# Danderson123/Amira

Measured on AMD Instinct MI355X. Metric: gene-mers/s to corrected GeneMerGraph, higher is better.
Workload: dtype int32; 1 GPU; synthetic 1M reads x 60 genes, k=5, 20k-gene vocab: build + error-correction sweep (build, filter(3,1), correct, build, clip(5), correct, build); reads_per_gpu=1000000, genes_per_read=60, k=5, vocab=20000, gene_mers_per_gpu=56000000, final_nodes=472478, final_edges=1054844, multi_gpu=n/a

## Files before the change

amira_amd/csrc/amg_adjacency.hip:

```cpp
#include "amg_device.h"

__global__ void k_adj_keys(const int* __restrict__ e_src, const signed char* __restrict__ e_sdir,
                           long long n_edges, unsigned int* __restrict__ keys,
                           unsigned int* __restrict__ vals) {
  long long e = (long long)blockIdx.x * blockDim.x + threadIdx.x;
  if (e >= n_edges) return;
  keys[e] = 2u * (unsigned int)e_src[e] + (e_sdir[e] > 0 ? 0u : 1u);
  vals[e] = (unsigned int)e;
}

__global__ void k_row_offsets(const unsigned int* __restrict__ keys, long long n_edges, long long n_rows,
                              long long* __restrict__ off) {
  long long i = (long long)blockIdx.x * blockDim.x + threadIdx.x;
  if (i > n_edges) return;
  const long long prev = i > 0 ? (long long)keys[i - 1] : -1;
  const long long cur = i < n_edges ? (long long)keys[i] : n_rows;
  for (long long r = prev + 1; r <= cur; ++r) off[r] = i;
}

__device__ __forceinline__ unsigned int adj_row_of(const int* __restrict__ e_src, const signed char* __restrict__ e_sdir,
                                                   long long e) {
  return 2u * (unsigned int)e_src[e] + (e_sdir[e] > 0 ? 0u : 1u);
}

__global__ void k_adjc_ticket(const int* __restrict__ e_src, const signed char* __restrict__ e_sdir, long long n_edges,
                              unsigned int* __restrict__ cnt, unsigned int* __restrict__ tick) {
  long long e = (long long)blockIdx.x * blockDim.x + threadIdx.x;
  if (e < n_edges) tick[e] = atomicAdd(&cnt[adj_row_of(e_src, e_sdir, e)], 1u);
}

__global__ void k_adjc_fill(const int* __restrict__ e_src, const signed char* __restrict__ e_sdir, long long n_edges,
                            const long long* __restrict__ off, const unsigned int* __restrict__ tick,
                            unsigned int* __restrict__ tmp) {
  long long e = (long long)blockIdx.x * blockDim.x + threadIdx.x;
  if (e < n_edges) tmp[off[adj_row_of(e_src, e_sdir, e)] + tick[e]] = (unsigned int)e;
}

__global__ __launch_bounds__(256) void k_adjc_rows(const long long* __restrict__ off, long long n_rows,
                                                   const unsigned int* __restrict__ tmp, int* __restrict__ adj_edge,
                                                   unsigned int* __restrict__ long_rows, unsigned long long* n_long) {
  long long r = (long long)blockIdx.x * blockDim.x + threadIdx.x;
  long long o = 0;
  int cnt = 0;
  if (r < n_rows) {
    o = off[r];
    cnt = (int)(off[r + 1] - o);
  }
  bool mine = cnt > 2;
  if (cnt == 1) {
    adj_edge[o] = (int)tmp[o];
  } else if (cnt == 2) {
    const unsigned int a = tmp[o], b = tmp[o + 1];
    adj_edge[o] = (int)(a < b ? a : b);
    adj_edge[o + 1] = (int)(a < b ? b : a);
  } else if (cnt > WAVE_ROW_MAX) {
    long_rows[atomicAdd(n_long, 1ull)] = (unsigned int)r;
    mine = false;
  }
  wave_rows_in_order(mine, 0u, o, cnt, tmp,
                     [&](unsigned int, long long ro, int, int rank, unsigned int x) { adj_edge[ro + rank] = (int)x; });
}

#define HUB_BLOCKS 8
__global__ __launch_bounds__(256) void k_adjc_long(const unsigned int* __restrict__ long_rows,
                                                   const unsigned long long* __restrict__ n_long,
                                                   const long long* __restrict__ off, const unsigned int* __restrict__ tmp,
                                                   int* __restrict__ adj_edge, unsigned int* hub_bits, long long hub_words) {
  __shared__ unsigned int s_wave[4];
  const unsigned long long n = *n_long;
  for (unsigned long long q = blockIdx.x; q < n; q += gridDim.x) {
    const unsigned int r = long_rows[q];
    const long long o = off[r];
    const int cnt = (int)(off[r + 1] - o);
    if (cnt > HUGE_ROW) continue;
    for (int j = threadIdx.x; j < cnt; j += 256) {
      const unsigned int x = tmp[o + j];
      int rank = 0;
      for (int i = 0; i < cnt; ++i) rank += tmp[o + i] < x ? 1 : 0;
      adj_edge[o + rank] = (int)x;
    }
  }
  if (blockIdx.x >= HUB_BLOCKS) return;
  for (unsigned long long q = blockIdx.x; q < n; q += HUB_BLOCKS) {
    const unsigned int r = long_rows[q];
    const long long o = off[r];
    const long long cnt = off[r + 1] - o;
    if (cnt <= HUGE_ROW) continue;
    huge_row_in_order(tmp + o, cnt, hub_bits + (long long)blockIdx.x * hub_words, hub_words, s_wave,
                      [&](long long rank, unsigned int id) { adj_edge[o + rank] = (int)id; });
  }
}

__global__ void k_uf_init(int* parent, long long n) {
  long long i = (long long)blockIdx.x * blockDim.x + threadIdx.x;
  if (i < n) parent[i] = (int)i;
}

__global__ void k_uf_links(const unsigned long long* __restrict__ pkey, long long n_pairs, unsigned int* __restrict__ starts) {
  long long i = (long long)blockIdx.x * blockDim.x + threadIdx.x;
  if (i >= n_pairs) return;
  const unsigned long long key = pkey[i];
  const unsigned int a = (unsigned int)((key >> 32) & 0x7fffffffull), b = (unsigned int)(key & 0xffffffffull) - 1u;
  if (b == a + 1u) starts[b] = 0u;
}

__global__ void k_uf_run_starts(const unsigned int* __restrict__ starts, const long long* __restrict__ run_of, long long n,
                                int* __restrict__ run_start) {
  long long i = (long long)blockIdx.x * blockDim.x + threadIdx.x;
  if (i < n && starts[i]) run_start[run_of[i]] = (int)i;
}

__global__ void k_uf_init_runs(const unsigned int* __restrict__ starts, const long long* __restrict__ run_of,
                               const int* __restrict__ run_start, long long n, int* __restrict__ parent) {
  long long i = (long long)blockIdx.x * blockDim.x + threadIdx.x;
  if (i < n) parent[i] = run_start[run_of[i] + (long long)starts[i] - 1];
}

__global__ void k_uf_union(const unsigned long long* __restrict__ pkey, long long n_pairs, int* parent) {
  long long i = (long long)blockIdx.x * blockDim.x + threadIdx.x;
  if (i >= n_pairs) return;
  unsigned long long key = pkey[i];
  int a = (int)((key >> 32) & 0x7fffffffull);
  int b = (int)((key & 0xffffffffull) - 1ull);
  if (b == a + 1) return;
  while (true) {
    a = uf_find(parent, a);
    b = uf_find(parent, b);
    if (a == b) break;
    if (a > b) { int t = a; a = b; b = t; }
    int old = atomicCAS(parent + b, b, a);
    if (old == b) break;
    b = old;
  }
}

__global__ void k_uf_roots(int* parent, long long n, unsigned int* __restrict__ is_root, int* __restrict__ root_copy) {
  long long i = (long long)blockIdx.x * blockDim.x + threadIdx.x;
  if (i == 0) is_root[n] = 0u;
  if (i >= n) return;
  int r = uf_find(parent, (int)i);
  parent[i] = r;
  root_copy[i] = r;
  is_root[i] = (r == (int)i) ? 1u : 0u;
}

__global__ void k_uf_label(const int* __restrict__ root, const long long* __restrict__ root_rank,
                           long long n, int* __restrict__ comp) {
  long long i = (long long)blockIdx.x * blockDim.x + threadIdx.x;
  if (i >= n) return;
  int r = root[i];
  while (root[r] != r) r = root[r];
  comp[i] = (int)(root_rank[r] + 1);
}

int ensure_components(amg_ctx* c) {
  if (c->comp_valid) return AMG_OK;
  if (c->comp_from_claims) return bx_components_from_claims(c);
  hipStream_t st = c->stream;
  const long long P = c->n_pairs, D = c->n_nodes;
  stage_begin(c, "components");
  AMGCHK(c->node_comp.ensure((size_t)(D + 1) * sizeof(int)));
  int* parent = c->node_comp.as<int>();
  AMGCHK(c->s1.ensure((size_t)(D + 2) * sizeof(long long)));
  AMGCHK(c->s2.ensure((size_t)(D + 2) * sizeof(unsigned int) + (size_t)(D + 2) * sizeof(int)));
  unsigned int* is_root = c->s2.as<unsigned int>();
  int* root_copy = reinterpret_cast<int*>(is_root + (D + 2));
  long long ncomp = 0;
  if (D > 0) {
    if (P > 0) {
      AMGCHK(c->s3.ensure((size_t)(D + 2) * sizeof(unsigned int)));
      AMGCHK(c->s4.ensure((size_t)(D + 2) * sizeof(int)));
      AMGCHK(c->s5.ensure((size_t)(D + 2) * sizeof(long long)));
      unsigned int* starts = c->s3.as<unsigned int>();
      int* run_start = c->s4.as<int>();
      long long* run_of = c->s5.as<long long>();
      ClearList cl;
      cl.add(starts, (size_t)D * sizeof(unsigned int), 1u);
      AMGCHK(clear_many(c, cl));
      hipLaunchKernelGGL(k_uf_links, dim3(nblk(P, 256)), dim3(256), 0, st, c->pair_key.as<unsigned long long>(), P, starts);
      AMGCHK(prim_exscan_u32_to_i64(c, starts, run_of, (size_t)D));
      hipLaunchKernelGGL(k_uf_run_starts, dim3(nblk(D, 256)), dim3(256), 0, st, starts, run_of, D, run_start);
      hipLaunchKernelGGL(k_uf_init_runs, dim3(nblk(D, 256)), dim3(256), 0, st, starts, run_of, run_start, D, parent);
      hipLaunchKernelGGL(k_uf_union, dim3(nblk(P, 256)), dim3(256), 0, st,
                         c->pair_key.as<unsigned long long>(), P, parent);
    } else {
      hipLaunchKernelGGL(k_uf_init, dim3(nblk(D, 256)), dim3(256), 0, st, parent, D);
    }
    hipLaunchKernelGGL(k_uf_roots, dim3(nblk(D, 256)), dim3(256), 0, st, parent, D, is_root, root_copy);
    AMGCHK(prim_exscan_u32_to_i64(c, is_root, c->s1.as<long long>(), (size_t)D + 1));
    hipLaunchKernelGGL(k_uf_label, dim3(nblk(D, 256)), dim3(256), 0, st, root_copy,
                       c->s1.as<long long>(), D, parent);
    FetchList l;
    l.add(c->s1.as<long long>() + D);
    AMGCHK(fetch(c, l, reinterpret_cast<unsigned long long*>(&ncomp)));
  }
  stage_end(c);
  c->n_components = ncomp;
  c->comp_valid = true;
  return AMG_OK;
}

int ensure_adjacency(amg_ctx* c) {
  if (c->adj_valid) return AMG_OK;
  hipStream_t st = c->stream;
  const long long D = c->n_nodes, E = c->n_edges;
  stage_begin(c, "adjacency");
  AMGCHK(c->adj_off.ensure((size_t)(2 * D + 2) * sizeof(long long)));
  AMGCHK(c->adj_edge.ensure((size_t)(E + 2) * sizeof(int)));
  AMGCHK(c->s1.ensure((size_t)(E + 2) * sizeof(unsigned int)));
  AMGCHK(c->s2.ensure((size_t)(E + 2) * sizeof(unsigned int)));
  AMGCHK(c->s3.ensure((size_t)(E + 2) * sizeof(unsigned int)));
  const char* force_sort = getenv("AMG_ADJ_SORT");
  if (E > 0 && E <= (4ll << 20) && !(force_sort && force_sort[0] == '1')) {
    AMGCHK(c->s1.ensure((size_t)(2 * D + 2 > E + 2 ? 2 * D + 2 : E + 2) * sizeof(unsigned int)));
    unsigned int* cnt = c->s1.as<unsigned int>();
    unsigned int* tick = c->s2.as<unsigned int>();
    unsigned int* tmp = c->s3.as<unsigned int>();
    AMGCHK(c->s4.ensure((size_t)(E / WAVE_ROW_MAX + 2) * sizeof(unsigned int)));
    unsigned int* long_rows = c->s4.as<unsigned int>();
    unsigned long long* n_long = c->status.as<unsigned long long>() + ST_COMPACT_B;
    {
      ClearList cl;
      cl.add(cnt, (size_t)(2 * D + 2) * sizeof(unsigned int));
      cl.add(n_long, sizeof(unsigned long long));
      AMGCHK(clear_many(c, cl));
    }
    hipLaunchKernelGGL(k_adjc_ticket, dim3(nblk(E, 256)), dim3(256), 0, st, c->edge_src.as<int>(),
                       c->edge_sdir.as<signed char>(), E, cnt, tick);
    AMGCHK(prim_exscan_u32_to_i64(c, cnt, c->adj_off.as<long long>(), (size_t)(2 * D + 1)));
    hipLaunchKernelGGL(k_adjc_fill, dim3(nblk(E, 256)), dim3(256), 0, st, c->edge_src.as<int>(),
                       c->edge_sdir.as<signed char>(), E, c->adj_off.as<long long>(), tick, tmp);
    hipLaunchKernelGGL(k_adjc_rows, dim3(nblk(2 * D, 256)), dim3(256), 0, st, c->adj_off.as<long long>(), 2 * D, tmp,
                       c->adj_edge.as<int>(), long_rows, n_long);
    const long long hub_words = (E + 31) / 32 + 1;
    AMGCHK(c->hub_bits.ensure((size_t)HUB_BLOCKS * (size_t)hub_words * sizeof(unsigned int)));
    hipLaunchKernelGGL(k_adjc_long, dim3(256), dim3(256), 0, st, long_rows, n_long, c->adj_off.as<long long>(), tmp,
                       c->adj_edge.as<int>(), c->hub_bits.as<unsigned int>(), hub_words);
    stage_end(c);
    c->adj_valid = true;
    return AMG_OK;
  }
  if (E > 0) {
    hipLaunchKernelGGL(k_adj_keys, dim3(nblk(E, 256)), dim3(256), 0, st,
                       c->edge_src.as<int>(), c->edge_sdir.as<signed char>(), E,
                       c->s1.as<unsigned int>(), c->s2.as<unsigned int>());
    AMGCHK(prim_sort_u32_u32(c, c->s1.as<unsigned int>(), c->s3.as<unsigned int>(),
                             c->s2.as<unsigned int>(),
                             reinterpret_cast<unsigned int*>(c->adj_edge.p), (size_t)E,
                             ilog2_ceil((uint64_t)2 * D + 2) + 1));
  }
  hipLaunchKernelGGL(k_row_offsets, dim3(nblk(E + 1, 256)), dim3(256), 0, st,
                     c->s3.as<unsigned int>(), E, 2 * D, c->adj_off.as<long long>());
  stage_end(c);
  c->adj_valid = true;
  return AMG_OK;
}
```

amira_amd/csrc/amg_api.hip:

```cpp
#include <cstdarg>

#include "amg_device.h"

thread_local std::string g_amg_err;

int amg_fail(int code, const char* fmt, ...) {
  char buf[1024];
  va_list ap;
  va_start(ap, fmt);
  vsnprintf(buf, sizeof(buf), fmt, ap);
  va_end(ap);
  g_amg_err = buf;
  return code;
}

extern "C" const char* amg_last_error(void) { return g_amg_err.c_str(); }

void stages_reset(amg_ctx* c) {
  for (auto& s : c->stages) {
    (void)hipEventDestroy(s.a);
    (void)hipEventDestroy(s.b);
  }
  c->stages.clear();
}

void stage_begin(amg_ctx* c, const char* name) {
  if (!c->timing) return;
  StageTime s{name, nullptr, nullptr, 0.f};
  (void)hipEventCreate(&s.a);
  (void)hipEventCreate(&s.b);
  (void)hipEventRecord(s.a, c->stream);
  c->stages.push_back(s);
}

void stage_end(amg_ctx* c) {
  if (!c->timing || c->stages.empty()) return;
  (void)hipEventRecord(c->stages.back().b, c->stream);
}

extern "C" int amg_last_timings(amg_ctx* c, const char** names, float* ms, int cap) {
  if (!c) return amg_fail(AMG_E_ARG, "null ctx");
  (void)hipStreamSynchronize(c->stream);
  int n = 0;
  for (auto& s : c->stages) {
    if (n >= cap) break;
    float t = 0.f;
    if (hipEventElapsedTime(&t, s.a, s.b) != hipSuccess) t = -1.f;
    s.ms = t;
    names[n] = s.name;
    ms[n] = t;
    ++n;
  }
  return n;
}

extern "C" int amg_set_timing(amg_ctx* c, int on) {
  if (!c) return amg_fail(AMG_E_ARG, "null ctx");
  c->timing = on != 0;
  if (!c->timing) stages_reset(c);
  return AMG_OK;
}

__global__ __launch_bounds__(256) void k_clear_many(ClearArgs a) { clear_args_part(a, blockIdx.x, gridDim.x); }

__global__ void k_fetch(FetchList l, unsigned long long* mail, unsigned long long ticket) {
  const int i = threadIdx.x;
  const int n = l.n > 0 ? l.n : 1;
  if (i < n) {
    const unsigned long long v = i < l.n ? *l.p[i] : 0ull;
    mail[2 * i] = v;
    __threadfence_system();
    __hip_atomic_store(mail + 2 * i + 1, ticket, __ATOMIC_RELEASE, __HIP_MEMORY_SCOPE_SYSTEM);
  }
}

int fetch(amg_ctx* c, const FetchList& l, unsigned long long* out, const ClearList* filler) {
  if (l.overflow) return amg_fail(AMG_E_ARG, "fetch: more than %d words in one list", FETCH_MAX);
  const bool plain = getenv("AMG_PLAIN_SYNC") != nullptr;
  if (plain) {
    for (int i = 0; i < l.n; ++i)
      HIPCHK(hipMemcpyAsync(out + i, l.p[i], sizeof(unsigned long long), hipMemcpyDeviceToHost, c->stream));
    if (filler) AMGCHK(clear_many(c, *filler));
    HIPCHK(hipStreamSynchronize(c->stream));
    return AMG_OK;
  }
  if (!c->mail_host) {
    HIPCHK(hipHostMalloc(reinterpret_cast<void**>(&c->mail_host), 2 * (FETCH_MAX + 1) * sizeof(unsigned long long),
                         hipHostMallocMapped));
    HIPCHK(hipHostGetDevicePointer(reinterpret_cast<void**>(&c->mail_dev), c->mail_host, 0));
    for (int i = 0; i < 2 * (FETCH_MAX + 1); ++i) c->mail_host[i] = 0;
  }
  const unsigned long long ticket = ++c->mail_ticket;
  hipLaunchKernelGGL(k_fetch, dim3(1), dim3(FETCH_MAX <= 64 ? 64 : 128), 0, c->stream, l, c->mail_dev, ticket);
  if (filler) AMGCHK(clear_many(c, *filler));
  const int n = l.n > 0 ? l.n : 1;
  volatile unsigned long long* m = c->mail_host;
  int have = 0;
  for (unsigned long long spins = 0; have < n; ++spins) {
    while (have < n && __atomic_load_n(&m[2 * have + 1], __ATOMIC_ACQUIRE) == ticket) ++have;
    if (have == n) break;
    __builtin_ia32_pause();
    if ((spins & 0xfffffull) == 0xfffffull) {
      const hipError_t e = hipStreamQuery(c->stream);
      if (e != hipSuccess && e != hipErrorNotReady) return amg_fail(AMG_E_HIP, "%s", hipGetErrorString(e));
      if (e == hipSuccess) {
        while (have < n && __atomic_load_n(&m[2 * have + 1], __ATOMIC_ACQUIRE) == ticket) ++have;
        if (have < n) return amg_fail(AMG_E_HIP, "read-back kernel did not run");
      }
    }
  }
  for (int i = 0; i < l.n; ++i) out[i] = m[2 * i];
  return AMG_OK;
}

int stream_wait(amg_ctx* c) {
  FetchList l;
  return fetch(c, l, nullptr);
}

int fetch_status(amg_ctx* c, unsigned long long* out, const ClearList* filler) {
  FetchList l;
  l.add_words(c->status.p, ST_WORDS);
  return fetch(c, l, out, filler);
}

int clear_many(amg_ctx* c, const ClearList& l) {
  if (l.overflow) return amg_fail(AMG_E_ARG, "clear_many: more than %d ranges in one list", CLEAR_MAX);
  if (l.n == 0) return AMG_OK;
  const ClearArgs a = clear_args(l);
  unsigned long long most = 0;
  for (int i = 0; i < a.n; ++i) most = a.words[i] > most ? a.words[i] : most;
  unsigned long long blocks = (most / 4 + 256 * 8 - 1) / (256 * 8);
  if (blocks < 1) blocks = 1;
  if (blocks > 4096) blocks = 4096;
  hipLaunchKernelGGL(k_clear_many, dim3((unsigned int)blocks), dim3(256), 0, c->stream, a);
  return AMG_OK;
}

extern "C" int amg_create(int device, amg_ctx** out) {
  if (!out) return amg_fail(AMG_E_ARG, "null out pointer");
  *out = nullptr;
  int n = 0;
  hipError_t e = hipGetDeviceCount(&n);
  if (e != hipSuccess || n <= 0)
    return amg_fail(AMG_E_HIP, "no HIP device available (%s): libamg has no CPU path",
                    e == hipSuccess ? "count = 0" : hipGetErrorString(e));
  if (device < 0 || device >= n) return amg_fail(AMG_E_ARG, "device %d out of range [0,%d)", device, n);
  HIPCHK(hipSetDevice(device));
  amg_ctx* c = new amg_ctx();
  c->device = device;
  e = hipStreamCreateWithFlags(&c->stream, hipStreamNonBlocking);
  if (e != hipSuccess) {
    delete c;
    return amg_fail(AMG_E_HIP, "hipStreamCreate: %s", hipGetErrorString(e));
  }
  int r = c->status.ensure(ST_WORDS * sizeof(unsigned long long));
  if (r != AMG_OK) {
    delete c;
    return r;
  }
  const char* t = getenv("AMG_TIMING");
  c->timing = !(t && t[0] == '0');
  *out = c;
  return AMG_OK;
}

extern "C" int amg_destroy(amg_ctx* c) {
  if (!c) return AMG_OK;
  (void)hipSetDevice(c->device);
  (void)hipStreamSynchronize(c->stream);
  stages_reset(c);
  dist_release(c);
  bubbles_release(c);
  DevBuf* all[] = {&c->tokens,    &c->read_off,  &c->gene_start, &c->gene_end,  &c->read_len,
                   &c->node_tab,  &c->edge_tab,  &c->tok_slot,   &c->tok_node,  &c->tok_dir, &c->tok_pair,
                   &c->node_tokens, &c->node_cov, &c->node_first, &c->node_comp, &c->node_alive,
                   &c->edge_src,  &c->edge_tgt,  &c->edge_sdir,  &c->edge_tdir, &c->edge_cov,
                   &c->edge_alive, &c->adj_off,  &c->adj_edge,   &c->read_fix, &c->ladj_off, &c->ladj, &c->ladj_rows, &c->ladj_pos, &c->ladj_keys, &c->hub_bits, &c->pair_key, &c->pair_first, &c->pair_cnt, &c->match_read, &c->match_pos, &c->match_off, &c->match_wave,  &c->c_tokens_buf,
                   &c->c_read_off, &c->c_orig,   &c->c_changed,  &c->c_gstart,  &c->c_gend,
                   &c->c_read_len, &c->status,   &c->sort_tmp, &c->scan_state,   &c->s0, &c->s1, &c->s2, &c->s3,
                   &c->s4, &c->s5, &c->cnt_state, &c->cnt_list, &c->bnd_bits, &c->nw_rec, &c->gap_rec, &c->gm_mask, &c->gm_tab, &c->gm_res, &c->gm_list, &c->gm_q, &c->gm_pool, &c->gm_gene, &c->gm_fail, &c->gm_ctr, &c->routes_dev, &c->nw_big, &c->x_first, &c->x_slot, &c->x_final, &c->x_efirst, &c->x_eslot, &c->x_ecnt, &c->x_ncnt, &c->x_ftag, &c->f_ctrs, &c->x_efinal, &c->x_first_all, &c->pos_off, &c->c_pos_off, &c->pos1_s, &c->pos1_e,
                   &c->c_src, &c->rd_src, &c->alt_tok_node, &c->alt_tok_dir, &c->alt_ntok, &c->alt_ncov, &c->alt_nfirst,
                   &c->alt_nalive, &c->alt_pkey, &c->alt_pfirst, &c->alt_pcnt};
  for (DevBuf* b : all) b->release();
  if (c->mail_host) (void)hipHostFree(c->mail_host);
  (void)hipStreamDestroy(c->stream);
  delete c;
  return AMG_OK;
}

extern "C" int amg_sync(amg_ctx* c) {
  if (!c) return amg_fail(AMG_E_ARG, "null ctx");
  HIPCHK(hipStreamSynchronize(c->stream));
  return AMG_OK;
}

extern "C" void* amg_stream(amg_ctx* c) { return c ? (void*)c->stream : nullptr; }

static int copy_in(amg_ctx* c, DevBuf& dst, const void* src, size_t bytes, int on_device) {
  if (on_device == 2) {
    dst.borrow(src, bytes);
    return AMG_OK;
  }
  AMGCHK(dst.ensure(bytes + 64));
  if (bytes)
    HIPCHK(hipMemcpyAsync(dst.p, src, bytes, on_device ? hipMemcpyDeviceToDevice : hipMemcpyHostToDevice,
                          c->stream));
  return AMG_OK;
}

extern "C" int amg_set_reads(amg_ctx* c, const int32_t* tokens, const int64_t* read_offsets,
                             int64_t n_reads, int32_t two_v, int on_device) {
  if (!c) return amg_fail(AMG_E_ARG, "null ctx");
  if (n_reads < 0 || !read_offsets) return amg_fail(AMG_E_ARG, "bad read_offsets / n_reads");
  if (two_v <= 0 || (two_v & 1)) return amg_fail(AMG_E_ARG, "two_v must be a positive even number");
  HIPCHK(hipSetDevice(c->device));
  int64_t n_tokens = 0;
  if (on_device) {
    HIPCHK(hipMemcpy(&n_tokens, read_offsets + n_reads, sizeof(int64_t), hipMemcpyDeviceToHost));
  } else {
    if (read_offsets[0] != 0) return amg_fail(AMG_E_ARG, "read_offsets[0] must be 0");
    for (int64_t r = 0; r < n_reads; ++r)
      if (read_offsets[r + 1] < read_offsets[r])
        return amg_fail(AMG_E_ARG, "read_offsets not monotone at read %lld", (long long)r);
    n_tokens = read_offsets[n_reads];
  }
  if (n_tokens < 0) return amg_fail(AMG_E_ARG, "read_offsets[n_reads] is negative");
  if (n_tokens > 0 && !tokens) return amg_fail(AMG_E_ARG, "null tokens");
  AMGCHK(copy_in(c, c->tokens, tokens, (size_t)n_tokens * sizeof(int32_t), on_device));
  AMGCHK(copy_in(c, c->read_off, read_offsets, (size_t)(n_reads + 1) * sizeof(int64_t), on_device));
  HIPCHK(hipStreamSynchronize(c->stream));
  c->n_reads = n_reads;
  c->n_tokens = n_tokens;
  c->two_v = two_v;
  c->have_pos = c->have_read_len = false;
  c->built = false;
  c->derive_ready = c->dist_candidate = false;
  c->hint_bound = 0;
  c->have_corrected = false;
  c->match_valid = false;
  c->node_hint = 0;
  c->cnt_hint_reset = true;
  return AMG_OK;
}

extern "C" int amg_set_positions(amg_ctx* c, const int64_t* gene_start, const int64_t* gene_end,
                                 const int64_t* read_len, int on_device) {
  if (!c) return amg_fail(AMG_E_ARG, "null ctx");
  if (c->two_v <= 0) return amg_fail(AMG_E_STATE, "amg_set_reads first");
  if (!gene_start || !gene_end) return amg_fail(AMG_E_ARG, "null positions");
  HIPCHK(hipSetDevice(c->device));
  AMGCHK(copy_in(c, c->gene_start, gene_start, (size_t)c->n_tokens * sizeof(int64_t), on_device));
  AMGCHK(copy_in(c, c->gene_end, gene_end, (size_t)c->n_tokens * sizeof(int64_t), on_device));
  c->have_pos = true;
  c->pos_identity = true;
  c->pos0_own = false;
  c->pos_n0 = c->n_tokens;
  c->pos1_used = c->c_pos1_used = 0;
  c->have_corrected = false;
  c->have_read_len = false;
  if (read_len) {
    AMGCHK(copy_in(c, c->read_len, read_len, (size_t)c->n_reads * sizeof(int64_t), on_device));
    c->have_read_len = true;
  }
  HIPCHK(hipStreamSynchronize(c->stream));
  return AMG_OK;
}

extern "C" int amg_set_read_lengths(amg_ctx* c, const int64_t* read_len, int on_device) {
  if (!c || !read_len) return amg_fail(AMG_E_ARG, "null argument");
  if (c->two_v <= 0) return amg_fail(AMG_E_STATE, "amg_set_reads first");
  HIPCHK(hipSetDevice(c->device));
  AMGCHK(copy_in(c, c->read_len, read_len, (size_t)c->n_reads * sizeof(int64_t), on_device));
  c->have_read_len = true;
  HIPCHK(hipStreamSynchronize(c->stream));
  return AMG_OK;
}

__global__ void k_count_flags(const unsigned char* __restrict__ f, long long n,
                              unsigned long long* out) {
  long long i = (long long)blockIdx.x * blockDim.x + threadIdx.x;
  unsigned long long v = (i < n && f[i]) ? 1ull : 0ull;
  for (int d = 32; d > 0; d >>= 1) v += __shfl_down(v, d, 64);
  if ((threadIdx.x & 63) == 0 && v) atomicAdd(out, v);
}

static int count_flags(amg_ctx* c, const DevBuf& buf, long long n, int64_t* out) {
  *out = 0;
  if (n <= 0) return AMG_OK;
  unsigned long long* ctr = c->status.as<unsigned long long>() + ST_MISC;
  HIPCHK(hipMemsetAsync(ctr, 0, sizeof(unsigned long long), c->stream));
  hipLaunchKernelGGL(k_count_flags, dim3((unsigned)((n + 255) / 256)), dim3(256), 0, c->stream,
                     buf.as<unsigned char>(), n, ctr);
  unsigned long long h = 0;
  HIPCHK(hipMemcpyAsync(&h, ctr, sizeof(h), hipMemcpyDeviceToHost, c->stream));
  HIPCHK(hipStreamSynchronize(c->stream));
  *out = (int64_t)h;
  return AMG_OK;
}

extern "C" int amg_sizes(amg_ctx* c, int64_t* n_reads, int64_t* n_tokens) {
  if (!c) return amg_fail(AMG_E_ARG, "null ctx");
  if (n_reads) *n_reads = c->n_reads;
  if (n_tokens) *n_tokens = c->n_tokens;
  return AMG_OK;
}

extern "C" int amg_graph_sizes(amg_ctx* c, int64_t* n_nodes, int64_t* n_edges, int32_t* k) {
  if (!c) return amg_fail(AMG_E_ARG, "null ctx");
  if (!c->built) return amg_fail(AMG_E_STATE, "amg_build first");
  if (n_nodes) *n_nodes = c->n_nodes;
  if (n_edges) *n_edges = c->n_edges;
  if (k) *k = c->k;
  return AMG_OK;
}

extern "C" int amg_counts(amg_ctx* c, amg_counts_t* o) {
  if (!c || !o) return amg_fail(AMG_E_ARG, "null argument");
  memset(o, 0, sizeof(*o));
  o->n_reads = c->n_reads;
  o->n_tokens = c->n_tokens;
  o->two_v = c->two_v;
  if (!c->built) return AMG_OK;
  HIPCHK(hipSetDevice(c->device));
  o->k = c->k;
  o->n_windows = c->n_windows;
  o->n_short_reads = c->n_short;
  o->n_nodes = c->n_nodes;
  o->n_edges = c->n_edges;
  o->n_pairs = c->n_pairs;
  AMGCHK(ensure_components(c));
  o->n_components = c->n_components;
  o->node_table_slots = c->node_slots;
  o->edge_table_slots = c->edge_slots;
  o->exact_keys = c->exact_keys ? (c->x_fp ? 2 : 1) : 0;
  o->derived = c->derived ? 1 : 0;
  o->build_retries = c->retries;
  AMGCHK(count_flags(c, c->node_alive, c->n_nodes, &o->n_live_nodes));
  AMGCHK(count_flags(c, c->edge_alive, c->n_edges, &o->n_live_edges));
  AMGCHK(count_flags(c, c->read_fix, c->n_reads, &o->n_reads_to_correct));
  return AMG_OK;
}

static int d2h(amg_ctx* c, void* dst, const DevBuf& src, size_t bytes) {
  if (!dst || bytes == 0) return AMG_OK;
  HIPCHK(hipMemcpyAsync(dst, src.p, bytes, hipMemcpyDeviceToHost, c->stream));
  return AMG_OK;
}

__global__ void k_first_split(const long long* __restrict__ first, long long n,
                              long long* __restrict__ tok, signed char* __restrict__ dir) {
  long long i = (long long)blockIdx.x * blockDim.x + threadIdx.x;
  if (i >= n) return;
  long long f = first[i];
  tok[i] = f >> 1;
  dir[i] = (f & 1) ? -1 : 1;
}

extern "C" int amg_get_nodes(amg_ctx* c, int32_t* canon_tokens, uint32_t* coverage,
                             int64_t* first_token, int8_t* first_dir, int32_t* component,
                             uint8_t* alive) {
  NEED_BUILT(c);
  const size_t D = (size_t)c->n_nodes;
  if (component) AMGCHK(ensure_components(c));
  AMGCHK(d2h(c, canon_tokens, c->node_tokens, D * c->k * sizeof(int32_t)));
  AMGCHK(d2h(c, coverage, c->node_cov, D * sizeof(uint32_t)));
  AMGCHK(d2h(c, component, c->node_comp, D * sizeof(int32_t)));
  AMGCHK(d2h(c, alive, c->node_alive, D));
  if ((first_token || first_dir) && D) {
    AMGCHK(c->s1.ensure(D * sizeof(long long)));
    AMGCHK(c->s2.ensure(D));
    hipLaunchKernelGGL(k_first_split, dim3((unsigned)((D + 255) / 256)), dim3(256), 0, c->stream,
                       c->node_first.as<long long>(), (long long)D, c->s1.as<long long>(),
                       c->s2.as<signed char>());
    AMGCHK(d2h(c, first_token, c->s1, D * sizeof(int64_t)));
    AMGCHK(d2h(c, first_dir, c->s2, D));
  }
  HIPCHK(hipStreamSynchronize(c->stream));
  return AMG_OK;
}

extern "C" int amg_get_edges(amg_ctx* c, int32_t* src, int32_t* tgt, int8_t* sdir, int8_t* tdir,
                             uint32_t* coverage, uint8_t* alive) {
  NEED_BUILT(c);
  const size_t E = (size_t)c->n_edges;
  AMGCHK(d2h(c, src, c->edge_src, E * sizeof(int32_t)));
  AMGCHK(d2h(c, tgt, c->edge_tgt, E * sizeof(int32_t)));
  AMGCHK(d2h(c, sdir, c->edge_sdir, E));
  AMGCHK(d2h(c, tdir, c->edge_tdir, E));
  AMGCHK(d2h(c, coverage, c->edge_cov, E * sizeof(uint32_t)));
  AMGCHK(d2h(c, alive, c->edge_alive, E));
  HIPCHK(hipStreamSynchronize(c->stream));
  return AMG_OK;
}

extern "C" int amg_get_read_nodes(amg_ctx* c, int32_t* tok_node, int8_t* tok_dir) {
  NEED_BUILT(c);
  AMGCHK(d2h(c, tok_node, c->tok_node, (size_t)c->n_tokens * sizeof(int32_t)));
  AMGCHK(d2h(c, tok_dir, c->tok_dir, (size_t)c->n_tokens));
  HIPCHK(hipStreamSynchronize(c->stream));
  return AMG_OK;
}

__global__ __launch_bounds__(256) void k_gather_read_nodes(const int* __restrict__ tok_node,
                                                            const long long* __restrict__ first, const long long* __restrict__ start,
                                                            long long n_rows, int* __restrict__ out) {
  const long long r = (long long)blockIdx.x * 4 + (threadIdx.x >> 6);
  if (r >= n_rows) return;
  const long long a = first[r], o = start[r], n = start[r + 1] - o;
  for (long long i = threadIdx.x & 63; i < n; i += 64) out[o + i] = tok_node[a + i];
}

extern "C" int amg_get_read_nodes_rows(amg_ctx* c, const int64_t* first_token, const int64_t* out_start, int64_t n_rows,
                                       int32_t* node_ids) {
  NEED_BUILT(c);
  if (n_rows < 0 || (n_rows > 0 && (!first_token || !out_start || !node_ids))) return amg_fail(AMG_E_ARG, "bad arguments");
  if (n_rows == 0) return AMG_OK;
  const long long total = out_start[n_rows];
  for (int64_t r = 0; r < n_rows; ++r) {
    const long long n = out_start[r + 1] - out_start[r];
    if (out_start[0] != 0 || n < 0 || first_token[r] < 0 || first_token[r] + n > c->n_tokens)
      return amg_fail(AMG_E_ARG, "amg_get_read_nodes_rows: row %lld lies outside the read set", (long long)r);
  }
  if (total == 0) return AMG_OK;
  hipStream_t st = c->stream;
  AMGCHK(c->s0.ensure((size_t)n_rows * sizeof(long long)));
  AMGCHK(c->s1.ensure((size_t)(n_rows + 1) * sizeof(long long)));
  AMGCHK(c->s2.ensure((size_t)total * sizeof(int)));
  HIPCHK(hipMemcpyAsync(c->s0.p, first_token, (size_t)n_rows * sizeof(long long), hipMemcpyHostToDevice, st));
  HIPCHK(hipMemcpyAsync(c->s1.p, out_start, (size_t)(n_rows + 1) * sizeof(long long), hipMemcpyHostToDevice, st));
  hipLaunchKernelGGL(k_gather_read_nodes, dim3((unsigned)((n_rows + 3) / 4)), dim3(256), 0, st, c->tok_node.as<int>(),
                     c->s0.as<long long>(), c->s1.as<long long>(), (long long)n_rows, c->s2.as<int>());
  HIPCHK(hipMemcpyAsync(node_ids, c->s2.p, (size_t)total * sizeof(int), hipMemcpyDeviceToHost, st));
  HIPCHK(hipStreamSynchronize(st));
  return AMG_OK;
}

extern "C" int amg_get_node_adj(amg_ctx* c, int64_t* offsets, int32_t* edge_ids) {
  NEED_BUILT(c);
  AMGCHK(ensure_adjacency(c));
  AMGCHK(d2h(c, offsets, c->adj_off, (size_t)(2 * c->n_nodes + 1) * sizeof(int64_t)));
  AMGCHK(d2h(c, edge_ids, c->adj_edge, (size_t)c->n_edges * sizeof(int32_t)));
  HIPCHK(hipStreamSynchronize(c->stream));
  return AMG_OK;
}

extern "C" int amg_get_reads_to_correct(amg_ctx* c, uint8_t* flags) {
  NEED_BUILT(c);
  AMGCHK(d2h(c, flags, c->read_fix, (size_t)c->n_reads));
  HIPCHK(hipStreamSynchronize(c->stream));
  return AMG_OK;
}

__global__ void k_read_window_count(const int* __restrict__ tok_node,
                                    const long long* __restrict__ read_off, long long n_reads,
                                    unsigned int* __restrict__ cnt) {
  long long r = (long long)blockIdx.x * blockDim.x + threadIdx.x;
  if (r >= n_reads) return;
  unsigned int n = 0;
  for (long long t = read_off[r]; t < read_off[r + 1]; ++t) n += tok_node[t] >= 0 ? 1u : 0u;
  cnt[r] = n;
}

__global__ void k_read_window_emit(const int* __restrict__ tok_node,
                                   const long long* __restrict__ read_off, long long n_reads,
                                   const long long* __restrict__ base, unsigned int* __restrict__ keys,
                                   unsigned int* __restrict__ vals) {
  long long r = (long long)blockIdx.x * blockDim.x + threadIdx.x;
  if (r >= n_reads) return;
  long long o = base[r];
  for (long long t = read_off[r]; t < read_off[r + 1]; ++t) {
    int n = tok_node[t];
    if (n >= 0) {
      keys[o] = (unsigned int)n;
      vals[o] = (unsigned int)r;
      ++o;
    }
  }
}

__global__ void k_mark_first_of_run(const unsigned int* __restrict__ keys,
                                    const unsigned int* __restrict__ vals, long long n,
                                    unsigned int* __restrict__ keep,
                                    unsigned int* __restrict__ per_node) {
  long long i = (long long)blockIdx.x * blockDim.x + threadIdx.x;
  if (i >= n) return;
  unsigned int kf = (i == 0 || keys[i] != keys[i - 1] || vals[i] != vals[i - 1]) ? 1u : 0u;
  keep[i] = kf;
  if (kf) atomicAdd(&per_node[keys[i]], 1u);
}

__global__ void k_scatter_kept(const unsigned int* __restrict__ vals, const unsigned int* __restrict__ keep,
                               const long long* __restrict__ pos, long long n, int* __restrict__ out) {
  long long i = (long long)blockIdx.x * blockDim.x + threadIdx.x;
  if (i >= n) return;
  if (keep[i]) out[pos[i]] = (int)vals[i];
}

extern "C" int amg_get_node_reads(amg_ctx* c, int64_t* offsets, int32_t* read_idx) {
  NEED_BUILT(c);
  if (!offsets) return amg_fail(AMG_E_ARG, "offsets must not be NULL");
  hipStream_t st = c->stream;
  const long long R = c->n_reads, D = c->n_nodes;
  AMGCHK(c->s0.ensure((size_t)(R + 2) * sizeof(unsigned int)));
  AMGCHK(c->s5.ensure((size_t)(R + 2) * sizeof(long long)));
  HIPCHK(hipMemsetAsync(c->s0.p, 0, (size_t)(R + 2) * sizeof(unsigned int), st));
  if (R > 0)
    hipLaunchKernelGGL(k_read_window_count, dim3((unsigned)((R + 255) / 256)), dim3(256), 0, st,
                       c->tok_node.as<int>(), c->read_off.as<long long>(), R, c->s0.as<unsigned int>());
  AMGCHK(prim_exscan_u32_to_i64(c, c->s0.as<unsigned int>(), c->s5.as<long long>(), (size_t)R + 1));
  long long W = 0;
  HIPCHK(hipMemcpyAsync(&W, c->s5.as<long long>() + R, sizeof(long long), hipMemcpyDeviceToHost, st));
  HIPCHK(hipStreamSynchronize(st));
  AMGCHK(c->s1.ensure((size_t)(W + 2) * sizeof(unsigned int)));
  AMGCHK(c->s2.ensure((size_t)(W + 2) * sizeof(unsigned int)));
  AMGCHK(c->s3.ensure((size_t)(W + 2) * sizeof(unsigned int)));
  AMGCHK(c->s4.ensure((size_t)(W + 2) * sizeof(unsigned int)));
  if (R > 0)
    hipLaunchKernelGGL(k_read_window_emit, dim3((unsigned)((R + 255) / 256)), dim3(256), 0, st,
                       c->tok_node.as<int>(), c->read_off.as<long long>(), R, c->s5.as<long long>(),
                       c->s1.as<unsigned int>(), c->s2.as<unsigned int>());
  AMGCHK(prim_sort_u32_u32(c, c->s1.as<unsigned int>(), c->s3.as<unsigned int>(),
                           c->s2.as<unsigned int>(), c->s4.as<unsigned int>(), (size_t)W,
                           ilog2_ceil((uint64_t)D + 2) + 1));
  AMGCHK(c->s0.ensure((size_t)(D + 2) * sizeof(unsigned int)));
  HIPCHK(hipMemsetAsync(c->s0.p, 0, (size_t)(D + 2) * sizeof(unsigned int), st));
  if (W > 0)
    hipLaunchKernelGGL(k_mark_first_of_run, dim3((unsigned)((W + 255) / 256)), dim3(256), 0, st,
                       c->s3.as<unsigned int>(), c->s4.as<unsigned int>(), W,
                       c->s1.as<unsigned int>(), c->s0.as<unsigned int>());
  AMGCHK(c->s5.ensure((size_t)(D + 2) * sizeof(long long)));
  AMGCHK(prim_exscan_u32_to_i64(c, c->s0.as<unsigned int>(), c->s5.as<long long>(), (size_t)D + 1));
  AMGCHK(d2h(c, offsets, c->s5, (size_t)(D + 1) * sizeof(int64_t)));
  HIPCHK(hipStreamSynchronize(st));
  if (read_idx && W > 0) {
    long long total = offsets[D];
    AMGCHK(c->s2.ensure((size_t)(W + 2) * sizeof(long long)));
    HIPCHK(hipMemsetAsync(c->s1.as<unsigned int>() + W, 0, sizeof(unsigned int), st));
    AMGCHK(prim_exscan_u32_to_i64(c, c->s1.as<unsigned int>(), c->s2.as<long long>(), (size_t)W + 1));
    AMGCHK(c->s0.ensure((size_t)(total + 2) * sizeof(int)));
    hipLaunchKernelGGL(k_scatter_kept, dim3((unsigned)((W + 255) / 256)), dim3(256), 0, st,
                       c->s4.as<unsigned int>(), c->s1.as<unsigned int>(), c->s2.as<long long>(), W,
                       c->s0.as<int>());
    AMGCHK(d2h(c, read_idx, c->s0, (size_t)total * sizeof(int32_t)));
    HIPCHK(hipStreamSynchronize(st));
  }
  return AMG_OK;
}
```

amira_amd/csrc/amg_build.hip:

```cpp
#include "amg_device.h"

#include "amg_tile.h"

uint64_t pow2_at_least(uint64_t x) {
  uint64_t p = 1024;
  while (p < x) p <<= 1;
  return p;
}

int bs_read_stats(amg_ctx* c, int k, const ClearList* also) {
  hipStream_t st = c->stream;
  const long long T = c->n_tokens, R = c->n_reads;
  stage_begin(c, "read_stats");
  const size_t words = (size_t)(T >> 5) + BND_PAD_WORDS;
  AMGCHK(c->bnd_bits.ensure(words * sizeof(unsigned int)));
  {
    ClearList cl;
    if (also) cl = *also;
    cl.add(c->bnd_bits.p, words * sizeof(unsigned int));
    AMGCHK(clear_many(c, cl));
  }
  if (R > 0)
    hipLaunchKernelGGL(k_read_stats, dim3(nblk(R, 256) < 512u ? nblk(R, 256) : 512u), dim3(256), 0, st,
                       c->read_off.as<long long>(), R, T, k, c->status.as<unsigned long long>(),
                       c->bnd_bits.as<unsigned int>());
  stage_end(c);
  return AMG_OK;
}

int bs_alloc_nodes(amg_ctx* c, long long D) {
  AMGCHK(c->node_tokens.ensure((size_t)(D * c->k + 1) * sizeof(int)));
  AMGCHK(c->node_cov.ensure((size_t)(D + 1) * sizeof(unsigned int)));
  AMGCHK(c->node_first.ensure((size_t)(D + 1) * sizeof(long long)));
  AMGCHK(c->node_comp.ensure((size_t)(D + 1) * sizeof(int)));
  AMGCHK(c->node_alive.ensure((size_t)(D + 1)));
  return AMG_OK;
}

int bs_alloc_pairs(amg_ctx* c, long long P) {
  AMGCHK(c->pair_key.ensure((size_t)(P + 2) * sizeof(unsigned long long)));
  AMGCHK(c->pair_first.ensure((size_t)(P + 2) * sizeof(unsigned long long)));
  AMGCHK(c->pair_cnt.ensure((size_t)(P + 2) * sizeof(unsigned int)));
  return AMG_OK;
}

int bs_finish_from_pairs(amg_ctx* c) {
  const long long P = c->n_pairs, R = c->n_reads;
  stage_begin(c, "edge_emit");
  AMGCHK(c->s5.ensure((size_t)(P + 2) * sizeof(long long)));
  long long* base = c->s5.as<long long>();
  const long long cap = 2 * P;
  AMGCHK(c->edge_src.ensure((size_t)(cap + 2) * sizeof(int)));
  AMGCHK(c->edge_tgt.ensure((size_t)(cap + 2) * sizeof(int)));
  AMGCHK(c->edge_sdir.ensure((size_t)(cap + 2)));
  AMGCHK(c->edge_tdir.ensure((size_t)(cap + 2)));
  AMGCHK(c->edge_cov.ensure((size_t)(cap + 2) * sizeof(unsigned int)));
  AMGCHK(c->edge_alive.ensure((size_t)(cap + 2)));
  AMGCHK(c->read_fix.ensure((size_t)R + 1));
  long long total = 0;
  {
    ClearList cl;
    cl.add(c->read_fix.p, (size_t)R + 1);
    if (P > 0) {
      AMGCHK(prim_exscan_emit_edges(c, c->pair_key.as<unsigned long long>(), c->pair_cnt.as<unsigned int>(),
                                    c->pair_first.as<unsigned long long>(), (size_t)P, base + P, c->edge_src.as<int>(),
                                    c->edge_tgt.as<int>(), c->edge_sdir.as<signed char>(), c->edge_tdir.as<signed char>(),
                                    c->edge_cov.as<unsigned int>(), c->edge_alive.as<unsigned char>(), &cl));
    } else {
      AMGCHK(clear_many(c, cl));
    }
  }
  {
    FetchList l;
    l.add(P > 0 ? static_cast<const void*>(base + P) : c->status.p);
    const bool learn = count_learn_add(c, &l);
    unsigned long long v[1 + COUNT_LEARN_WORDS] = {0};
    AMGCHK(fetch(c, l, v));
    if (P > 0) total = (long long)v[0];
    if (learn) count_learn_take(c, v + 1);
  }
  c->n_edges = total;
  stage_end(c);
  c->ladj_valid = false;
  c->ladj_stale = false;
  c->pristine = !c->comp_from_claims;
  c->edge_own_deaths = false;
  c->comp_valid = false;
  c->adj_valid = false;
  c->n_components = 0;
  return AMG_OK;
}

extern "C" int amg_finalize(amg_ctx* c) {
  if (!c) return amg_fail(AMG_E_ARG, "null ctx");
  if (!c->built) return amg_fail(AMG_E_STATE, "amg_build first");
  HIPCHK(hipSetDevice(c->device));
  stages_reset(c);
  AMGCHK(ensure_components(c));
  AMGCHK(ensure_adjacency(c));
  HIPCHK(hipStreamSynchronize(c->stream));
  return AMG_OK;
}

uint64_t slots_for(uint64_t n) {
  const uint64_t lo = n * 3, hi = n * 32, cap = 4ull << 20;
  const uint64_t want = hi < cap ? hi : cap;
  return pow2_at_least(want > lo ? want : lo);
}

void bs_size_tables(amg_ctx* c) {
  uint64_t want = c->node_hint > 0 ? slots_for((uint64_t)c->node_hint) : (uint64_t)c->n_tokens / 4;
  c->node_slots = (int64_t)pow2_at_least(want);
  if (c->node_slots > (1ll << 30)) c->node_slots = 1ll << 30;
  c->edge_slots = 1024;
}

BuildSwitches read_build_switches() {
  BuildSwitches sw;
  auto is_zero = [](const char* v) { return v && atoi(v) == 0; };
  if (const char* e = getenv("AMG_X_HEAD_TILES")) sw.head_tiles_set = true, sw.head_tiles = atoll(e);
  if (const char* e = getenv("AMG_CLAIM_SHARDS")) sw.claim_shards = atoi(e) != 0;
  sw.tight_bits = getenv("AMG_X_TIGHT_BITS") != nullptr;
  if (const char* e = getenv("AMG_KEY_MODE")) sw.key_fp = e[0] == 'f';
  sw.node_buckets = !is_zero(getenv("AMG_NODE_BUCKETS"));
  sw.generic_k = getenv("AMG_X_GENERIC_K") != nullptr;
  sw.rank_sort = getenv("AMG_X_RANK_SORT") != nullptr;
  if (const char* e = getenv("AMG_EDGE_LONE")) sw.edge_lone = atoi(e) != 0;
  sw.edge_home = !is_zero(getenv("AMG_EDGE_HOME"));
  sw.no_derive = getenv("AMG_NO_DERIVE") != nullptr;
  if (const char* e = getenv("AMG_TEST_WEAK_FP")) sw.weak_fp = atoi(e);
  if (const char* e = getenv("AMG_COUNT_INLINE")) sw.count_inline = e[0] == '1';
  if (const char* e = getenv("AMG_COUNT_LIST_SEG")) sw.count_list_seg = atoi(e);
  sw.count_debug = getenv("AMG_COUNT_DEBUG") != nullptr;
  return sw;
}

int grow_after_overflow(amg_ctx* c, Overflow cause) {
  ++c->retries;
  if (cause == OV_NODE_TABLE) {
    if (c->node_slots >= (1ll << 30)) return amg_fail(AMG_E_OVERFLOW, "node table at maximum size");
    c->node_slots = c->node_slots * 4 > (1ll << 30) ? (1ll << 30) : c->node_slots * 4;
  } else if (cause == OV_EDGE_TABLE) {
    c->edge_slots *= 4;
  } else {
    c->seed = c->seed * 6364136223846793005ull + 1442695040888963407ull;
    if (c->weak_fp_builds > 0) --c->weak_fp_builds;
  }
  return AMG_OK;
}

static int build_impl(amg_ctx* c, int32_t k, uint32_t min_node_cov, uint32_t min_edge_cov, bool* fused) {
  *fused = false;
  if (!c) return amg_fail(AMG_E_ARG, "null ctx");
  if (k < 1 || k > AMG_MAX_K) return amg_fail(AMG_E_ARG, "k must be in [1, %d]", AMG_MAX_K);
  if (c->two_v <= 0) return amg_fail(AMG_E_STATE, "amg_set_reads first");
  HIPCHK(hipSetDevice(c->device));
  stages_reset(c);
  c->sw = read_build_switches();
  const bool derive = c->derive_ready && k == c->k && !c->dist_mode && !c->sw.no_derive;
  c->derive_ready = c->dist_candidate = false;
  c->derived = false;
  c->built = false;
  c->have_corrected = false;
  c->match_valid = false;
  c->retries = 0;
  c->tok_base = 0;
  c->tok_total = c->n_tokens;
  if (derive) {
    bool done = false;
    AMGCHK(derive_from_previous(c, k, &done));
    if (done) return AMG_OK;
  }
  c->k = k;
  c->dist_mode = false;
  c->comp_from_claims = false;
  if (c->hint_bound > 0) {
    if (c->hint_bound_k == k) c->node_hint = c->hint_bound > 256 ? c->hint_bound : 256;
    c->hint_bound = 0;
  }
  c->weak_fp_builds = c->sw.weak_fp;
  c->count_inline = c->sw.count_inline;
  bs_size_tables(c);
  c->exact_keys = false;
  const bool exact = bx_applicable(c, k);
  for (int attempt = 0; attempt < 12; ++attempt) {
    Overflow which = OV_NONE;
    int r;
    if (exact && min_node_cov > 0) {
      r = bx_nodes_filtered(c, k, min_node_cov, &which);
      if (r == AMG_OK) r = bx_edges(c, &which, min_edge_cov);
      *fused = true;
    } else if (exact) {
      r = bx_nodes(c, k, &which);
      if (r == AMG_OK) r = bx_edges(c, &which);
    } else {
      r = bs_nodes_pass(c, k, &which);
      if (r == AMG_OK) r = bs_nodes_rank_local(c);
      if (r == AMG_OK) r = bs_edges_pass(c, &which);
      if (r == AMG_OK) r = bs_pairs_from_local(c);
    }
    if (r == AMG_OK) r = bs_finish_from_pairs(c);
    if (r == AMG_OK && *fused) r = bx_flag_dead_reads(c);
    if (r == AMG_OK) {
      c->built = true;
      const int64_t seen = *fused ? c->n_local_nodes : c->n_nodes;
      c->node_hint = seen > 256 ? seen : 256;
      return AMG_OK;
    }
    if (r != AMG_E_OVERFLOW || which == OV_NONE) return r;
    AMGCHK(grow_after_overflow(c, which));
  }
  return amg_fail(AMG_E_OVERFLOW, "build did not converge after 12 attempts");
}

extern "C" int amg_build(amg_ctx* c, int32_t k) {
  bool fused = false;
  return build_impl(c, k, 0, 0, &fused);
}

extern "C" int amg_build_filtered(amg_ctx* c, int32_t k, uint32_t min_node_cov, uint32_t min_edge_cov) {
  bool fused = false;
  const int r = build_impl(c, k, min_node_cov < 1 ? 1 : min_node_cov, min_edge_cov < 1 ? 1 : min_edge_cov, &fused);
  if (r != AMG_OK || fused) return r;
  return amg_filter(c, min_node_cov, min_edge_cov);
}

#define MULTI_MAX 8
extern "C" int amg_build_multi(amg_ctx* const* ctxs, const int32_t* ks, int32_t n) {
  if (!ctxs || !ks || n < 1 || n > MULTI_MAX) return amg_fail(AMG_E_ARG, "amg_build_multi: 1 .. %d graphs", MULTI_MAX);
  amg_ctx* c0 = ctxs[0];
  if (!c0 || c0->two_v <= 0) return amg_fail(AMG_E_STATE, "amg_set_reads on the first ctx first");
  for (int i = 0; i < n; ++i) {
    if (!ctxs[i]) return amg_fail(AMG_E_ARG, "null ctx");
    if (ctxs[i]->device != c0->device) return amg_fail(AMG_E_ARG, "amg_build_multi: one device");
    if (ks[i] < 1 || ks[i] > AMG_MAX_K) return amg_fail(AMG_E_ARG, "k must be in [1, %d]", AMG_MAX_K);
    for (int j = 0; j < i; ++j)
      if (ctxs[j] == ctxs[i]) return amg_fail(AMG_E_ARG, "amg_build_multi: one ctx per graph");
  }
  HIPCHK(hipSetDevice(c0->device));
  HIPCHK(hipStreamSynchronize(c0->stream));
  const long long T = c0->n_tokens, R = c0->n_reads;
  std::vector<hipStream_t> own(n);
  for (int i = 0; i < n; ++i) {
    amg_ctx* c = ctxs[i];
    own[i] = c->stream;
    if (i == 0) continue;
    HIPCHK(hipStreamSynchronize(c->stream));
    c->tokens.borrow(c0->tokens.p, (size_t)T * sizeof(int32_t));
    c->read_off.borrow(c0->read_off.p, (size_t)(R + 1) * sizeof(int64_t));
    c->n_reads = R;
    c->n_tokens = T;
    c->two_v = c0->two_v;
    c->have_pos = c->have_read_len = false;
    c->node_hint = 0;
    c->cnt_hint_reset = true;
    c->derive_ready = c->dist_candidate = false;
    c->stream = c0->stream;
  }
  struct Restore {
    amg_ctx* const* ctxs;
    std::vector<hipStream_t>& own;
    int n;
    ~Restore() {
      for (int i = 0; i < n; ++i) ctxs[i]->stream = own[i];
    }
  } restore{ctxs, own, n};
  for (int i = 0; i < n; ++i) AMGCHK(amg_build(ctxs[i], ks[i]));
  HIPCHK(hipStreamSynchronize(c0->stream));
  return AMG_OK;
}
```

amira_amd/csrc/amg_correct.h:

```cpp
#pragma once
#include "amg_device.h"

enum { RC_SKIP = 0, RC_COPY = 1, RC_DROP = 2, RC_TRIM = 3, RC_GAPPED = 4, RC_KEEP_ORIG = 5 };

struct CorrArgs {
  const int* tokens;
  const long long* read_off;
  const int* tok_node;
  const signed char* tok_dir;
  const unsigned char* read_fix;
  const long long* p0s;
  const long long* p0e;
  const long long* p1s;
  const long long* p1e;
  long long n0;
  const long long* pos_off;
  const long long* read_len;
  long long n_reads;
  int k, flip, have_pos;
  unsigned int* gflag;
  unsigned long long* max_bound;
  unsigned long long* lmask;
  unsigned long long* n_runs;
  unsigned char* cls;
  unsigned char* cls_final;
  int* r_start;
  int* r_end;
  unsigned int* bound;
  const long long* tmp_off;
  unsigned int* new_len;
  int* tmp_tok;
};

__device__ __forceinline__ void pos_base(const CorrArgs& a, long long off, const long long*& gs, const long long*& ge) {
  if (off < a.n0) {
    gs = a.p0s + off;
    ge = a.p0e + off;
  } else {
    gs = a.p1s + (off - a.n0);
    ge = a.p1e + (off - a.n0);
  }
}

__device__ __forceinline__ long long bcast_i64(long long v, int lane) {
  const unsigned int lo = (unsigned int)__builtin_amdgcn_readlane((int)(unsigned int)v, lane);
  const unsigned int hi = (unsigned int)__builtin_amdgcn_readlane((int)(unsigned int)((unsigned long long)v >> 32), lane);
  return (long long)(((unsigned long long)hi << 32) | lo);
}

__device__ __forceinline__ void wave_sync() {
  __builtin_amdgcn_fence(__ATOMIC_ACQ_REL, "wavefront");
  __builtin_amdgcn_wave_barrier();
}

struct __attribute__((aligned(16))) GapRec {
  int r, L0, start, end;
  long long t0, dst;
  unsigned long long mask;
  long long pad;
};

__device__ __forceinline__ unsigned long long gap_run_ends(unsigned long long lv, int start, int end) {
  const unsigned long long inside =
      (end >= 63 ? ~0ull : ((1ull << (end + 1)) - 1ull)) & ~((1ull << (start & 63)) - 1ull);
  return ~lv & inside & (lv >> 1);
}
__device__ __forceinline__ void gap_run_terminals(unsigned long long lv, int i, int& ps, int& pe) {
  ps = 63 - __clzll((long long)(lv & ((1ull << i) - 1ull)));
  pe = i + 1;
}

struct GapArgs {
  CorrArgs a;
  GView g;
  const GapRec* rec;
  const int* gapped_reads;
  long long n_gapped;
  int* pool;
  unsigned long long pool_cap;
  unsigned long long* pool_used;
  unsigned long long* status;
  int* cand;
  unsigned int cand_stride;
  unsigned char* final_cls;
  unsigned char* need_slow;
  const int* gq;
  const int4* qres;
  const int* qpool;
};

#define GF_MAXW 128
#define GF_MAXGAP 16
#define GF_POOL 384
#define GF_CAND 136
#define GF_MAXCOMBO 256
#define GM_INLINE 64
#define LEAN_CHUNK 32
#define CLS_READS 64
#define PACK_READS 64
enum {
  GS_NOT_TRIED = 1,
  GS_WINDOWS = 2,
  GS_RUNS = 3,
  GS_MEMO_UNFIT = 4,
  GS_RECORDS = 5,
  GS_COMBOS = 6,
  GS_CAND = 7,
  GS_CODES = 8
};
enum {
  GL_NO_SLOTS = 1,
  GL_ANSWERS = 2,
  GL_LONG = 3,
  GL_OTHER = 4,
  GL_CODES = 5
};

#define NWF_MAX_M 64
#define NWF_MAX_N 128
__device__ __forceinline__ bool nw_fast_ok(long long N, long long M) {
  return N <= NWF_MAX_N && M <= NWF_MAX_M && N > 0 && M > 0;
}

struct __attribute__((aligned(16))) NwRec {
  int r, M, N, pad;
  long long t0, dst;
  long long pdst;
  long long poff;
};

struct NwArgs {
  CorrArgs a;
  const NwRec* rec;
  long long* o_gs;
  long long* o_ge;
  const int* gapped_reads;
  long long n_gapped;
  const unsigned char* final_cls;
  const long long* big_off;
  unsigned char* big_buf;
  int allow_fast;
  int shortcuts;
};

struct PackArgs {
  CorrArgs a;
  const long long* new_idx;
  const long long* new_off;
  const unsigned char* final_cls;
  int* o_tok;
  long long* o_off;
  int* o_orig;
  unsigned char* o_changed;
  long long* o_src;
  const long long* pos_new;
  long long* o_posoff;
  long long* o_rl;
  long long out_reads, out_tokens;
  unsigned long long* dead_kept;
};

struct CorrSwitches {
  bool gap_memo;
  bool fast_gapped;
  bool lean_gapped;
  int fast_nw;
  int nw_shortcuts;
  const char* node_bound;
  bool routes;
  const char* gap_pool;
  const char* memo_spill;
};

struct CorrScratch {
  size_t per_read = 0;
  unsigned char *cls = nullptr, *final_cls = nullptr;
  int *r_start = nullptr, *r_end = nullptr;
  long long *nw_size = nullptr, *nw_off = nullptr;
  unsigned int *bound = nullptr, *new_len = nullptr, *flag = nullptr;
  long long *tmp_off = nullptr, *new_idx = nullptr, *new_off = nullptr;
  int* tmp_tok = nullptr;
  long long *plen = nullptr, *poffs = nullptr, *pos_new = nullptr;
  unsigned long long *max_bound = nullptr, *n_general = nullptr;
  unsigned long long* n_runs = nullptr;
  unsigned long long* dead_kept = nullptr;
  bool count_alive = false;
  DevBuf* glist = nullptr;
  DevBuf* cand = nullptr;
  DevBuf* pool = nullptr;
  DevBuf* need_slow = nullptr;
};

struct CorrCounts {
  long long tmp_total = 0, n_gapped = 0, total_runs = 0;
  unsigned long long max_bound = 0;
  bool carry = false;
  long long out_reads = 0, out_tokens = 0, big_total = 0, pos_total = 0;
  unsigned long long n_general = 0;
  long long n_queries = 0;
  int pool_retries = 0;
  bool lean_ran = false, fast_ran = false, memo = false;
};

static void fill_pos_args(amg_ctx* c, CorrArgs& a) {
  a.p0s = c->have_pos ? c->gene_start.as<long long>() : nullptr;
  a.p0e = c->have_pos ? c->gene_end.as<long long>() : nullptr;
  a.p1s = c->pos1_s.as<long long>();
  a.p1e = c->pos1_e.as<long long>();
  a.n0 = c->pos_n0;
  a.pos_off = (c->have_pos && !c->pos_identity) ? c->pos_off.as<long long>() : nullptr;
}

void corr_classify_launch(amg_ctx* c, const CorrArgs& a);
int corr_gapped(amg_ctx* c, const CorrSwitches& sw, const CorrScratch& S, const CorrArgs& a, CorrCounts& n);
int corr_nw_sizes(amg_ctx* c, const CorrSwitches& sw, const CorrScratch& S, const CorrArgs& a, long long n_gapped,
                  FetchList& shape);
int corr_grow_pos_pools(amg_ctx* c, const CorrCounts& n);
int corr_positions(amg_ctx* c, const CorrSwitches& sw, const CorrScratch& S, const CorrArgs& a, const CorrCounts& n);

int routes_begin(amg_ctx* c);
int routes_gapped(amg_ctx* c, const CorrScratch& S, const CorrCounts& n, const unsigned char* need_slow, const int* gq);
int routes_nw(amg_ctx* c, const CorrScratch& S, const CorrCounts& n);
int routes_end(amg_ctx* c, const CorrCounts& n);
```

amira_amd/csrc/amg_correct.hip:

```cpp
#include "amg_correct.h"

__global__ __launch_bounds__(256) void k_count_alive(const unsigned char* __restrict__ alive, long long n,
                                                     unsigned long long* out) {
  __shared__ unsigned int s_part[4];
  unsigned int c = 0;
  for (long long i = ((long long)blockIdx.x * blockDim.x + threadIdx.x) * 4; i < n; i += (long long)gridDim.x * blockDim.x * 4) {
    if (i + 4 <= n) {
      const unsigned int w = *reinterpret_cast<const unsigned int*>(alive + i);
      c += __popc(w & 0x01010101u);
    } else {
      for (long long j = i; j < n; ++j) c += alive[j] ? 1u : 0u;
    }
  }
  for (int d = 32; d > 0; d >>= 1) c += (unsigned int)__shfl_xor((int)c, d, 64);
  if ((threadIdx.x & 63) == 0) s_part[threadIdx.x >> 6] = c;
  __syncthreads();
  if (threadIdx.x == 0 && (s_part[0] | s_part[1] | s_part[2] | s_part[3]))
    atomicAdd(out, (unsigned long long)s_part[0] + s_part[1] + s_part[2] + s_part[3]);
}

__global__ __launch_bounds__(256) void k_corr_pack(PackArgs A) {
  const CorrArgs& a = A.a;
  const int lane = threadIdx.x & 63;
  const long long r = ((long long)blockIdx.x * 4 + (threadIdx.x >> 6)) * PACK_READS + lane;
  if (blockIdx.x == 0 && threadIdx.x == 0) A.o_off[A.out_reads] = A.out_tokens;
  long long dst = 0, src = 0;
  int n = 0;
  unsigned int dead = 0;
  if (r < a.n_reads && a.new_len[r] > 0) {
    dst = A.new_off[r];
    n = (int)a.new_len[r];
    const unsigned char fc = A.final_cls[r];
    if (fc == RC_KEEP_ORIG) {
      const long long nw = a.read_off[r + 1] - a.read_off[r] - a.k + 1;
      dead = nw <= 64 ? (unsigned int)(nw - __popcll(a.lmask[r])) : (unsigned int)nw;
    }
    long long poff = 0;
    if (fc == RC_GAPPED) {
      src = a.tmp_off[r] | (1ll << 62);
      if (a.have_pos) poff = A.pos_new[r];
    } else {
      const long long cut = fc == RC_TRIM ? a.r_start[r] : 0;
      src = a.read_off[r] + cut;
      if (a.have_pos) poff = (a.pos_off ? a.pos_off[r] : a.read_off[r]) + cut;
    }
    const long long q = A.new_idx[r];
    A.o_off[q] = dst;
    A.o_orig[q] = (int)r;
    A.o_changed[q] = (fc == RC_TRIM || fc == RC_GAPPED) ? 1 : 0;
    A.o_src[q] = fc == RC_GAPPED ? -1ll : src;
    if (a.have_pos) A.o_posoff[q] = poff;
    if (a.read_len) A.o_rl[q] = a.read_len[r];
  }
  if (__ballot(dead != 0u) != 0ull) {
    for (int d = 32; d > 0; d >>= 1) dead += (unsigned int)__shfl_xor((int)dead, d, 64);
    if (lane == 0) atomicAdd(A.dead_kept + 16 * (blockIdx.x & 15), (unsigned long long)dead);
  }
  if (__ballot(n > 0) == 0ull) return;
  for (int j0 = 0; j0 < PACK_READS; j0 += 4) {
    const int* sp[4];
    long long d[4];
    int nn[4], vt[4];
#pragma unroll
    for (int j = 0; j < 4; ++j) {
      nn[j] = __builtin_amdgcn_readlane(n, j0 + j);
      const long long sj = bcast_i64(src, j0 + j);
      d[j] = bcast_i64(dst, j0 + j);
      sp[j] = ((sj >> 62) & 1 ? a.tmp_tok : a.tokens) + (sj & ~(1ll << 62));
    }
#pragma unroll
    for (int j = 0; j < 4; ++j)
      if (lane < nn[j]) vt[j] = sp[j][lane];
#pragma unroll
    for (int j = 0; j < 4; ++j)
      if (lane < nn[j]) A.o_tok[d[j] + lane] = vt[j];
#pragma unroll
    for (int j = 0; j < 4; ++j)
      for (int i = 64 + lane; i < nn[j]; i += 64)
        A.o_tok[d[j] + i] = sp[j][i];
  }
}

static CorrSwitches read_switches() {
  auto is_one = [](const char* name) {
    const char* v = getenv(name);
    return v && v[0] == '1';
  };
  CorrSwitches sw;
  sw.gap_memo = !is_one("AMG_NO_GAP_MEMO");
  sw.fast_gapped = !is_one("AMG_NO_FAST_GAPPED");
  sw.lean_gapped = !is_one("AMG_NO_LEAN_GAPPED");
  sw.fast_nw = !is_one("AMG_NO_FAST_NW");
  sw.nw_shortcuts = !is_one("AMG_NW_NO_SHORTCUT");
  sw.node_bound = getenv("AMG_TEST_NODE_BOUND");
  sw.routes = is_one("AMG_CORR_ROUTES");
  sw.gap_pool = getenv("AMG_TEST_GAP_POOL");
  sw.memo_spill = getenv("AMG_TEST_MEMO_SPILL");
  return sw;
}

static int plan_per_read(amg_ctx* c, CorrScratch& S) {
  const size_t per_read = (size_t)(c->n_reads + 2);
  AMGCHK(c->s0.ensure(per_read * (1 + 1) + 64));
  AMGCHK(c->s1.ensure(per_read * sizeof(int) * 2 + per_read * sizeof(long long) * 2 + 64));
  AMGCHK(c->s2.ensure(per_read * sizeof(unsigned int) * 3));
  AMGCHK(c->s3.ensure(per_read * sizeof(long long) * 3));
  AMGCHK(c->gm_mask.ensure(per_read * sizeof(unsigned long long)));
  AMGCHK(c->gm_ctr.ensure((16 + 256 + 256 + 16) * sizeof(unsigned long long)));
  S.per_read = per_read;
  S.cls = c->s0.as<unsigned char>();
  S.final_cls = S.cls + per_read;
  S.r_start = c->s1.as<int>();
  S.r_end = S.r_start + per_read;
  S.nw_size = reinterpret_cast<long long*>(((uintptr_t)(S.r_end + per_read) + 15) & ~(uintptr_t)15);
  S.nw_off = S.nw_size + per_read;
  S.bound = c->s2.as<unsigned int>();
  S.new_len = S.bound + per_read;
  S.flag = S.new_len + per_read;
  S.tmp_off = c->s3.as<long long>();
  S.new_idx = S.tmp_off + per_read;
  S.new_off = S.new_idx + per_read;
  S.max_bound = S.n_general = c->status.as<unsigned long long>() + ST_MISC;
  S.n_runs = c->gm_ctr.as<unsigned long long>() + 16;
  S.dead_kept = S.n_runs + 256;
  S.count_alive = c->n_nodes >= (1ll << 20);
  S.glist = &c->c_orig;
  S.cand = &c->c_gstart;
  S.pool = &c->c_gend;
  S.need_slow = &c->c_changed;
  return AMG_OK;
}

static int plan_staging(amg_ctx* c, CorrScratch& S, long long tmp_total) {
  AMGCHK(c->c_tokens_buf.ensure((size_t)(tmp_total + 4) * sizeof(int)));
  AMGCHK(c->s4.ensure((size_t)(tmp_total + 4) * sizeof(int)));
  S.tmp_tok = c->s4.as<int>();
  return AMG_OK;
}

static int plan_positions(amg_ctx* c, CorrScratch& S, long long n_gapped) {
  AMGCHK(c->s5.ensure((size_t)(2 * (n_gapped + 2) + c->n_reads + 2) * sizeof(long long)));
  S.plen = c->s5.as<long long>();
  S.poffs = S.plen + (n_gapped + 2);
  S.pos_new = S.poffs + (n_gapped + 2);
  return AMG_OK;
}

static void corr_args(amg_ctx* c, const CorrScratch& S, CorrArgs& a) {
  a.tokens = c->tokens.as<int>();
  a.read_off = c->read_off.as<long long>();
  a.tok_node = c->tok_node.as<int>();
  a.tok_dir = c->tok_dir.as<signed char>();
  a.read_fix = c->read_fix.as<unsigned char>();
  fill_pos_args(c, a);
  a.read_len = c->have_read_len ? c->read_len.as<long long>() : nullptr;
  a.n_reads = c->n_reads;
  a.k = c->k;
  a.flip = c->two_v - 1;
  a.have_pos = c->have_pos ? 1 : 0;
  a.gflag = S.flag;
  a.max_bound = S.max_bound;
  a.lmask = c->gm_mask.as<unsigned long long>();
  a.n_runs = S.n_runs;
  a.cls = S.cls;
  a.cls_final = S.final_cls;
  a.r_start = S.r_start;
  a.r_end = S.r_end;
  a.bound = S.bound;
  a.tmp_off = S.tmp_off;
  a.new_len = S.new_len;
  a.tmp_tok = S.tmp_tok;
}

static int corr_classify(amg_ctx* c, const CorrScratch& S, const CorrArgs& a, CorrCounts& n) {
  hipStream_t st = c->stream;
  const long long R = c->n_reads;
  {
    ClearList cl;
    cl.add(S.bound, S.per_read * sizeof(unsigned int) * 3);
    cl.add(S.max_bound, sizeof(unsigned long long));
    cl.add(S.n_runs, (256 + 256 + 16) * sizeof(unsigned long long));
    AMGCHK(clear_many(c, cl));
  }
  if (R > 0) corr_classify_launch(c, a);
  if (S.count_alive)
    hipLaunchKernelGGL(k_count_alive, dim3(128), dim3(256), 0, st, c->node_alive.as<unsigned char>(), c->n_nodes,
                       S.dead_kept + 256);
  AMGCHK(prim_exscan_u32_pair(c, S.bound, S.tmp_off, S.flag, S.new_idx, (size_t)R));
  FetchList l;
  l.add(S.tmp_off + R);
  l.add(S.max_bound);
  l.add(S.new_idx + R);
  for (int i = 0; i < 16; ++i) l.add(S.n_runs + 16 * i);
  unsigned long long v[3 + 16];
  AMGCHK(fetch(c, l, v));
  n.tmp_total = (long long)v[0];
  n.max_bound = v[1];
  n.n_gapped = (long long)v[2];
  for (int i = 0; i < 16; ++i) n.total_runs += (long long)v[3 + i];
  n.carry = n.n_gapped > 0 && c->have_pos;
  return AMG_OK;
}

static int corr_shape(amg_ctx* c, const CorrSwitches& sw, CorrScratch& S, const CorrArgs& a, CorrCounts& n) {
  const long long R = c->n_reads;
  AMGCHK(prim_exscan_keep_and_len(c, S.new_len, S.new_idx, S.new_off, (size_t)R));
  FetchList shape;
  shape.add(S.new_idx + R);
  shape.add(S.new_off + R);
  if (n.carry) {
    AMGCHK(plan_positions(c, S, n.n_gapped));
    AMGCHK(corr_nw_sizes(c, sw, S, a, n.n_gapped, shape));
  }
  unsigned long long v[5] = {0, 0, 0, 0, 0};
  AMGCHK(fetch(c, shape, v));
  n.out_reads = (long long)v[0];
  n.out_tokens = (long long)v[1];
  n.big_total = (long long)v[2];
  n.pos_total = (long long)v[3];
  n.n_general = v[4];
  return AMG_OK;
}

static int ensure_outputs(amg_ctx* c, const CorrCounts& n) {
  AMGCHK(c->c_tokens_buf.ensure((size_t)(n.out_tokens + 64) * sizeof(int)));
  AMGCHK(c->c_read_off.ensure((size_t)(n.out_reads + 2) * sizeof(long long)));
  AMGCHK(c->c_orig.ensure((size_t)(n.out_reads + 2) * sizeof(int)));
  AMGCHK(c->c_changed.ensure((size_t)(n.out_reads + 2)));
  AMGCHK(c->c_src.ensure((size_t)(n.out_reads + 2) * sizeof(long long)));
  if (c->have_pos) AMGCHK(c->c_pos_off.ensure((size_t)(n.out_reads + 2) * sizeof(long long)));
  if (c->have_read_len) AMGCHK(c->c_read_len.ensure((size_t)(n.out_reads + 2) * sizeof(long long)));
  return AMG_OK;
}

static int corr_pack(amg_ctx* c, const CorrScratch& S, const CorrArgs& a, const CorrCounts& n) {
  PackArgs Pk;
  Pk.a = a;
  Pk.new_idx = S.new_idx;
  Pk.new_off = S.new_off;
  Pk.final_cls = S.final_cls;
  Pk.o_tok = c->c_tokens_buf.as<int>();
  Pk.o_off = c->c_read_off.as<long long>();
  Pk.o_orig = c->c_orig.as<int>();
  Pk.o_changed = c->c_changed.as<unsigned char>();
  Pk.o_src = c->c_src.as<long long>();
  Pk.pos_new = S.pos_new;
  Pk.o_posoff = c->have_pos ? c->c_pos_off.as<long long>() : nullptr;
  Pk.o_rl = c->have_read_len ? c->c_read_len.as<long long>() : nullptr;
  Pk.out_reads = n.out_reads;
  Pk.out_tokens = n.out_tokens;
  Pk.dead_kept = S.dead_kept;
  if (c->n_reads > 0)
    hipLaunchKernelGGL(k_corr_pack, dim3(nblk(c->n_reads, 4 * PACK_READS)), dim3(256), 0, c->stream, Pk);
  else
    HIPCHK(hipMemcpyAsync(c->c_read_off.as<long long>() + n.out_reads, &n.out_tokens, sizeof(long long),
                          hipMemcpyHostToDevice, c->stream));
  return AMG_OK;
}

static int corr_node_bound(amg_ctx* c, const CorrSwitches& sw, const CorrScratch& S, const CorrCounts& n) {
  FetchList l;
  for (int i = 0; i < 16; ++i) l.add(S.dead_kept + 16 * i);
  l.add(S.dead_kept + 256);
  unsigned long long v[17];
  AMGCHK(fetch(c, l, v));
  unsigned long long bound = S.count_alive ? v[16] : (unsigned long long)c->n_nodes;
  unsigned long long dead_kept = 0;
  for (int i = 0; i < 16; ++i) dead_kept += v[i];
  bound += dead_kept;
  c->c_derivable = n.n_gapped == 0 && dead_kept == 0 && !c->edge_own_deaths;
  c->c_node_bound = (int64_t)bound;
  if (sw.node_bound) c->c_node_bound = atoll(sw.node_bound);
  c->c_node_bound_k = c->k;
  return AMG_OK;
}

extern "C" int amg_correct_reads(amg_ctx* c, int64_t* n_out_reads, int64_t* n_out_tokens) {
  NEED_BUILT(c);
  const CorrSwitches sw = read_switches();
  stages_reset(c);
  c->have_corrected = false;
  CorrScratch S;
  CorrCounts n;
  CorrArgs a;
  AMGCHK(plan_per_read(c, S));
  corr_args(c, S, a);
  c->have_routes = false;
  if (sw.routes) AMGCHK(routes_begin(c));

  stage_begin(c, "correct_classify");
  AMGCHK(corr_classify(c, S, a, n));
  stage_end(c);
  AMGCHK(plan_staging(c, S, n.tmp_total));
  corr_args(c, S, a);

  if (n.n_gapped > 0) {
    stage_begin(c, "live_adjacency");
    AMGCHK(ensure_live_adj(c));
    stage_end(c);
    stage_begin(c, "correct_gapped");
    AMGCHK(corr_gapped(c, sw, S, a, n));
    stage_end(c);
  }

  stage_begin(c, "correct_pack");
  AMGCHK(corr_shape(c, sw, S, a, n));
  stage_end(c);
  AMGCHK(ensure_outputs(c, n));

  if (n.carry) {
    stage_begin(c, "correct_positions");
    AMGCHK(corr_grow_pos_pools(c, n));
    corr_args(c, S, a);
    AMGCHK(corr_positions(c, sw, S, a, n));
    if (sw.routes) AMGCHK(routes_nw(c, S, n));
    stage_end(c);
  }

  stage_begin(c, "correct_pack");
  AMGCHK(corr_pack(c, S, a, n));
  AMGCHK(corr_node_bound(c, sw, S, n));
  stage_end(c);
  if (sw.routes) AMGCHK(routes_end(c, n));
  c->c_reads = n.out_reads;
  c->c_tokens = n.out_tokens;
  c->c_pos1_used = c->pos1_used + (n.carry ? n.pos_total : 0);
  c->have_corrected = true;
  if (n_out_reads) *n_out_reads = n.out_reads;
  if (n_out_tokens) *n_out_tokens = n.out_tokens;
  return AMG_OK;
}
```

amira_amd/csrc/amg_count.hip:

```cpp
#include "amg_device.h"

#define HOT_IDS 39936
#define COUNT_MAX_SWEEPS 4
#define COUNT_LIST_SEG 256
#define COUNT_MAX_BLOCKS 256
#define COUNT_LIST_HEAD (2 + COUNT_MAX_BLOCKS)
struct CountSweeps {
  unsigned long long beyond[COUNT_MAX_SWEEPS];
  unsigned long long done[COUNT_MAX_SWEEPS];
};
struct CountHint { unsigned long long beyond, n; };
struct CountState {
  CountSweeps sweeps[2];
  CountHint hint[2];
};

template <bool GATHER>
__global__ __launch_bounds__(1024) void k_count_ids(int* __restrict__ ids, long long n,
                                                    const Slot* __restrict__ tab, long long lo,
                                                    int sweep, int last, CountSweeps* state,
                                                    CountHint* hint, unsigned int* __restrict__ out,
                                                    bool marked, unsigned int* list, unsigned int seg_cap) {
  __shared__ unsigned int s_cnt[HOT_IDS];
  __shared__ unsigned int s_listed;
  bool tail_all = last != 0;
  if (sweep > 0) {
    for (int q = 0; q < sweep; ++q)
      if (state->done[q]) return;
    const unsigned long long left = state->beyond[sweep - 1];
    if (sweep == 1 && blockIdx.x == 0 && threadIdx.x == 0) {
      hint->beyond = left;
      hint->n = (unsigned long long)n;
    }
    if (left == 0ull) return;
    if (sweep == 1 && list && list[1] == 1u && list[0] == 0u) {
      const unsigned int mine = list[2 + blockIdx.x];
      for (unsigned int i = threadIdx.x; i < mine; i += 1024u)
        atomicAdd(&out[list[COUNT_LIST_HEAD + blockIdx.x * COUNT_LIST_SEG + i]], 1u);
      if (blockIdx.x == 0 && threadIdx.x == 0) state->done[sweep] = 1ull;
      return;
    }
    if (left * 8ull <= (unsigned long long)n) tail_all = true;
  } else if (hint->n != 0ull && hint->beyond * 8ull <= hint->n) {
    tail_all = true;
  }
  const bool listing = sweep == 0 && !tail_all && list != nullptr && gridDim.x <= COUNT_MAX_BLOCKS;
  if (threadIdx.x == 0) s_listed = 0u;
  auto list_id = [&](int id) {
    const unsigned int at = atomicAdd(&s_listed, 1u);
    if (at < seg_cap) list[COUNT_LIST_HEAD + blockIdx.x * COUNT_LIST_SEG + at] = (unsigned int)id;
  };
  for (int i = threadIdx.x; i < HOT_IDS; i += 1024) s_cnt[i] = 0;
  __syncthreads();
  const long long stride = (long long)gridDim.x * 1024;
  unsigned int beyond = 0;
  auto tally = [&](int id, long long t) {
    bool made = false;
    if (marked && id != -1) {
      made = ((unsigned int)id & AMG_MADE_FLAG) != 0u;
      id = (int)((unsigned int)id & ~AMG_FLAG_MASK);
    }
    if (GATHER) {
      id = id < 0 ? -1 : tab[id].id;
      ids[t] = id;
    }
    if (id < 0 || made) return;
    const long long rel = (long long)id - lo;
    if (rel < 0) return;
    if (rel < HOT_IDS) {
      atomicAdd(&s_cnt[rel], 1u);
    } else {
      ++beyond;
      if (tail_all) atomicAdd(&out[id], 1u);
      else if (listing) list_id(id);
    }
  };
  typedef int i4 __attribute__((ext_vector_type(4)));
  const long long n4 = ((reinterpret_cast<uintptr_t>(ids) & 15) == 0) ? (n >> 2) : 0;
  i4* ids4 = reinterpret_cast<i4*>(ids);
  long long q = (long long)blockIdx.x * 1024 + threadIdx.x;
  auto tally4 = [&](i4 x, long long qi) {
    unsigned int mades = 0;
    if (marked) {
#pragma unroll
      for (int j = 0; j < 4; ++j)
        if (x[j] != -1 && ((unsigned int)x[j] & AMG_MADE_FLAG)) mades |= 1u << j;
    }
    if (GATHER) {
      i4 y;
#pragma unroll
      for (int j = 0; j < 4; ++j) {
        int id = x[j];
        if (marked && id != -1) id = (int)((unsigned int)id & ~AMG_FLAG_MASK);
        y[j] = id < 0 ? -1 : tab[id].id;
      }
      ids4[qi] = y;
      x = y;
    }
#pragma unroll
    for (int j = 0; j < 4; ++j) {
      int id = x[j];
      if (!GATHER && marked && id != -1) id = (int)((unsigned int)id & ~AMG_FLAG_MASK);
      if (id < 0 || (mades & (1u << j))) continue;
      const long long rel = (long long)id - lo;
      if (rel < 0) continue;
      if (rel < HOT_IDS) {
        atomicAdd(&s_cnt[rel], 1u);
      } else {
        ++beyond;
        if (tail_all) atomicAdd(&out[id], 1u);
        else if (listing) list_id(id);
      }
    }
  };
  for (; q + 3 * stride < n4; q += 4 * stride) {
    i4 v[4];
#pragma unroll
    for (int j = 0; j < 4; ++j) v[j] = GATHER ? ids4[q + j * stride] : __builtin_nontemporal_load(ids4 + q + j * stride);
#pragma unroll
    for (int j = 0; j < 4; ++j) tally4(v[j], q + j * stride);
  }
  for (; q < n4; q += stride) tally4(GATHER ? ids4[q] : __builtin_nontemporal_load(ids4 + q), q);
  for (long long t = 4 * n4 + (long long)blockIdx.x * 1024 + threadIdx.x; t < n; t += stride) tally(ids[t], t);
  for (int d = 32; d > 0; d >>= 1) beyond += __shfl_down(beyond, d, 64);
  if ((threadIdx.x & 63) == 0 && beyond) atomicAdd(&state->beyond[sweep], (unsigned long long)beyond);
  if (tail_all && blockIdx.x == 0 && threadIdx.x == 0) state->done[sweep] = 1ull;
  __syncthreads();
  if (listing && threadIdx.x == 0) {
    const unsigned int got = s_listed;
    list[2 + blockIdx.x] = got < seg_cap ? got : seg_cap;
    if (got > seg_cap) list[0] = 1u;
    if (blockIdx.x == 0) list[1] = 1u;
  }
  for (int i = threadIdx.x; i < HOT_IDS; i += 1024) {
    const unsigned int cnt = s_cnt[i];
    if (cnt) atomicAdd(&out[lo + i], cnt);
  }
}

static_assert(sizeof(CountState) == (4 * COUNT_MAX_SWEEPS + 4) * sizeof(unsigned long long), "cnt_state: two blocks, two hints");

int count_ids(amg_ctx* c, CountKind what, CountIds form, int* ids, long long n, long long n_ids, unsigned int* out,
              const Slot* gather_tab) {
  hipStream_t st = c->stream;
  const bool marked = form == IdsClaimsMarked;
  ClearList cl;
  cl.add(out, (size_t)(n_ids + 1) * sizeof(unsigned int), marked ? 1u : 0u);
  const bool fresh = !c->cnt_state.p || c->cnt_hint_reset;
  AMGCHK(c->cnt_state.ensure(sizeof(CountState)));
  if (fresh) c->cnt_sweeps[CountNodes] = c->cnt_sweeps[CountEdgeClasses] = COUNT_MAX_SWEEPS;
  c->cnt_hint_reset = false;
  CountState* cs = c->cnt_state.as<CountState>();
  CountSweeps* state = &cs->sweeps[what];
  CountHint* hint = &cs->hint[what];
  if (fresh) cl.add(cs, sizeof(CountState));
  else cl.add(state, sizeof(CountSweeps));
  AMGCHK(c->cnt_list.ensure((size_t)(COUNT_LIST_HEAD + COUNT_MAX_BLOCKS * COUNT_LIST_SEG) * sizeof(unsigned int)));
  unsigned int* list = c->cnt_list.as<unsigned int>();
  cl.add(list, COUNT_LIST_HEAD * sizeof(unsigned int));
  const unsigned int seg_cap = (unsigned int)std::min(std::max(c->sw.count_list_seg, 0), COUNT_LIST_SEG);
  AMGCHK(clear_many(c, cl));
  c->cnt_launched[0] = c->cnt_launched[1] = 0;
  if (n <= 0 || n_ids <= 0) return AMG_OK;
  long long ranges = (n_ids + HOT_IDS - 1) / HOT_IDS;
  if (ranges > COUNT_MAX_SWEEPS) ranges = COUNT_MAX_SWEEPS;
  if (ranges > c->cnt_sweeps[what]) ranges = c->cnt_sweeps[what];
  long long want_blocks = (n + 2 * HOT_IDS - 1) / (2 * HOT_IDS);
  unsigned int blocks = (unsigned int)(want_blocks < 1 ? 1 : (want_blocks < COUNT_MAX_BLOCKS ? want_blocks : COUNT_MAX_BLOCKS));
  c->cnt_launched[0] = (int)ranges;
  c->cnt_launched[1] = (int)blocks;
  for (long long r = 0; r < ranges; ++r) {
    const long long lo = r * HOT_IDS;
    const int last = (r == ranges - 1) ? 1 : 0;
    if (gather_tab && r == 0)
      hipLaunchKernelGGL(k_count_ids<true>, dim3(blocks), dim3(1024), 0, st, ids, n, gather_tab, lo,
                         (int)r, last, state, hint, out, marked, list, seg_cap);
    else
      hipLaunchKernelGGL(k_count_ids<false>, dim3(blocks), dim3(1024), 0, st, ids, n, gather_tab, lo,
                         (int)r, last, state, hint, out, marked, list, seg_cap);
  }
  if (c->sw.count_debug) {
    CountSweeps h;
    HIPCHK(hipStreamSynchronize(st));
    HIPCHK(hipMemcpy(&h, state, sizeof(h), hipMemcpyDeviceToHost));
    fprintf(stderr, "[amg] count %s%s: n %lld ids %lld sweeps %lld beyond %llu %llu %llu %llu done %llu %llu %llu %llu\n",
            what == CountNodes ? "nodes" : "edge classes", marked ? " (marked claims)" : "", n, n_ids, ranges, h.beyond[0],
            h.beyond[1], h.beyond[2], h.beyond[3], h.done[0], h.done[1], h.done[2], h.done[3]);
  }
  return AMG_OK;
}

static_assert(COUNT_LEARN_WORDS == 2 * COUNT_MAX_SWEEPS, "the done flags of both kinds");
bool count_learn_add(amg_ctx* c, FetchList* l) {
  if (!c->cnt_state.p || c->cnt_hint_reset) return false;
  CountState* cs = c->cnt_state.as<CountState>();
  for (int s = 0; s < 2; ++s) l->add_words(cs->sweeps[s].done, COUNT_MAX_SWEEPS);
  return true;
}

void count_learn_take(amg_ctx* c, const unsigned long long* done) {
  for (int s = 0; s < 2; ++s) {
    int used = COUNT_MAX_SWEEPS;
    for (int q = COUNT_MAX_SWEEPS - 1; q >= 0; --q)
      if (done[s * COUNT_MAX_SWEEPS + q]) used = q + 1;
    c->cnt_sweeps[s] = used;
  }
}

extern "C" int amg_count_probe(amg_ctx* c, int kind, int form, int32_t* ids, int64_t n, int64_t n_ids, const int32_t* tab_ids,
                               int64_t n_slots, int misalign, int flags, uint32_t* counts, int64_t* state) {
  if (!c || (kind != CountNodes && kind != CountEdgeClasses) || form < 0 || form > 2 || n < 0 || n_ids < 0 ||
      n_ids >= (1ll << 29) || (n > 0 && !ids) || misalign < 0 || misalign > 3 || !counts || !state ||
      (form == 2 && (n_slots < 0 || (n_slots > 0 && !tab_ids))))
    return amg_fail(AMG_E_ARG, "count_probe: bad arguments");
  for (int64_t i = 0; i < n; ++i) {
    long long id = ids[i];
    if (form == 1 && id != -1) id = (long long)((unsigned int)ids[i] & ~AMG_FLAG_MASK);
    if (form == 2 && id >= 0) {
      if (id >= n_slots) return amg_fail(AMG_E_ARG, "count_probe: slot %lld at %lld beyond the table", id, (long long)i);
      id = tab_ids[id];
    }
    if (id >= n_ids) return amg_fail(AMG_E_ARG, "count_probe: id %lld at %lld, n_ids %lld", id, (long long)i, (long long)n_ids);
  }
  HIPCHK(hipSetDevice(c->device));
  const size_t guard = 64;
  const size_t ids_words = guard + (size_t)n + 4 + guard, cnt_words = (size_t)n_ids + 1 + guard;
  const size_t tab_bytes = form == 2 ? ((size_t)n_slots + 1) * sizeof(Slot) : 0;
  const size_t ids_cap = (ids_words * 4 + 255) & ~(size_t)255, cnt_cap = (cnt_words * 4 + 255) & ~(size_t)255;
  char* d = nullptr;
  HIPCHK(hipMalloc(reinterpret_cast<void**>(&d), ids_cap + cnt_cap + tab_bytes));
  int* dbuf = reinterpret_cast<int*>(d);
  int* dids = dbuf + guard + misalign;
  unsigned int* dcnt = reinterpret_cast<unsigned int*>(d + ids_cap);
  Slot* dtab = form == 2 ? reinterpret_cast<Slot*>(d + ids_cap + cnt_cap) : nullptr;
  std::vector<unsigned int> back;
  int rc = AMG_OK;
  do {
    if (hipMemset(d, 0xff, ids_cap + cnt_cap) != hipSuccess) { rc = amg_fail(AMG_E_HIP, "count_probe: memset"); break; }
    if (n && hipMemcpy(dids, ids, (size_t)n * 4, hipMemcpyHostToDevice) != hipSuccess) { rc = amg_fail(AMG_E_HIP, "h2d"); break; }
    if (form == 2) {
      std::vector<Slot> tab((size_t)n_slots + 1);
      memset(tab.data(), 0xff, tab.size() * sizeof(Slot));
      for (int64_t i = 0; i < n_slots; ++i) tab[i].id = tab_ids[i];
      if (hipMemcpy(dtab, tab.data(), tab_bytes, hipMemcpyHostToDevice) != hipSuccess) { rc = amg_fail(AMG_E_HIP, "h2d"); break; }
    }
    if (hipDeviceSynchronize() != hipSuccess) { rc = amg_fail(AMG_E_HIP, "count_probe: sync"); break; }
    c->sw = read_build_switches();
    if (flags & 1) c->cnt_hint_reset = true;
    rc = count_ids(c, (CountKind)kind, form == 1 ? IdsClaimsMarked : IdsPlain, dids, n, n_ids, dcnt, dtab);
    if (rc != AMG_OK) break;
    if (flags & 2) {
      FetchList l;
      unsigned long long v[COUNT_LEARN_WORDS] = {0};
      if (count_learn_add(c, &l)) {
        if ((rc = fetch(c, l, v)) != AMG_OK) break;
        count_learn_take(c, v);
      }
    }
    if (hipStreamSynchronize(c->stream) != hipSuccess) { rc = amg_fail(AMG_E_HIP, "count_probe: stream"); break; }
    CountSweeps h;
    unsigned int lst[2];
    if (hipMemcpy(&h, &c->cnt_state.as<CountState>()->sweeps[kind], sizeof(h), hipMemcpyDeviceToHost) != hipSuccess ||
        hipMemcpy(lst, c->cnt_list.p, sizeof(lst), hipMemcpyDeviceToHost) != hipSuccess) {
      rc = amg_fail(AMG_E_HIP, "d2h");
      break;
    }
    back.resize(ids_words > cnt_words ? ids_words : cnt_words);
    bool intact = true;
    if (hipMemcpy(back.data(), dbuf, ids_words * 4, hipMemcpyDeviceToHost) != hipSuccess) { rc = amg_fail(AMG_E_HIP, "d2h"); break; }
    const size_t first = guard + (size_t)misalign;
    for (size_t i = 0; i < ids_words; ++i)
      if ((i < first || i >= first + (size_t)n) && back[i] != 0xffffffffu) intact = false;
    if (n) memcpy(ids, back.data() + first, (size_t)n * 4);
    if (hipMemcpy(back.data(), dcnt, cnt_words * 4, hipMemcpyDeviceToHost) != hipSuccess) { rc = amg_fail(AMG_E_HIP, "d2h"); break; }
    for (size_t i = (size_t)n_ids + 1; i < cnt_words; ++i)
      if (back[i] != 0xffffffffu) intact = false;
    memcpy(counts, back.data(), ((size_t)n_ids + 1) * 4);
    for (int q = 0; q < COUNT_MAX_SWEEPS; ++q) state[q] = (int64_t)h.beyond[q], state[4 + q] = (int64_t)h.done[q];
    state[8] = lst[0];
    state[9] = lst[1];
    state[10] = c->cnt_launched[0];
    state[11] = c->cnt_launched[1];
    state[12] = c->cnt_sweeps[kind];
    state[13] = intact ? 1 : 0;
  } while (false);
  (void)hipFree(d);
  return rc;
}
```

amira_amd/csrc/amg_derive.hip:

```cpp
#include "amg_device.h"

__device__ __forceinline__ long long dv_new_token(long long t, const long long* __restrict__ src,
                                                  const long long* __restrict__ read_off, long long n_reads, int k,
                                                  bool* ok) {
  long long lo = 0, hi = n_reads;
  while (lo < hi) {
    const long long mid = (lo + hi) >> 1;
    if (src[mid] <= t) lo = mid + 1; else hi = mid;
  }
  const long long i = lo - 1;
  if (i < 0) {
    *ok = false;
    return 0;
  }
  const long long q = t - src[i], len = read_off[i + 1] - read_off[i];
  if (q + k > len) *ok = false;
  return read_off[i] + q;
}

#define DV_READS 64
__device__ __forceinline__ long long dv_bcast(long long v, int lane) {
  const unsigned int lo = (unsigned int)__builtin_amdgcn_readlane((int)(unsigned int)(unsigned long long)v, lane);
  const unsigned int hi = (unsigned int)__builtin_amdgcn_readlane((int)(unsigned int)((unsigned long long)v >> 32), lane);
  return (long long)(((unsigned long long)hi << 32) | lo);
}
__global__ __launch_bounds__(256) void k_dv_windows(const long long* __restrict__ read_off, const long long* __restrict__ src,
                                                    long long n_reads, int k, const int* __restrict__ old_node,
                                                    const signed char* __restrict__ old_dir,
                                                    const long long* __restrict__ new_id, int* __restrict__ tok_node,
                                                    signed char* __restrict__ tok_dir, unsigned long long* bad) {
  const int lane = threadIdx.x & 63;
  const long long r0 = ((long long)blockIdx.x * 4 + (threadIdx.x >> 6)) * DV_READS;
  if (r0 >= n_reads) return;
  long long o = 0, s = 0;
  int n = 0;
  if (r0 + lane < n_reads) {
    o = read_off[r0 + lane];
    n = (int)(read_off[r0 + lane + 1] - o);
    s = src[r0 + lane];
  }
  for (int j0 = 0; j0 < DV_READS; j0 += 4) {
    long long oo[4], ss[4];
    int nn[4], most = 0;
#pragma unroll
    for (int j = 0; j < 4; ++j) {
      nn[j] = __builtin_amdgcn_readlane(n, j0 + j);
      oo[j] = dv_bcast(o, j0 + j);
      ss[j] = dv_bcast(s, j0 + j);
      most = nn[j] > most ? nn[j] : most;
    }
    for (int q = lane; q < most; q += 64) {
      int old[4];
      signed char d[4];
#pragma unroll
      for (int j = 0; j < 4; ++j) {
        old[j] = -1;
        d[j] = 0;
        if (q + k <= nn[j]) {
          old[j] = old_node[ss[j] + q];
          d[j] = old_dir[ss[j] + q];
        }
      }
#pragma unroll
      for (int j = 0; j < 4; ++j) {
        if (q >= nn[j]) continue;
        int v = -1;
        if (q + k <= nn[j]) {
          if (old[j] >= 0) v = (int)new_id[old[j]];
          else *bad = 1ull;
        }
        tok_node[oo[j] + q] = v;
        tok_dir[oo[j] + q] = v >= 0 ? d[j] : (signed char)0;
      }
    }
  }
}

__global__ void k_dv_nodes(const unsigned char* __restrict__ alive, const long long* __restrict__ new_id, long long n_old, int k,
                           const int* __restrict__ tok_in, const unsigned int* __restrict__ cov_in,
                           const long long* __restrict__ first_in, const long long* __restrict__ src,
                           const long long* __restrict__ read_off, long long n_reads, long long own_lo, long long own_hi,
                           int* __restrict__ tok_out, unsigned int* __restrict__ cov_out, long long* __restrict__ first_out,
                           unsigned char* __restrict__ alive_out, unsigned long long* bad) {
  long long n = (long long)blockIdx.x * blockDim.x + threadIdx.x;
  if (n >= n_old || !alive[n]) return;
  const long long i = new_id[n];
  for (int x = 0; x < k; ++x) tok_out[i * k + x] = tok_in[n * k + x];
  cov_out[i] = cov_in[n];
  alive_out[i] = 1;
  const long long f = first_in[n], tg = f >> 1;
  if (tg < own_lo || tg >= own_hi) {
    first_out[i] = 0;
    return;
  }
  bool ok = true;
  const long long t = dv_new_token(tg - own_lo, src, read_off, n_reads, k, &ok);
  if (!ok) *bad = 2ull;
  first_out[i] = (t << 1) | (f & 1ll);
}

__global__ void k_dv_pair_keep(const unsigned long long* __restrict__ pkey, long long n_pairs,
                               const unsigned char* __restrict__ alive, unsigned int* __restrict__ keep) {
  long long p = (long long)blockIdx.x * blockDim.x + threadIdx.x;
  if (p >= n_pairs) return;
  const unsigned long long key = pkey[p];
  const unsigned int lo = (unsigned int)((key >> 32) & 0x7fffffffull), hi = (unsigned int)(key & 0xffffffffull) - 1u;
  keep[p] = (alive[lo] && alive[hi]) ? 1u : 0u;
}

__global__ void k_dv_pairs(const unsigned long long* __restrict__ pkey, const unsigned long long* __restrict__ pfirst,
                           const unsigned int* __restrict__ pcnt, long long n_pairs, const unsigned int* __restrict__ keep,
                           const long long* __restrict__ pos, const long long* __restrict__ new_id,
                           const long long* __restrict__ src, const long long* __restrict__ read_off, long long n_reads, int k,
                           long long own_lo, long long own_hi,
                           unsigned long long* __restrict__ okey, unsigned long long* __restrict__ ofirst,
                           unsigned int* __restrict__ ocnt, unsigned long long* bad) {
  long long p = (long long)blockIdx.x * blockDim.x + threadIdx.x;
  if (p >= n_pairs || !keep[p]) return;
  const unsigned long long key = pkey[p], f = pfirst[p];
  const unsigned int lo = (unsigned int)((key >> 32) & 0x7fffffffull), hi = (unsigned int)(key & 0xffffffffull) - 1u;
  const unsigned long long nlo = (unsigned long long)new_id[lo], nhi = (unsigned long long)new_id[hi];
  const long long q = pos[p];
  okey[q] = (key & (1ull << 63)) | (nlo << 32) | (nhi + 1ull);
  ocnt[q] = pcnt[p];
  const long long tg = (long long)(f >> 3);
  if (tg < own_lo || tg >= own_hi) {
    ofirst[q] = 0ull;
    return;
  }
  bool ok = true;
  const long long t = dv_new_token(tg - own_lo, src, read_off, n_reads, k, &ok);
  if (!ok) *bad = 3ull;
  ofirst[q] = ((unsigned long long)t << 3) | (f & 7ull);
}

__global__ void k_dv_bounds(const long long* __restrict__ base, int world, const long long* __restrict__ node_first,
                            long long n_nodes, const long long* __restrict__ new_id, const unsigned long long* __restrict__ pfirst,
                            long long n_pairs, const long long* __restrict__ ppos, long long* __restrict__ bounds) {
  const int r = blockIdx.x * blockDim.x + threadIdx.x;
  if (r > world) return;
  {
    long long lo = 0, hi = n_nodes;
    const long long want = r == world ? 0x7fffffffffffffffll : (base[r] << 1);
    while (lo < hi) {
      const long long mid = (lo + hi) >> 1;
      if (node_first[mid] < want) lo = mid + 1; else hi = mid;
    }
    bounds[r] = new_id[lo];
  }
  {
    long long lo = 0, hi = n_pairs;
    const unsigned long long want = r == world ? ~0ull : ((unsigned long long)base[r] << 3);
    while (lo < hi) {
      const long long mid = (lo + hi) >> 1;
      if (pfirst[mid] < want) lo = mid + 1; else hi = mid;
    }
    bounds[world + 1 + r] = ppos[lo];
  }
}

int derive_local(amg_ctx* c, int k, long long own_lo, long long own_tokens, const long long* d_bases, int world,
                 long long* bounds_host, long long* D2_out, long long* P2_out, bool* ok) {
  *ok = false;
  hipStream_t st = c->stream;
  const long long D = c->n_nodes, P = c->n_pairs, R = c->n_reads, T = c->n_tokens;
  stage_begin(c, "derive");
  unsigned long long* bad = c->status.as<unsigned long long>() + ST_MISC;
  AMGCHK(c->s2.ensure((size_t)(D + 2) * sizeof(long long)));
  AMGCHK(c->s3.ensure((size_t)(P + 2) * sizeof(unsigned int)));
  AMGCHK(c->s4.ensure((size_t)(P + 2) * sizeof(long long)));
  long long* new_id = c->s2.as<long long>();
  unsigned int* keep = c->s3.as<unsigned int>();
  long long* ppos = c->s4.as<long long>();
  {
    ClearList cl;
    cl.add(c->status.p, ST_WORDS * sizeof(unsigned long long));
    cl.add(keep + P, sizeof(unsigned int));
    AMGCHK(clear_many(c, cl));
  }
  AMGCHK(prim_exscan_bytes_set(c, c->node_alive.as<unsigned char>(), new_id, (size_t)D));
  if (P > 0)
    hipLaunchKernelGGL(k_dv_pair_keep, dim3(nblk(P, 256)), dim3(256), 0, st, c->pair_key.as<unsigned long long>(), P,
                       c->node_alive.as<unsigned char>(), keep);
  AMGCHK(prim_exscan_u32_to_i64(c, keep, ppos, (size_t)P + 1));
  AMGCHK(c->alt_tok_node.ensure((size_t)(T + 8) * sizeof(int)));
  AMGCHK(c->alt_tok_dir.ensure((size_t)(T + 8)));
  if (R > 0)
    hipLaunchKernelGGL(k_dv_windows, dim3(nblk(R, 4 * DV_READS)), dim3(256), 0, st, c->read_off.as<long long>(),
                       c->rd_src.as<long long>(), R, k, c->tok_node.as<int>(), c->tok_dir.as<signed char>(), new_id,
                       c->alt_tok_node.as<int>(), c->alt_tok_dir.as<signed char>(), bad);
  long long* d_bounds = nullptr;
  if (d_bases) {
    AMGCHK(c->s1.ensure((size_t)(2 * (world + 1)) * sizeof(long long)));
    d_bounds = c->s1.as<long long>();
    hipLaunchKernelGGL(k_dv_bounds, dim3(nblk(world + 1, 64)), dim3(64), 0, st, d_bases, world, c->node_first.as<long long>(), D,
                       new_id, c->pair_first.as<unsigned long long>(), P, ppos, d_bounds);
  }
  unsigned long long v[2 + FETCH_MAX - 2];
  {
    FetchList l;
    l.add(new_id + D);
    l.add(ppos + P);
    if (d_bounds) l.add_words(d_bounds, 2 * (world + 1));
    if (l.overflow) return amg_fail(AMG_E_ARG, "derive: world too large");
    AMGCHK(fetch(c, l, v));
  }
  const long long D2 = (long long)v[0], P2 = (long long)v[1];
  if (bounds_host)
    for (int i = 0; i < 2 * (world + 1); ++i) bounds_host[i] = (long long)v[2 + i];
  AMGCHK(c->alt_ntok.ensure((size_t)(D2 * k + 1) * sizeof(int)));
  AMGCHK(c->alt_ncov.ensure((size_t)(D2 + 1) * sizeof(unsigned int)));
  AMGCHK(c->alt_nfirst.ensure((size_t)(D2 + 1) * sizeof(long long)));
  AMGCHK(c->alt_nalive.ensure((size_t)(D2 + 1)));
  AMGCHK(c->alt_pkey.ensure((size_t)(P2 + 2) * sizeof(unsigned long long)));
  AMGCHK(c->alt_pfirst.ensure((size_t)(P2 + 2) * sizeof(unsigned long long)));
  AMGCHK(c->alt_pcnt.ensure((size_t)(P2 + 2) * sizeof(unsigned int)));
  if (D > 0)
    hipLaunchKernelGGL(k_dv_nodes, dim3(nblk(D, 256)), dim3(256), 0, st, c->node_alive.as<unsigned char>(), new_id, D, k,
                       c->node_tokens.as<int>(), c->node_cov.as<unsigned int>(), c->node_first.as<long long>(),
                       c->rd_src.as<long long>(), c->read_off.as<long long>(), R, own_lo, own_lo + own_tokens,
                       c->alt_ntok.as<int>(), c->alt_ncov.as<unsigned int>(), c->alt_nfirst.as<long long>(),
                       c->alt_nalive.as<unsigned char>(), bad);
  if (P > 0)
    hipLaunchKernelGGL(k_dv_pairs, dim3(nblk(P, 256)), dim3(256), 0, st, c->pair_key.as<unsigned long long>(),
                       c->pair_first.as<unsigned long long>(), c->pair_cnt.as<unsigned int>(), P, keep, ppos, new_id,
                       c->rd_src.as<long long>(), c->read_off.as<long long>(), R, k, own_lo, own_lo + own_tokens,
                       c->alt_pkey.as<unsigned long long>(), c->alt_pfirst.as<unsigned long long>(),
                       c->alt_pcnt.as<unsigned int>(), bad);
  stage_end(c);
  AMGCHK(bs_read_stats(c, k));
  unsigned long long hs[ST_WORDS];
  AMGCHK(fetch_status(c, hs));
  if (hs[ST_MISC] || hs[ST_BADINPUT]) return AMG_OK;
  c->n_windows = (int64_t)hs[ST_N_WINDOWS];
  c->n_short = (int64_t)hs[ST_N_SHORT];
  *D2_out = D2;
  *P2_out = P2;
  *ok = true;
  return AMG_OK;
}

int derive_commit(amg_ctx* c, long long D2, long long P2) {
  std::swap(c->tok_node, c->alt_tok_node);
  std::swap(c->tok_dir, c->alt_tok_dir);
  std::swap(c->node_tokens, c->alt_ntok);
  std::swap(c->node_cov, c->alt_ncov);
  std::swap(c->node_first, c->alt_nfirst);
  std::swap(c->node_alive, c->alt_nalive);
  std::swap(c->pair_key, c->alt_pkey);
  std::swap(c->pair_first, c->alt_pfirst);
  std::swap(c->pair_cnt, c->alt_pcnt);
  AMGCHK(c->node_comp.ensure((size_t)(D2 + 1) * sizeof(int)));
  c->n_nodes = c->n_local_nodes = D2;
  c->n_pairs = c->n_local_pairs = P2;
  c->comp_from_claims = false;
  c->filtered_build = false;
  AMGCHK(bs_finish_from_pairs(c));
  c->built = true;
  c->derived = true;
  c->node_hint = D2 > 256 ? D2 : 256;
  return AMG_OK;
}

int derive_from_previous(amg_ctx* c, int k, bool* done) {
  *done = false;
  if (c->n_nodes <= 0 || c->n_reads <= 0 || c->n_tokens <= 0) return AMG_OK;
  long long D2 = 0, P2 = 0;
  bool ok = false;
  AMGCHK(derive_local(c, k, 0, 0x3fffffffffffffffll, nullptr, 1, nullptr, &D2, &P2, &ok));
  if (!ok) return AMG_OK;
  AMGCHK(derive_commit(c, D2, P2));
  *done = true;
  return AMG_OK;
}
```

amira_amd/csrc/amg_filter.hip:

```cpp
#include "amg_device.h"

__global__ void k_filter_nodes(const unsigned int* __restrict__ cov, unsigned char* __restrict__ alive,
                               long long n, unsigned int min_cov) {
  long long i = (long long)blockIdx.x * blockDim.x + threadIdx.x;
  if (i < n && alive[i] && cov[i] < min_cov) alive[i] = 0;
}

__global__ void k_filter_edges(const int* __restrict__ src, const int* __restrict__ tgt,
                               const unsigned int* __restrict__ cov,
                               const unsigned char* __restrict__ node_alive,
                               unsigned char* __restrict__ alive, long long n, unsigned int min_cov) {
  long long e = (long long)blockIdx.x * blockDim.x + threadIdx.x;
  if (e >= n || !alive[e]) return;
  if ((min_cov > 1 && cov[e] < min_cov) || !node_alive[src[e]] || !node_alive[tgt[e]]) alive[e] = 0;
}

#define READS_PER_WAVE 8
__global__ __launch_bounds__(256) void k_mask_reads(int* __restrict__ tok_node,
                                                    const long long* __restrict__ read_off,
                                                    long long n_reads,
                                                    const unsigned char* __restrict__ node_alive,
                                                    unsigned char* __restrict__ read_fix) {
  const long long rbase = ((long long)blockIdx.x * 4 + (threadIdx.x >> 6)) * READS_PER_WAVE;
  if (rbase >= n_reads) return;
  const int lane = threadIdx.x & 63;
  const long long off_l = (lane <= READS_PER_WAVE && rbase + lane <= n_reads) ? read_off[rbase + lane] : 0;
  long long a[READS_PER_WAVE], b[READS_PER_WAVE];
  int v[READS_PER_WAVE];
#pragma unroll
  for (int j = 0; j < READS_PER_WAVE; ++j) {
    a[j] = __shfl(off_l, j, 64);
    b[j] = rbase + j < n_reads ? __shfl(off_l, j + 1, 64) : a[j];
  }
#pragma unroll
  for (int j = 0; j < READS_PER_WAVE; ++j) v[j] = a[j] + lane < b[j] ? tok_node[a[j] + lane] : -1;
  bool dead[READS_PER_WAVE];
#pragma unroll
  for (int j = 0; j < READS_PER_WAVE; ++j) dead[j] = v[j] >= 0 && !node_alive[v[j]];
#pragma unroll
  for (int j = 0; j < READS_PER_WAVE; ++j) {
    if (dead[j]) tok_node[a[j] + lane] = -2;
    bool hit = dead[j];
    for (long long t = a[j] + 64 + lane; t < b[j]; t += 64) {
      const int n = tok_node[t];
      if (n >= 0 && !node_alive[n]) {
        tok_node[t] = -2;
        hit = true;
      }
    }
    if (__any(hit) && lane == 0) read_fix[rbase + j] = 1;
  }
}

static int apply_removals(amg_ctx* c, unsigned int min_edge_cov) {
  hipStream_t st = c->stream;
  if (c->ladj_valid && min_edge_cov <= 1 && !getenv("AMG_NO_LADJ_PATCH")) c->ladj_stale = true;
  else if (!c->ladj_stale || min_edge_cov > 1) c->ladj_stale = false;
  c->ladj_valid = false;
  c->pristine = false;
  if (min_edge_cov > 1) c->edge_own_deaths = true;
  c->match_valid = false;
  if (c->n_edges > 0)
    hipLaunchKernelGGL(k_filter_edges, dim3(nblk(c->n_edges, 256)), dim3(256), 0, st,
                       c->edge_src.as<int>(), c->edge_tgt.as<int>(), c->edge_cov.as<unsigned int>(),
                       c->node_alive.as<unsigned char>(), c->edge_alive.as<unsigned char>(),
                       c->n_edges, min_edge_cov);
  if (c->n_reads > 0)
    hipLaunchKernelGGL(k_mask_reads, dim3(nblk(c->n_reads, 4 * READS_PER_WAVE)), dim3(256), 0, st,
                       c->tok_node.as<int>(), c->read_off.as<long long>(), c->n_reads,
                       c->node_alive.as<unsigned char>(), c->read_fix.as<unsigned char>());
  return AMG_OK;
}

extern "C" int amg_filter(amg_ctx* c, uint32_t min_node_cov, uint32_t min_edge_cov) {
  NEED_BUILT(c);
  stages_reset(c);
  stage_begin(c, "filter");
  if (c->n_nodes > 0)
    hipLaunchKernelGGL(k_filter_nodes, dim3(nblk(c->n_nodes, 256)), dim3(256), 0, c->stream,
                       c->node_cov.as<unsigned int>(), c->node_alive.as<unsigned char>(),
                       c->n_nodes, min_node_cov);
  AMGCHK(apply_removals(c, min_edge_cov));
  stage_end(c);
  c->have_corrected = false;
  return AMG_OK;
}

__global__ void k_kill_listed(const int* __restrict__ ids, long long n, long long n_nodes,
                              unsigned char* __restrict__ alive) {
  long long i = (long long)blockIdx.x * blockDim.x + threadIdx.x;
  if (i >= n) return;
  int v = ids[i];
  if (v >= 0 && v < n_nodes) alive[v] = 0;
}

extern "C" int amg_remove_nodes(amg_ctx* c, const int32_t* node_ids, int64_t n) {
  NEED_BUILT(c);
  if (n < 0 || (n > 0 && !node_ids)) return amg_fail(AMG_E_ARG, "bad node list");
  if (n == 0) return AMG_OK;
  AMGCHK(c->s0.ensure((size_t)n * sizeof(int)));
  HIPCHK(hipMemcpyAsync(c->s0.p, node_ids, (size_t)n * sizeof(int), hipMemcpyHostToDevice, c->stream));
  hipLaunchKernelGGL(k_kill_listed, dim3(nblk(n, 256)), dim3(256), 0, c->stream, c->s0.as<int>(),
                     (long long)n, c->n_nodes, c->node_alive.as<unsigned char>());
  AMGCHK(apply_removals(c, 0));
  HIPCHK(hipStreamSynchronize(c->stream));
  c->have_corrected = false;
  return AMG_OK;
}



__global__ void k_live_keys(const unsigned char* __restrict__ e_alive, const int* __restrict__ e_src,
                            const signed char* __restrict__ e_sdir, const long long* __restrict__ pos,
                            long long n_edges, unsigned int* __restrict__ keys, unsigned int* __restrict__ vals) {
  long long e = (long long)blockIdx.x * blockDim.x + threadIdx.x;
  if (e >= n_edges || !e_alive[e]) return;
  const long long o = pos[e];
  keys[o] = 2u * (unsigned int)e_src[e] + (e_sdir[e] > 0 ? 0u : 1u);
  vals[o] = (unsigned int)e;
}

__global__ void k_lr_count(const unsigned int* __restrict__ keys, long long n_live, int4* __restrict__ lrows) {
  long long i = (long long)blockIdx.x * blockDim.x + threadIdx.x;
  if (i < n_live) atomicAdd(&lrows[keys[i]].y, 1);
}

#define LR_PER 8
__global__ __launch_bounds__(256) void k_lr_alloc(const unsigned int* __restrict__ keys, long long n_live,
                                                  int4* __restrict__ lrows, unsigned int* __restrict__ tick,
                                                  unsigned long long* pool) {
  __shared__ unsigned int s_wave[4];
  __shared__ unsigned long long s_base;
  const long long i0 = (long long)blockIdx.x * (256 * LR_PER) + threadIdx.x;
  unsigned int cnt[LR_PER], key[LR_PER], mine = 0;
#pragma unroll
  for (int j = 0; j < LR_PER; ++j) {
    const long long i = i0 + (long long)j * 256;
    cnt[j] = 0;
    key[j] = 0;
    if (i < n_live) {
      key[j] = keys[i];
      const unsigned int t = (unsigned int)atomicAdd(&lrows[key[j]].z, 1);
      tick[i] = t;
      if (t == 0) cnt[j] = (unsigned int)lrows[key[j]].y | 0x80000000u;
      mine += cnt[j] & 0x7fffffffu;
    }
  }
  unsigned int total;
  unsigned int off = block_exscan_256(mine, &total, s_wave);
  if (threadIdx.x == 0) s_base = total ? atomicAdd(pool, (unsigned long long)total) : 0ull;
  __syncthreads();
#pragma unroll
  for (int j = 0; j < LR_PER; ++j)
    if (cnt[j] & 0x80000000u) {
      lrows[key[j]].x = (int)(s_base + off);
      off += cnt[j] & 0x7fffffffu;
    }
}

#define LR_DONE 0xffffffffu
__global__ void k_lr_fill(const unsigned int* __restrict__ keys, const unsigned int* __restrict__ edge_of,
                          unsigned int* __restrict__ tick, long long n_live, int4* __restrict__ lrows,
                          const int* __restrict__ e_tgt, const signed char* __restrict__ e_tdir,
                          unsigned int* __restrict__ tmp, int2* __restrict__ lent) {
  long long i = (long long)blockIdx.x * blockDim.x + threadIdx.x;
  if (i >= n_live) return;
  const unsigned int key = keys[i], e = edge_of[i];
  const int4 rw = lrows[key];
  if (rw.y == 1) {
    const int t = e_tgt[e], d = (int)e_tdir[e];
    lent[rw.x] = make_int2(t, d);
    lrows[key] = make_int4(rw.x, 1, t, d);
    tick[i] = LR_DONE;
    return;
  }
  tmp[rw.x + tick[i]] = e;
}

__global__ __launch_bounds__(256) void k_lr_finish(const unsigned int* __restrict__ keys, const unsigned int* __restrict__ tick,
                                                   long long n_live, const unsigned int* __restrict__ tmp,
                                                   const int* __restrict__ e_tgt, const signed char* __restrict__ e_tdir,
                                                   int4* __restrict__ lrows, int2* __restrict__ lent,
                                                   unsigned int* __restrict__ long_rows, unsigned long long* n_long) {
  long long i = (long long)blockIdx.x * blockDim.x + threadIdx.x;
  bool mine = i < n_live && tick[i] == 0u;
  unsigned int key = 0;
  int off = 0, cnt = 0;
  if (mine) {
    key = keys[i];
    off = lrows[key].x;
    cnt = lrows[key].y;
    if (cnt > WAVE_ROW_MAX) {
      long_rows[atomicAdd(n_long, 1ull)] = key;
      mine = false;
    } else if (cnt == 2) {
      unsigned int a = tmp[off], b = tmp[off + 1];
      if (a > b) {
        const unsigned int t = a;
        a = b;
        b = t;
      }
      const int ta = e_tgt[a], da = (int)e_tdir[a];
      lent[off] = make_int2(ta, da);
      lent[off + 1] = make_int2(e_tgt[b], (int)e_tdir[b]);
      lrows[key] = make_int4(off, 2, ta, da);
      mine = false;
    }
  }
  wave_rows_in_order(mine, key, (long long)off, cnt, tmp, [&](unsigned int row, long long o, int n, int rank, unsigned int x) {
    const int t = e_tgt[x], d = (int)e_tdir[x];
    lent[o + rank] = make_int2(t, d);
    if (rank == 0) lrows[row] = make_int4((int)o, n, t, d);
  });
}

#define LR_HUB_BLOCKS 8
__global__ __launch_bounds__(256) void k_lr_long(const unsigned int* __restrict__ long_rows,
                                                 const unsigned long long* __restrict__ n_long,
                                                 const unsigned int* __restrict__ tmp, const int* __restrict__ e_tgt,
                                                 const signed char* __restrict__ e_tdir, int4* __restrict__ lrows,
                                                 int2* __restrict__ lent, unsigned int* hub_bits, long long hub_words) {
  __shared__ unsigned int s_wave[4];
  const unsigned long long n = *n_long;
  for (unsigned long long r = blockIdx.x; r < n; r += gridDim.x) {
    const unsigned int key = long_rows[r];
    const int off = lrows[key].x, cnt = lrows[key].y;
    __syncthreads();
    if (cnt > HUGE_ROW) continue;
    for (int j = threadIdx.x; j < cnt; j += 256) {
      const unsigned int x = tmp[off + j];
      int rank = 0;
      for (int q = 0; q < cnt; ++q) rank += tmp[off + q] < x ? 1 : 0;
      lent[off + rank] = make_int2(e_tgt[x], (int)e_tdir[x]);
      if (rank == 0) lrows[key] = make_int4(off, cnt, e_tgt[x], (int)e_tdir[x]);
    }
  }
  if (blockIdx.x >= LR_HUB_BLOCKS) return;
  for (unsigned long long r = blockIdx.x; r < n; r += LR_HUB_BLOCKS) {
    const unsigned int key = long_rows[r];
    const int off = lrows[key].x, cnt = lrows[key].y;
    if (cnt <= HUGE_ROW) continue;
    huge_row_in_order(tmp + off, (long long)cnt, hub_bits + (long long)blockIdx.x * hub_words, hub_words, s_wave,
                      [&](long long rank, unsigned int x) {
                        lent[off + rank] = make_int2(e_tgt[x], (int)e_tdir[x]);
                        if (rank == 0) lrows[key] = make_int4(off, cnt, e_tgt[x], (int)e_tdir[x]);
                      });
  }
}

__global__ void k_lr_patch(int4* __restrict__ lrows, int2* __restrict__ lent, long long n_rows,
                           const unsigned char* __restrict__ n_alive) {
  long long r = (long long)blockIdx.x * blockDim.x + threadIdx.x;
  if (r >= n_rows) return;
  const int4 rw = lrows[r];
  if (rw.y == 0) return;
  if (!n_alive[r >> 1]) {
    lrows[r] = make_int4(rw.x, 0, 0, 0);
    return;
  }
  if (rw.y == 1) {
    if (!n_alive[rw.z]) lrows[r] = make_int4(rw.x, 0, 0, 0);
    return;
  }
  int w = 0;
  int2 first = make_int2(0, 0);
  for (int j = 0; j < rw.y; ++j) {
    const int2 e = lent[rw.x + j];
    if (!n_alive[e.x]) continue;
    if (w != j) lent[rw.x + w] = e;
    if (w == 0) first = e;
    ++w;
  }
  if (w != rw.y) lrows[r] = make_int4(rw.x, w, first.x, first.y);
}

int ensure_live_adj(amg_ctx* c) {
  if (c->ladj_valid) return AMG_OK;
  hipStream_t st = c->stream;
  if (c->ladj_stale) {
    hipLaunchKernelGGL(k_lr_patch, dim3(nblk(2 * c->n_nodes, 256)), dim3(256), 0, st, c->ladj_rows.as<int4>(),
                       c->ladj.as<int2>(), 2 * c->n_nodes, c->node_alive.as<unsigned char>());
    c->ladj_stale = false;
    c->ladj_valid = true;
    return AMG_OK;
  }
  const long long rows = 2 * c->n_nodes, E = c->n_edges;
  AMGCHK(c->ladj_rows.ensure((size_t)(rows + 2) * sizeof(int4)));
  AMGCHK(c->ladj_pos.ensure((size_t)(E + 2) * sizeof(long long)));
  unsigned long long* ctr = c->status.as<unsigned long long>() + ST_COMPACT_A;
  {
    ClearList cl;
    cl.add(c->ladj_rows.p, (size_t)(rows + 2) * sizeof(int4));
    cl.add(ctr, 2 * sizeof(unsigned long long));
    AMGCHK(prim_exscan_bytes_set(c, c->edge_alive.as<unsigned char>(), c->ladj_pos.as<long long>(), (size_t)E, &cl));
  }
  long long total = 0;
  {
    FetchList l;
    l.add(c->ladj_pos.as<long long>() + E);
    AMGCHK(fetch(c, l, reinterpret_cast<unsigned long long*>(&total)));
  }
  AMGCHK(c->ladj.ensure((size_t)(total + 1) * sizeof(int2)));
  AMGCHK(c->ladj_keys.ensure(5 * (size_t)(total + 2) * sizeof(unsigned int)));
  unsigned int* keys = c->ladj_keys.as<unsigned int>();
  unsigned int* edge_of = keys + (total + 2);
  unsigned int* tick = edge_of + (total + 2);
  unsigned int* tmp = tick + (total + 2);
  unsigned int* long_rows = tmp + (total + 2);
  if (total > 0) {
    hipLaunchKernelGGL(k_live_keys, dim3(nblk(E, 256)), dim3(256), 0, st, c->edge_alive.as<unsigned char>(),
                       c->edge_src.as<int>(), c->edge_sdir.as<signed char>(), c->ladj_pos.as<long long>(), E, keys,
                       edge_of);
    hipLaunchKernelGGL(k_lr_count, dim3(nblk(total, 256)), dim3(256), 0, st, keys, total, c->ladj_rows.as<int4>());
    hipLaunchKernelGGL(k_lr_alloc, dim3(nblk(total, 256 * LR_PER)), dim3(256), 0, st, keys, total, c->ladj_rows.as<int4>(),
                       tick, ctr);
    hipLaunchKernelGGL(k_lr_fill, dim3(nblk(total, 256)), dim3(256), 0, st, keys, edge_of, tick, total,
                       c->ladj_rows.as<int4>(), c->edge_tgt.as<int>(), c->edge_tdir.as<signed char>(), tmp, c->ladj.as<int2>());
    hipLaunchKernelGGL(k_lr_finish, dim3(nblk(total, 256)), dim3(256), 0, st, keys, tick, total, tmp, c->edge_tgt.as<int>(),
                       c->edge_tdir.as<signed char>(), c->ladj_rows.as<int4>(), c->ladj.as<int2>(), long_rows, ctr + 1);
    const long long hub_words = (E + 31) / 32 + 1;
    AMGCHK(c->hub_bits.ensure((size_t)LR_HUB_BLOCKS * (size_t)hub_words * sizeof(unsigned int)));
    hipLaunchKernelGGL(k_lr_long, dim3(64), dim3(256), 0, st, long_rows, ctr + 1, tmp, c->edge_tgt.as<int>(),
                       c->edge_tdir.as<signed char>(), c->ladj_rows.as<int4>(), c->ladj.as<int2>(),
                       c->hub_bits.as<unsigned int>(), hub_words);
  }
  c->ladj_valid = true;
  return AMG_OK;
}

GView make_view(amg_ctx* c) {
  GView g;
  g.lent = c->ladj.as<int2>();
  g.lrows = c->ladj_rows.as<int4>();
  g.n_alive = c->node_alive.as<unsigned char>();
  g.n_cov = c->node_cov.as<unsigned int>();
  g.n_tok = c->node_tokens.as<int>();
  g.n_first = c->node_first.as<long long>();
  g.n_comp = c->node_comp.as<int>();
  g.k = c->k;
  g.flip = c->two_v - 1;
  return g;
}

__device__ __forceinline__ int node_degree(const GView& g, int n) {
  return g.lrows[2ll * n].y + g.lrows[2ll * n + 1].y;
}

__device__ __forceinline__ int lin_step(const GView& g, int n, bool use_forward, int* tgt, int* tdir) {
  const long long row = 2ll * n + (use_forward ? 0 : 1);
  const int4 rw = g.lrows[row];
  if (rw.y == 0 || (use_forward && rw.y != 1)) return 0;
  *tgt = rw.z;
  *tdir = rw.w;
  const int deg = node_degree(g, *tgt);
  return ((deg == 1 || deg == 2) && *tgt != n) ? 2 : 1;
}

extern "C" int amg_remove_edges(amg_ctx* c, const int32_t* edge_ids, int64_t n) {
  NEED_BUILT(c);
  if (n < 0 || (n > 0 && !edge_ids)) return amg_fail(AMG_E_ARG, "bad edge list");
  if (n == 0) return AMG_OK;
  AMGCHK(c->s0.ensure((size_t)n * sizeof(int)));
  HIPCHK(hipMemcpyAsync(c->s0.p, edge_ids, (size_t)n * sizeof(int), hipMemcpyHostToDevice, c->stream));
  hipLaunchKernelGGL(k_kill_listed, dim3(nblk(n, 256)), dim3(256), 0, c->stream, c->s0.as<int>(), (long long)n,
                     c->n_edges, c->edge_alive.as<unsigned char>());
  c->ladj_valid = false;
  c->pristine = false;
  c->edge_own_deaths = true;
  c->ladj_stale = false;
  c->match_valid = false;
  HIPCHK(hipStreamSynchronize(c->stream));
  c->have_corrected = false;
  return AMG_OK;
}

#define CLIP_MAX 64
__global__ void k_clip_mark(GView g, long long n_nodes, int min_length, const unsigned long long* __restrict__ acc,
                            const unsigned int* __restrict__ comp_live,
                            const unsigned char* __restrict__ protect,
                            unsigned char* __restrict__ kill) {
  long long i = (long long)blockIdx.x * blockDim.x + threadIdx.x;
  if (i >= n_nodes || !g.n_alive[i]) return;
  int n = (int)i;
  if (node_degree(g, n) != 1) return;
  int d0 = (g.n_first[n] & 1ll) ? -1 : 1;
  int path[CLIP_MAX];
  int len = 0;
  path[len++] = n;
  int tgt = -1, td = 0;
  int r = lin_step(g, n, d0 == -1, &tgt, &td);
  while (r == 2 && tgt != n) {
    if (len >= min_length) return;
    path[len++] = tgt;
    r = lin_step(g, tgt, td == 1, &tgt, &td);
  }
  r = lin_step(g, n, d0 == 1, &tgt, &td);
  while (r == 2 && tgt != n) {
    if (len >= min_length) return;
    path[len++] = tgt;
    r = lin_step(g, tgt, td == 1, &tgt, &td);
  }
  if (!(len > 0 && len < min_length)) return;
  const double thr = ((double)acc[0] / (double)acc[1]) * 1.5;
  bool all_high = true;
  for (int j = 0; j < len; ++j) all_high = all_high && ((double)g.n_cov[path[j]] > thr);
  if (all_high) return;
  if (comp_live) {
    int distinct = 0;
    for (int j = 0; j < len; ++j) {
      bool dup = false;
      for (int q = 0; q < j; ++q) dup = dup || (path[q] == path[j]);
      distinct += dup ? 0 : 1;
    }
    if ((unsigned int)distinct == comp_live[g.n_comp[n]]) return;
  } else {
    bool closed = true;
    for (int j = 0; j < len && closed; ++j)
      for (int side = 0; side < 2 && closed; ++side) {
        const int4 rw = g.lrows[2ll * path[j] + side];
        for (int q = 0; q < rw.y && closed; ++q) {
          const int t = q == 0 ? rw.z : g.lent[rw.x + q].x;
          bool in = false;
          for (int m = 0; m < len; ++m) in = in || (path[m] == t);
          closed = in;
        }
      }
    if (closed) return;
  }
  for (int j = 0; j < len; ++j)
    if (!protect || !protect[path[j]]) kill[path[j]] = 1;
}

__global__ void k_comp_hist(const int* __restrict__ comp, const unsigned char* __restrict__ alive,
                            const unsigned int* __restrict__ cov, long long n, unsigned int min_cov,
                            unsigned int* __restrict__ live_cnt, unsigned int* __restrict__ high_cnt,
                            unsigned long long* __restrict__ acc ) {
  int cid = -1;
  unsigned int n_live = 0, n_high = 0;
  unsigned long long s_cov = 0, s_n = 0;
  for (long long i = (long long)blockIdx.x * blockDim.x + threadIdx.x; i < n; i += (long long)gridDim.x * blockDim.x) {
    if (!alive[i]) continue;
    if (acc) {
      s_cov += cov[i];
      s_n += 1;
    }
    const int id = comp[i];
    if (id != cid) {
      if (cid >= 0) {
        atomicAdd(&live_cnt[cid], n_live);
        if (high_cnt && n_high) atomicAdd(&high_cnt[cid], n_high);
      }
      cid = id;
      n_live = n_high = 0;
    }
    ++n_live;
    n_high += (high_cnt && cov[i] >= min_cov) ? 1u : 0u;
  }
  const int lane = threadIdx.x & 63;
  if (acc) {
    __shared__ unsigned long long s_part[2][4];
    for (int d = 32; d > 0; d >>= 1) {
      s_cov += __shfl_xor(s_cov, d, 64);
      s_n += __shfl_xor(s_n, d, 64);
    }
    if (lane == 0) {
      s_part[0][threadIdx.x >> 6] = s_cov;
      s_part[1][threadIdx.x >> 6] = s_n;
    }
    __syncthreads();
    if (threadIdx.x == 0) {
      const unsigned long long n_all = s_part[1][0] + s_part[1][1] + s_part[1][2] + s_part[1][3];
      if (n_all) {
        atomicAdd(&acc[0], s_part[0][0] + s_part[0][1] + s_part[0][2] + s_part[0][3]);
        atomicAdd(&acc[1], n_all);
      }
    }
  }
  bool active = cid >= 0;
  unsigned long long todo = __ballot(active);
  while (todo) {
    const int leader = __ffsll((long long)todo) - 1;
    const int lc = __shfl(cid, leader, 64);
    const bool same = active && cid == lc;
    const unsigned long long m = __ballot(same);
    unsigned int sl = same ? n_live : 0u, sh = same ? n_high : 0u;
    for (int d = 32; d > 0; d >>= 1) {
      sl += __shfl_xor(sl, d, 64);
      sh += __shfl_xor(sh, d, 64);
    }
    if (lane == leader) {
      atomicAdd(&live_cnt[lc], sl);
      if (high_cnt && sh) atomicAdd(&high_cnt[lc], sh);
    }
    active = active && !same;
    todo &= ~m;
  }
}

__global__ __launch_bounds__(256) void k_cov_acc(const unsigned char* __restrict__ alive, const unsigned int* __restrict__ cov,
                                                 long long n, unsigned long long* __restrict__ acc) {
  __shared__ unsigned long long s_part[2][4];
  unsigned long long s_cov = 0, s_n = 0;
  for (long long i = (long long)blockIdx.x * blockDim.x + threadIdx.x; i < n; i += (long long)gridDim.x * blockDim.x)
    if (alive[i]) {
      s_cov += cov[i];
      s_n += 1;
    }
  for (int d = 32; d > 0; d >>= 1) {
    s_cov += __shfl_xor(s_cov, d, 64);
    s_n += __shfl_xor(s_n, d, 64);
  }
  if ((threadIdx.x & 63) == 0) {
    s_part[0][threadIdx.x >> 6] = s_cov;
    s_part[1][threadIdx.x >> 6] = s_n;
  }
  __syncthreads();
  if (threadIdx.x == 0) {
    const unsigned long long n_all = s_part[1][0] + s_part[1][1] + s_part[1][2] + s_part[1][3];
    if (n_all) {
      atomicAdd(&acc[0], s_part[0][0] + s_part[0][1] + s_part[0][2] + s_part[0][3]);
      atomicAdd(&acc[1], n_all);
    }
  }
}

__global__ void k_scatter_ids(const unsigned char* __restrict__ killed, const long long* __restrict__ pos,
                              long long n, int* __restrict__ out) {
  long long i = (long long)blockIdx.x * blockDim.x + threadIdx.x;
  if (i < n && killed[i]) out[pos[i]] = (int)i;
}

static int finish_kill(amg_ctx* c, int64_t* n_removed, int32_t* removed_ids) {
  hipStream_t st = c->stream;
  const long long D = c->n_nodes;
  AMGCHK(c->s2.ensure((size_t)(D + 2) * sizeof(long long)));
  AMGCHK(prim_exscan_apply_kill(c, c->s0.as<unsigned char>(), c->node_alive.as<unsigned char>(), c->s2.as<long long>(),
                                (size_t)D));
  long long total = 0;
  {
    FetchList l;
    l.add(c->s2.as<long long>() + D);
    AMGCHK(fetch(c, l, reinterpret_cast<unsigned long long*>(&total)));
  }
  if (n_removed) *n_removed = total;
  if (removed_ids && total > 0) {
    AMGCHK(c->s3.ensure((size_t)total * sizeof(int)));
    hipLaunchKernelGGL(k_scatter_ids, dim3(nblk(D, 256)), dim3(256), 0, st, c->s0.as<unsigned char>(),
                       c->s2.as<long long>(), D, c->s3.as<int>());
    HIPCHK(hipMemcpyAsync(removed_ids, c->s3.p, (size_t)total * sizeof(int), hipMemcpyDeviceToHost, st));
  }
  if (total > 0) AMGCHK(apply_removals(c, 0));
  if (removed_ids && total > 0) HIPCHK(hipStreamSynchronize(st));
  return AMG_OK;
}

extern "C" int amg_remove_short_linear_paths(amg_ctx* c, int32_t min_length, const uint8_t* protect,
                                             int64_t* n_removed, int32_t* removed_ids) {
  NEED_BUILT(c);
  if (min_length < 1 || min_length > CLIP_MAX)
    return amg_fail(AMG_E_ARG, "min_length must be in [1, %d]", CLIP_MAX);
  hipStream_t st = c->stream;
  const long long D = c->n_nodes;
  if (n_removed) *n_removed = 0;
  if (D == 0) return AMG_OK;
  stages_reset(c);
  const bool by_labels = !c->pristine || getenv("AMG_CLIP_COMPONENTS");
  if (by_labels) AMGCHK(ensure_components(c));
  stage_begin(c, "clip");
  unsigned long long* acc = c->status.as<unsigned long long>() + ST_COV_SUM;
  AMGCHK(c->s0.ensure((size_t)D + 8));
  if (by_labels) AMGCHK(c->s4.ensure((size_t)(c->n_components + 2) * sizeof(unsigned int)));
  {
    ClearList cl;
    cl.add(acc, 2 * sizeof(unsigned long long));
    cl.add(c->s0.p, (size_t)D + 8);
    if (by_labels) cl.add(c->s4.p, (size_t)(c->n_components + 2) * sizeof(unsigned int));
    AMGCHK(clear_many(c, cl));
  }
  if (by_labels)
    hipLaunchKernelGGL(k_comp_hist, dim3(nblk(D, 256) < 256u ? nblk(D, 256) : 256u), dim3(256), 0, st, c->node_comp.as<int>(),
                       c->node_alive.as<unsigned char>(), c->node_cov.as<unsigned int>(), D, 0u,
                       c->s4.as<unsigned int>(), (unsigned int*)nullptr, acc);
  else
    hipLaunchKernelGGL(k_cov_acc, dim3(nblk(D, 2048) < 256u ? nblk(D, 2048) : 256u), dim3(256), 0, st,
                       c->node_alive.as<unsigned char>(), c->node_cov.as<unsigned int>(), D, acc);
  unsigned char* d_protect = nullptr;
  if (protect) {
    AMGCHK(c->s5.ensure((size_t)D + 8));
    HIPCHK(hipMemcpyAsync(c->s5.p, protect, (size_t)D, hipMemcpyHostToDevice, st));
    d_protect = c->s5.as<unsigned char>();
  }
  AMGCHK(ensure_live_adj(c));
  hipLaunchKernelGGL(k_clip_mark, dim3(nblk(D, 128)), dim3(128), 0, st, make_view(c), D, (int)min_length,
                     acc, by_labels ? c->s4.as<unsigned int>() : (const unsigned int*)nullptr, d_protect,
                     c->s0.as<unsigned char>());
  int r = finish_kill(c, n_removed, removed_ids);
  stage_end(c);
  c->have_corrected = false;
  return r;
}

__global__ void k_kill_low_components(const int* __restrict__ comp, const unsigned char* __restrict__ alive,
                                      const unsigned int* __restrict__ high_cnt, long long n,
                                      unsigned char* __restrict__ kill) {
  long long i = (long long)blockIdx.x * blockDim.x + threadIdx.x;
  if (i < n && alive[i] && high_cnt[comp[i]] == 0) kill[i] = 1;
}

extern "C" int amg_remove_low_coverage_components(amg_ctx* c, uint32_t min_cov) {
  NEED_BUILT(c);
  hipStream_t st = c->stream;
  const long long D = c->n_nodes;
  if (D == 0) return AMG_OK;
  AMGCHK(ensure_components(c));
  size_t nc = (size_t)(c->n_components + 2);
  AMGCHK(c->s0.ensure((size_t)D + 8));
  AMGCHK(c->s4.ensure(2 * nc * sizeof(unsigned int)));
  {
    ClearList cl;
    cl.add(c->s0.p, (size_t)D + 8);
    cl.add(c->s4.p, 2 * nc * sizeof(unsigned int));
    AMGCHK(clear_many(c, cl));
  }
  unsigned int* live = c->s4.as<unsigned int>();
  unsigned int* high = live + nc;
  hipLaunchKernelGGL(k_comp_hist, dim3(nblk(D, 256) < 256u ? nblk(D, 256) : 256u), dim3(256), 0, st, c->node_comp.as<int>(),
                     c->node_alive.as<unsigned char>(), c->node_cov.as<unsigned int>(), D, min_cov, live, high,
                     (unsigned long long*)nullptr);
  hipLaunchKernelGGL(k_kill_low_components, dim3(nblk(D, 256)), dim3(256), 0, st, c->node_comp.as<int>(),
                     c->node_alive.as<unsigned char>(), high, D, c->s0.as<unsigned char>());
  c->have_corrected = false;
  return finish_kill(c, nullptr, nullptr);
}
```

amira_amd/csrc/amg_internal.h:

```cpp
#pragma once
#include <cstdint>
#include <cstdio>
#include <cstring>
#include <string>
#include <vector>

#include <hip/hip_runtime.h>

#include "../../include/amg.h"

extern thread_local std::string g_amg_err;
int amg_fail(int code, const char* fmt, ...);

#define HIPCHK(call)                                                                   \
  do {                                                                                 \
    hipError_t e_ = (call);                                                            \
    if (e_ != hipSuccess)                                                              \
      return amg_fail(AMG_E_HIP, "%s:%d %s -> %s", __FILE__, __LINE__, #call,          \
                      hipGetErrorString(e_));                                          \
  } while (0)
#define AMGCHK(call)                 \
  do {                               \
    int r_ = (call);                 \
    if (r_ != AMG_OK) return r_;     \
  } while (0)

struct DevBuf {
  void* p = nullptr;
  size_t cap = 0;
  void* own_p = nullptr;
  size_t own_cap = 0;
  bool borrowed = false;
  void borrow(const void* ptr, size_t bytes) {
    if (!borrowed) {
      own_p = p;
      own_cap = cap;
    }
    p = const_cast<void*>(ptr);
    cap = bytes;
    borrowed = true;
  }
  void unborrow() {
    if (!borrowed) return;
    p = own_p;
    cap = own_cap;
    own_p = nullptr;
    own_cap = 0;
    borrowed = false;
  }
  int ensure(size_t bytes) {
    unborrow();
    if (bytes <= cap) return AMG_OK;
    if (p) (void)hipFree(p);
    p = nullptr;
    cap = 0;
    size_t want = bytes + bytes / 8 + 256;
    hipError_t e = hipMalloc(&p, want);
    if (e != hipSuccess) {
      p = nullptr;
      return amg_fail(AMG_E_NOMEM, "hipMalloc(%zu) failed: %s", want, hipGetErrorString(e));
    }
    cap = want;
    return AMG_OK;
  }
  void release() {
    unborrow();
    if (p) (void)hipFree(p);
    p = nullptr;
    cap = 0;
  }
  template <class T>
  T* as() const {
    return reinterpret_cast<T*>(p);
  }
};

struct __attribute__((aligned(32))) Slot {
  unsigned long long key;
  unsigned long long first_inv;
  unsigned int count;
  int id;
  unsigned long long pad;
};
static_assert(sizeof(Slot) == 32, "slot must be one 32-byte sector");

enum {
  ST_NODE_INSERTS = 0,
  ST_PAIR_INSERTS = 1,
  ST_OVERFLOW = 2,
  ST_PALINDROME = 3,
  ST_COLLISION = 4,
  ST_N_WINDOWS = 5,
  ST_N_SHORT = 6,
  ST_COMPACT_A = 7,
  ST_COMPACT_B = 8,
  ST_MISC = 9,
  ST_BADINPUT = 10,
  ST_COV_SUM = 11,
  ST_WORDS = 16
};

struct StageTime {
  const char* name;
  hipEvent_t a, b;
  float ms;
};

static const uint64_t kAmgSeed0 = 0x9E3779B97F4A7C15ull;
static const unsigned int kProbeLimit = 1024;

struct BuildSwitches {
  bool head_tiles_set = false;
  long long head_tiles = 0;
  int claim_shards = -1;
  bool tight_bits = false;
  bool key_fp = false;
  bool node_buckets = true;
  bool generic_k = false;
  bool rank_sort = false;
  int edge_lone = -1;
  bool edge_home = true;
  bool no_derive = false;
  int weak_fp = 0;
  bool count_inline = false;
  int count_list_seg = 1 << 30;
  bool count_debug = false;
};
BuildSwitches read_build_switches();

enum Overflow { OV_NONE = 0, OV_NODE_TABLE = 1, OV_EDGE_TABLE = 2, OV_COLLISION = 3 };
static inline int overflowed(Overflow* which, Overflow cause) { return *which = cause, AMG_E_OVERFLOW; }

struct DistState;
struct BubbleState;

struct amg_ctx {
  int device = 0;
  hipStream_t stream = nullptr;

  DevBuf tokens;
  DevBuf read_off;
  DevBuf gene_start;
  DevBuf gene_end;
  DevBuf read_len;
  bool have_pos = false, have_read_len = false;
  DevBuf pos_off, c_pos_off;
  DevBuf pos1_s, pos1_e;
  bool pos_identity = true;
  int64_t pos_n0 = 0, pos1_used = 0, c_pos1_used = 0;
  int64_t n_reads = 0, n_tokens = 0;
  int32_t two_v = 0;

  bool built = false;
  int32_t k = 0;
  uint64_t seed = kAmgSeed0;
  int64_t n_windows = 0, n_short = 0;
  int64_t n_nodes = 0, n_pairs = 0, n_edges = 0, n_components = 0;
  int64_t node_slots = 0, edge_slots = 0, retries = 0;
  int64_t node_hint = 0;
  int64_t c_node_bound = 0;
  int c_node_bound_k = 0;
  int64_t hint_bound = 0;
  int hint_bound_k = 0;
  bool filtered_build = false;
  int64_t n_local_nodes = 0, n_local_pairs = 0;
  int64_t tok_base = 0;
  int64_t tok_total = 0;

  DevBuf node_tab;
  DevBuf edge_tab;
  DevBuf tok_slot;
  DevBuf tok_node;
  DevBuf tok_dir;
  DevBuf tok_pair;
  bool packed_nodes = false;
  int weak_fp_builds = 0;
  bool dist_mode = false;
  bool count_inline = false;
  DevBuf node_tokens;
  DevBuf node_cov;
  DevBuf node_first;
  DevBuf node_comp;
  DevBuf node_alive;
  DevBuf edge_src, edge_tgt;
  DevBuf edge_sdir, edge_tdir;
  DevBuf edge_cov;
  DevBuf edge_alive;
  DevBuf pair_key, pair_first;
  DevBuf pair_cnt;
  DevBuf adj_off;
  DevBuf adj_edge;
  DevBuf ladj_off;
  DevBuf ladj;
  DevBuf ladj_rows;
  DevBuf ladj_pos, ladj_keys;
  DevBuf hub_bits;
  bool ladj_valid = false;
  bool ladj_stale = false;
  bool comp_valid = false, adj_valid = false;
  bool pristine = false;
  DevBuf read_fix;

  bool have_corrected = false;
  bool pos0_own = false;
  int64_t c_reads = 0, c_tokens = 0;
  DevBuf c_tokens_buf, c_read_off, c_orig, c_changed, c_gstart, c_gend, c_read_len;

  DevBuf c_src, rd_src;
  bool c_derivable = false;
  bool derive_ready = false;
  bool derived = false;
  bool dist_candidate = false;
  bool edge_own_deaths = false;
  DevBuf alt_tok_node, alt_tok_dir, alt_ntok, alt_ncov, alt_nfirst, alt_nalive, alt_pkey, alt_pfirst, alt_pcnt;

  bool exact_keys = false;
  int x_bits = 0;
  bool x_fp = false;
  bool x_two = false;
  int x_kbits = 0;
  int64_t x_nspace = 0, x_espace = 0;
  int64_t x_max_claims = 0, x_max_eclaims = 0;
  bool dist_x = false;
  DevBuf x_first, x_slot;
  DevBuf x_final;
  DevBuf x_efirst, x_eslot;
  DevBuf x_ecnt;
  DevBuf x_ncnt;
  int64_t rank_flags_clean = 0;
  DevBuf x_ftag;
  DevBuf f_ctrs;
  DevBuf x_efinal;
  DevBuf x_first_all;
  bool comp_from_claims = false;

  int world = 1;
  uint32_t dist_min_node = 1, dist_min_edge = 1;
  DistState* dist = nullptr;
  BubbleState* bub = nullptr;

  bool match_valid = false;
  int64_t match_total = 0, match_npat = 0;
  DevBuf match_read, match_pos, match_off, match_wave;

  DevBuf status;
  unsigned long long* mail_host = nullptr;
  unsigned long long* mail_dev = nullptr;
  unsigned long long mail_ticket = 0;
  DevBuf sort_tmp;
  DevBuf scan_state;
  unsigned long long scan_tickets = 0;
  unsigned int scan_epoch = 0;
  DevBuf s0, s1, s2, s3, s4, s5;
  DevBuf nw_big;
  DevBuf gap_rec;
  DevBuf gm_mask;
  DevBuf gm_tab;
  DevBuf gm_res;
  DevBuf gm_list;
  DevBuf gm_q;
  DevBuf gm_pool;
  DevBuf gm_gene;
  DevBuf gm_fail;
  DevBuf gm_ctr;
  DevBuf nw_rec;
  DevBuf routes_dev;
  bool have_routes = false;
  int64_t routes[AMG_ROUTE_WORDS] = {0};
  DevBuf bnd_bits;
  DevBuf cnt_state;
  bool cnt_hint_reset = false;
  DevBuf cnt_list;
  int cnt_sweeps[2] = {4, 4};
  int cnt_launched[2] = {0, 0};

  BuildSwitches sw;
  std::vector<StageTime> stages;
  bool timing = true;
};

int prim_sort_u64_u32(amg_ctx* c, const unsigned long long* kin, unsigned long long* kout,
                      const unsigned int* vin, unsigned int* vout, size_t n, int end_bit);
int prim_sort_u32_u32(amg_ctx* c, const unsigned int* kin, unsigned int* kout,
                      const unsigned int* vin, unsigned int* vout, size_t n, int end_bit);
struct ClearList;
int prim_exscan_i64(amg_ctx* c, const long long* in, long long* out, size_t n);
int prim_exscan_u32_to_i64(amg_ctx* c, const unsigned int* in, long long* out, size_t n);
int prim_exscan_u32_pair(amg_ctx* c, const unsigned int* in_a, long long* out_a, const unsigned int* in_b, long long* out_b,
                         size_t n);
int prim_exscan_i64_pair(amg_ctx* c, const long long* in_a, long long* out_a, const long long* in_b, long long* out_b,
                         size_t n);
int prim_exscan_bytes_set(amg_ctx* c, const unsigned char* in, long long* out, size_t n, const ClearList* side = nullptr);
int prim_exscan_apply_kill(amg_ctx* c, unsigned char* kill, unsigned char* alive, long long* out, size_t n);
int prim_exscan_keep_and_len(amg_ctx* c, const unsigned int* len, long long* out_keep, long long* out_off, size_t n);
int prim_exscan_flag_words(amg_ctx* c, const unsigned char* flags, unsigned int* bits, long long* out, size_t n_words);
int prim_exscan_bits_popc(amg_ctx* c, const unsigned int* bits, long long* out, size_t n_words);
int prim_exscan_pair_width(amg_ctx* c, const unsigned long long* pkey, long long* out, size_t n_pairs);
int prim_exscan_emit_edges(amg_ctx* c, const unsigned long long* pkey, const unsigned int* pcnt,
                           const unsigned long long* pfirst, size_t n_pairs, long long* total, int* e_src, int* e_tgt,
                           signed char* e_sdir, signed char* e_tdir, unsigned int* e_cov, unsigned char* e_alive,
                           const ClearList* side);

#define CLEAR_MAX 8
struct ClearList {
  void* p[CLEAR_MAX];
  unsigned long long bytes[CLEAR_MAX];
  int n = 0;
  bool overflow = false;
  unsigned int fill[CLEAR_MAX];
  void add(void* ptr, size_t b, unsigned int value = 0u) {
    if (b == 0) return;
    if (n >= CLEAR_MAX) {
      overflow = true;
      return;
    }
    p[n] = ptr;
    bytes[n] = (unsigned long long)((b + 3) & ~(size_t)3);
    fill[n] = value;
    ++n;
  }
};
int clear_many(amg_ctx* c, const ClearList& l);

#define FETCH_MAX 96
struct FetchList {
  const unsigned long long* p[FETCH_MAX];
  int n = 0;
  bool overflow = false;
  void add(const void* q) {
    if (n < FETCH_MAX)
      p[n++] = static_cast<const unsigned long long*>(q);
    else
      overflow = true;
  }
  void add_words(const void* q, int words) { for (int i = 0; i < words; ++i) add(static_cast<const unsigned long long*>(q) + i); }
};
int fetch(amg_ctx* c, const FetchList& l, unsigned long long* out, const ClearList* filler = nullptr);
static_assert(ST_WORDS <= FETCH_MAX, "fetch_status reads the status words in one list");
int fetch_status(amg_ctx* c, unsigned long long* out , const ClearList* filler = nullptr);
int stream_wait(amg_ctx* c);

void stage_begin(amg_ctx* c, const char* name);
void stage_end(amg_ctx* c);
void stages_reset(amg_ctx* c);

struct GView {
  const int2* lent;
  const int4* lrows;
  const unsigned char* n_alive;
  const unsigned int* n_cov;
  const int* n_tok;
  const long long* n_first;
  const int* n_comp;
  int k, flip;
};
int ensure_live_adj(amg_ctx* c);
GView make_view(amg_ctx* c);
void bubbles_release(amg_ctx* c);

void dist_release(amg_ctx* c);
int derive_from_previous(amg_ctx* c, int k, bool* done);
int derive_local(amg_ctx* c, int k, long long own_lo, long long own_tokens, const long long* d_bases, int world,
                 long long* bounds_host, long long* D2_out, long long* P2_out, bool* ok);
int derive_commit(amg_ctx* c, long long D2, long long P2);

uint64_t pow2_at_least(uint64_t x);
uint64_t slots_for(uint64_t n_keys);
void bs_size_tables(amg_ctx* c);
int grow_after_overflow(amg_ctx* c, Overflow cause);
int bs_read_stats(amg_ctx* c, int k, const ClearList* also = nullptr);
int bs_alloc_nodes(amg_ctx* c, long long D);
int bs_alloc_pairs(amg_ctx* c, long long P);
int bs_finish_from_pairs(amg_ctx* c);
int bs_nodes_pass(amg_ctx* c, int k, Overflow* which);
int bs_nodes_rank_local(amg_ctx* c);
int bs_edges_pass(amg_ctx* c, Overflow* which);
int bs_pairs_from_local(amg_ctx* c);
int ensure_components(amg_ctx* c);
int ensure_adjacency(amg_ctx* c);
enum CountKind { CountNodes = 0, CountEdgeClasses = 1 };
enum CountIds {
  IdsPlain,
  IdsClaimsMarked,
};
int count_ids(amg_ctx* c, CountKind what, CountIds form, int* ids, long long n, long long n_ids, unsigned int* out,
              const Slot* gather_tab = nullptr);
#define COUNT_LEARN_WORDS 8
bool count_learn_add(amg_ctx* c, FetchList* l);
void count_learn_take(amg_ctx* c, const unsigned long long* done );
bool bx_applicable(const amg_ctx* c, int k);
bool bx_fits(const amg_ctx* c, int k);
bool bx_tuple_fits(const amg_ctx* c, int k);
int bx_nodes(amg_ctx* c, int k, Overflow* which);
int bx_nodes_upsert(amg_ctx* c, int k, Overflow* which, bool sharded = false, bool rank_follows = true);
int bx_nodes_rank(amg_ctx* c);
int bx_edges(amg_ctx* c, Overflow* which, unsigned int min_edge_cov = 0);
int bx_nodes_filtered(amg_ctx* c, int k, unsigned int min_cov, Overflow* which);
int bx_flag_dead_reads(amg_ctx* c);
int bx_edges_upsert(amg_ctx* c, Overflow* which, bool lone = false, bool sharded = false, bool rank_follows = true);
int bx_edges_rank(amg_ctx* c, unsigned int min_edge_cov = 0, bool nodes_counted = false);
int bx_node_count(amg_ctx* c, bool tag);
int bx_bits(const amg_ctx* c, int k);
int bx_pairs_rank(amg_ctx* c, const int* final_of_claim, int* efinal);
int bx_components_from_claims(amg_ctx* c);
int bs_count_by_slot(amg_ctx* c, CountKind what, const int* slots, int* ids_scratch, long long n, Slot* tab,
                     const unsigned int* slot_sorted, long long n_ids, unsigned int* out);

#define NEED_BUILT(c)                                                     \
  do {                                                                    \
    if (!(c)) return amg_fail(AMG_E_ARG, "null ctx");                     \
    if (!(c)->built) return amg_fail(AMG_E_STATE, "amg_build first");     \
    HIPCHK(hipSetDevice((c)->device));                                    \
  } while (0)

static inline unsigned int nblk(long long n, int per) {
  long long b = (n + per - 1) / per;
  return (unsigned int)(b < 1 ? 1 : b);
}

static inline int ilog2_ceil(uint64_t x) {
  int b = 0;
  while ((1ull << b) < x && b < 63) ++b;
  return b;
}
```

Baseline: 10.04 billion gene-mers/s.

## Defer edge and component counts to device-resident late words to drop host syncs

Edge count after build and component count after union-find are no longer fetched to the host right away. They stay in a device 'late' buffer that kernels read through a pointer and launch over an upper bound. The values ride along on the next fetch, or are settled by a stream wait when a host consumer needs them. The dead-kept tally moves out of the pack kernel into its own kernel. This removes several blocking device-to-host round trips per pipeline stage, at the cost of oversized grids and more complex state tracking.

```diff
diff --git a/amira_amd/csrc/amg_adjacency.hip b/amira_amd/csrc/amg_adjacency.hip
--- a/amira_amd/csrc/amg_adjacency.hip
+++ b/amira_amd/csrc/amg_adjacency.hip
@@ -23,17 +23,18 @@
   return 2u * (unsigned int)e_src[e] + (e_sdir[e] > 0 ? 0u : 1u);
 }
 
-__global__ void k_adjc_ticket(const int* __restrict__ e_src, const signed char* __restrict__ e_sdir, long long n_edges,
-                              unsigned int* __restrict__ cnt, unsigned int* __restrict__ tick) {
+__global__ void k_adjc_ticket(const int* __restrict__ e_src, const signed char* __restrict__ e_sdir,
+                              const long long* __restrict__ n_edges, unsigned int* __restrict__ cnt,
+                              unsigned int* __restrict__ tick) {
   long long e = (long long)blockIdx.x * blockDim.x + threadIdx.x;
-  if (e < n_edges) tick[e] = atomicAdd(&cnt[adj_row_of(e_src, e_sdir, e)], 1u);
-}
-
-__global__ void k_adjc_fill(const int* __restrict__ e_src, const signed char* __restrict__ e_sdir, long long n_edges,
-                            const long long* __restrict__ off, const unsigned int* __restrict__ tick,
-                            unsigned int* __restrict__ tmp) {
+  if (e < *n_edges) tick[e] = atomicAdd(&cnt[adj_row_of(e_src, e_sdir, e)], 1u);
+}
+
+__global__ void k_adjc_fill(const int* __restrict__ e_src, const signed char* __restrict__ e_sdir,
+                            const long long* __restrict__ n_edges, const long long* __restrict__ off,
+                            const unsigned int* __restrict__ tick, unsigned int* __restrict__ tmp) {
   long long e = (long long)blockIdx.x * blockDim.x + threadIdx.x;
-  if (e < n_edges) tmp[off[adj_row_of(e_src, e_sdir, e)] + tick[e]] = (unsigned int)e;
+  if (e < *n_edges) tmp[off[adj_row_of(e_src, e_sdir, e)] + tick[e]] = (unsigned int)e;
 }
 
 __global__ __launch_bounds__(256) void k_adjc_rows(const long long* __restrict__ off, long long n_rows,
@@ -145,8 +146,9 @@
 }
 
 __global__ void k_uf_label(const int* __restrict__ root, const long long* __restrict__ root_rank,
-                           long long n, int* __restrict__ comp) {
-  long long i = (long long)blockIdx.x * blockDim.x + threadIdx.x;
+                           long long n, int* __restrict__ comp, long long* __restrict__ n_comp) {
+  long long i = (long long)blockIdx.x * blockDim.x + threadIdx.x;
+  if (i == 0) *n_comp = root_rank[n];
   if (i >= n) return;
   int r = root[i];
   while (root[r] != r) r = root[r];
@@ -165,7 +167,6 @@
   AMGCHK(c->s2.ensure((size_t)(D + 2) * sizeof(unsigned int) + (size_t)(D + 2) * sizeof(int)));
   unsigned int* is_root = c->s2.as<unsigned int>();
   int* root_copy = reinterpret_cast<int*>(is_root + (D + 2));
-  long long ncomp = 0;
   if (D > 0) {
     if (P > 0) {
       AMGCHK(c->s3.ensure((size_t)(D + 2) * sizeof(unsigned int)));
@@ -189,13 +190,11 @@
     hipLaunchKernelGGL(k_uf_roots, dim3(nblk(D, 256)), dim3(256), 0, st, parent, D, is_root, root_copy);
     AMGCHK(prim_exscan_u32_to_i64(c, is_root, c->s1.as<long long>(), (size_t)D + 1));
     hipLaunchKernelGGL(k_uf_label, dim3(nblk(D, 256)), dim3(256), 0, st, root_copy,
-                       c->s1.as<long long>(), D, parent);
-    FetchList l;
-    l.add(c->s1.as<long long>() + D);
-    AMGCHK(fetch(c, l, reinterpret_cast<unsigned long long*>(&ncomp)));
+                       c->s1.as<long long>(), D, parent, const_cast<long long*>(late_word(c, LATE_N_COMPONENTS)));
   }
   stage_end(c);
-  c->n_components = ncomp;
+  c->n_components = 0;
+  c->late_pending[LATE_N_COMPONENTS] = D > 0;
   c->comp_valid = true;
   return AMG_OK;
 }
@@ -203,15 +202,19 @@
 int ensure_adjacency(amg_ctx* c) {
   if (c->adj_valid) return AMG_OK;
   hipStream_t st = c->stream;
-  const long long D = c->n_nodes, E = c->n_edges;
+  const char* force_sort = getenv("AMG_ADJ_SORT");
+  const bool force = force_sort && force_sort[0] == '1';
+  if (c->edge_bound > (4ll << 20) || force) AMGCHK(late_settle(c));
+  const long long D = c->n_nodes, E = c->edge_bound;
+  const bool sorted = E > (4ll << 20) || force;
+  const long long* n_edges = late_word(c, LATE_N_EDGES);
   stage_begin(c, "adjacency");
   AMGCHK(c->adj_off.ensure((size_t)(2 * D + 2) * sizeof(long long)));
   AMGCHK(c->adj_edge.ensure((size_t)(E + 2) * sizeof(int)));
   AMGCHK(c->s1.ensure((size_t)(E + 2) * sizeof(unsigned int)));
   AMGCHK(c->s2.ensure((size_t)(E + 2) * sizeof(unsigned int)));
   AMGCHK(c->s3.ensure((size_t)(E + 2) * sizeof(unsigned int)));
-  const char* force_sort = getenv("AMG_ADJ_SORT");
-  if (E > 0 && E <= (4ll << 20) && !(force_sort && force_sort[0] == '1')) {
+  if (E > 0 && !sorted) {
     AMGCHK(c->s1.ensure((size_t)(2 * D + 2 > E + 2 ? 2 * D + 2 : E + 2) * sizeof(unsigned int)));
     unsigned int* cnt = c->s1.as<unsigned int>();
     unsigned int* tick = c->s2.as<unsigned int>();
@@ -226,10 +229,10 @@
       AMGCHK(clear_many(c, cl));
     }
     hipLaunchKernelGGL(k_adjc_ticket, dim3(nblk(E, 256)), dim3(256), 0, st, c->edge_src.as<int>(),
-                       c->edge_sdir.as<signed char>(), E, cnt, tick);
+                       c->edge_sdir.as<signed char>(), n_edges, cnt, tick);
     AMGCHK(prim_exscan_u32_to_i64(c, cnt, c->adj_off.as<long long>(), (size_t)(2 * D + 1)));
     hipLaunchKernelGGL(k_adjc_fill, dim3(nblk(E, 256)), dim3(256), 0, st, c->edge_src.as<int>(),
-                       c->edge_sdir.as<signed char>(), E, c->adj_off.as<long long>(), tick, tmp);
+                       c->edge_sdir.as<signed char>(), n_edges, c->adj_off.as<long long>(), tick, tmp);
     hipLaunchKernelGGL(k_adjc_rows, dim3(nblk(2 * D, 256)), dim3(256), 0, st, c->adj_off.as<long long>(), 2 * D, tmp,
                        c->adj_edge.as<int>(), long_rows, n_long);
     const long long hub_words = (E + 31) / 32 + 1;
diff --git a/amira_amd/csrc/amg_api.hip b/amira_amd/csrc/amg_api.hip
--- a/amira_amd/csrc/amg_api.hip
+++ b/amira_amd/csrc/amg_api.hip
@@ -74,14 +74,60 @@
   }
 }
 
-int fetch(amg_ctx* c, const FetchList& l, unsigned long long* out, const ClearList* filler) {
-  if (l.overflow) return amg_fail(AMG_E_ARG, "fetch: more than %d words in one list", FETCH_MAX);
+struct LateRide {
+  int at = -1;
+  int word[LATE_WORDS] = {0};
+  int n = 0;
+  int learn_at = -1;
+};
+static LateRide late_ride(amg_ctx* c, FetchList* l) {
+  LateRide r;
+  int want = 0;
+  for (int w = 0; w < LATE_WORDS; ++w) want += c->late_pending[w] ? 1 : 0;
+  if (want == 0 && !c->late_learn) return r;
+  if (l->n + want + COUNT_LEARN_WORDS > FETCH_MAX) return r;
+  r.at = l->n;
+  for (int w = 0; w < LATE_WORDS; ++w)
+    if (c->late_pending[w]) {
+      l->add(late_word(c, (LateWord)w));
+      r.word[r.n++] = w;
+    }
+  if (c->late_learn) {
+    if (count_learn_add(c, l)) r.learn_at = r.at + r.n;
+    c->late_learn = false;
+  }
+  return r;
+}
+static void late_take(amg_ctx* c, const LateRide& r, const unsigned long long* v) {
+  if (r.at < 0) return;
+  for (int i = 0; i < r.n; ++i) {
+    const long long x = (long long)v[r.at + i];
+    if (r.word[i] == LATE_N_EDGES) c->n_edges = c->edge_bound = x;
+    else c->n_components = x;
+    c->late_pending[r.word[i]] = false;
+  }
+  if (r.learn_at >= 0) count_learn_take(c, v + r.learn_at);
+}
+
+int late_settle(amg_ctx* c) {
+  bool any = c->late_learn;
+  for (int w = 0; w < LATE_WORDS; ++w) any = any || c->late_pending[w];
+  return any ? stream_wait(c) : AMG_OK;
+}
+
+int fetch(amg_ctx* c, const FetchList& asked, unsigned long long* out, const ClearList* filler) {
+  if (asked.overflow) return amg_fail(AMG_E_ARG, "fetch: more than %d words in one list", FETCH_MAX);
+  FetchList l = asked;
+  const LateRide ride = late_ride(c, &l);
+  unsigned long long all[FETCH_MAX];
   const bool plain = getenv("AMG_PLAIN_SYNC") != nullptr;
   if (plain) {
     for (int i = 0; i < l.n; ++i)
-      HIPCHK(hipMemcpyAsync(out + i, l.p[i], sizeof(unsigned long long), hipMemcpyDeviceToHost, c->stream));
+      HIPCHK(hipMemcpyAsync(all + i, l.p[i], sizeof(unsigned long long), hipMemcpyDeviceToHost, c->stream));
     if (filler) AMGCHK(clear_many(c, *filler));
     HIPCHK(hipStreamSynchronize(c->stream));
+    for (int i = 0; i < asked.n; ++i) out[i] = all[i];
+    late_take(c, ride, all);
     return AMG_OK;
   }
   if (!c->mail_host) {
@@ -109,7 +155,9 @@
       }
     }
   }
-  for (int i = 0; i < l.n; ++i) out[i] = m[2 * i];
+  for (int i = 0; i < l.n; ++i) all[i] = m[2 * i];
+  for (int i = 0; i < asked.n; ++i) out[i] = all[i];
+  late_take(c, ride, all);
   return AMG_OK;
 }
 
@@ -155,6 +203,7 @@
     return amg_fail(AMG_E_HIP, "hipStreamCreate: %s", hipGetErrorString(e));
   }
   int r = c->status.ensure(ST_WORDS * sizeof(unsigned long long));
+  if (r == AMG_OK) r = c->late.ensure(LATE_WORDS * sizeof(unsigned long long));
   if (r != AMG_OK) {
     delete c;
     return r;
@@ -178,7 +227,7 @@
                    &c->edge_src,  &c->edge_tgt,  &c->edge_sdir,  &c->edge_tdir, &c->edge_cov,
                    &c->edge_alive, &c->adj_off,  &c->adj_edge,   &c->read_fix, &c->ladj_off, &c->ladj, &c->ladj_rows, &c->ladj_pos, &c->ladj_keys, &c->hub_bits, &c->pair_key, &c->pair_first, &c->pair_cnt, &c->match_read, &c->match_pos, &c->match_off, &c->match_wave,  &c->c_tokens_buf,
                    &c->c_read_off, &c->c_orig,   &c->c_changed,  &c->c_gstart,  &c->c_gend,
-                   &c->c_read_len, &c->status,   &c->sort_tmp, &c->scan_state,   &c->s0, &c->s1, &c->s2, &c->s3,
+                   &c->c_read_len, &c->status, &c->late, &c->sort_tmp, &c->scan_state,   &c->s0, &c->s1, &c->s2, &c->s3,
                    &c->s4, &c->s5, &c->cnt_state, &c->cnt_list, &c->bnd_bits, &c->nw_rec, &c->gap_rec, &c->gm_mask, &c->gm_tab, &c->gm_res, &c->gm_list, &c->gm_q, &c->gm_pool, &c->gm_gene, &c->gm_fail, &c->gm_ctr, &c->routes_dev, &c->nw_big, &c->x_first, &c->x_slot, &c->x_final, &c->x_efirst, &c->x_eslot, &c->x_ecnt, &c->x_ncnt, &c->x_ftag, &c->f_ctrs, &c->x_efinal, &c->x_first_all, &c->pos_off, &c->c_pos_off, &c->pos1_s, &c->pos1_e,
                    &c->c_src, &c->rd_src, &c->alt_tok_node, &c->alt_tok_dir, &c->alt_ntok, &c->alt_ncov, &c->alt_nfirst,
                    &c->alt_nalive, &c->alt_pkey, &c->alt_pfirst, &c->alt_pcnt};
@@ -309,6 +358,8 @@
 extern "C" int amg_graph_sizes(amg_ctx* c, int64_t* n_nodes, int64_t* n_edges, int32_t* k) {
   if (!c) return amg_fail(AMG_E_ARG, "null ctx");
   if (!c->built) return amg_fail(AMG_E_STATE, "amg_build first");
+  HIPCHK(hipSetDevice(c->device));
+  AMGCHK(late_settle(c));
   if (n_nodes) *n_nodes = c->n_nodes;
   if (n_edges) *n_edges = c->n_edges;
   if (k) *k = c->k;
@@ -323,13 +374,14 @@
   o->two_v = c->two_v;
   if (!c->built) return AMG_OK;
   HIPCHK(hipSetDevice(c->device));
+  AMGCHK(ensure_components(c));
+  AMGCHK(late_settle(c));
   o->k = c->k;
   o->n_windows = c->n_windows;
   o->n_short_reads = c->n_short;
   o->n_nodes = c->n_nodes;
   o->n_edges = c->n_edges;
   o->n_pairs = c->n_pairs;
-  AMGCHK(ensure_components(c));
   o->n_components = c->n_components;
   o->node_table_slots = c->node_slots;
   o->edge_table_slots = c->edge_slots;
@@ -383,6 +435,7 @@
 extern "C" int amg_get_edges(amg_ctx* c, int32_t* src, int32_t* tgt, int8_t* sdir, int8_t* tdir,
                              uint32_t* coverage, uint8_t* alive) {
   NEED_BUILT(c);
+  AMGCHK(late_settle(c));
   const size_t E = (size_t)c->n_edges;
   AMGCHK(d2h(c, src, c->edge_src, E * sizeof(int32_t)));
   AMGCHK(d2h(c, tgt, c->edge_tgt, E * sizeof(int32_t)));
@@ -439,6 +492,7 @@
 extern "C" int amg_get_node_adj(amg_ctx* c, int64_t* offsets, int32_t* edge_ids) {
   NEED_BUILT(c);
   AMGCHK(ensure_adjacency(c));
+  AMGCHK(late_settle(c));
   AMGCHK(d2h(c, offsets, c->adj_off, (size_t)(2 * c->n_nodes + 1) * sizeof(int64_t)));
   AMGCHK(d2h(c, edge_ids, c->adj_edge, (size_t)c->n_edges * sizeof(int32_t)));
   HIPCHK(hipStreamSynchronize(c->stream));
diff --git a/amira_amd/csrc/amg_build.hip b/amira_amd/csrc/amg_build.hip
--- a/amira_amd/csrc/amg_build.hip
+++ b/amira_amd/csrc/amg_build.hip
@@ -47,8 +47,6 @@
 int bs_finish_from_pairs(amg_ctx* c) {
   const long long P = c->n_pairs, R = c->n_reads;
   stage_begin(c, "edge_emit");
-  AMGCHK(c->s5.ensure((size_t)(P + 2) * sizeof(long long)));
-  long long* base = c->s5.as<long long>();
   const long long cap = 2 * P;
   AMGCHK(c->edge_src.ensure((size_t)(cap + 2) * sizeof(int)));
   AMGCHK(c->edge_tgt.ensure((size_t)(cap + 2) * sizeof(int)));
@@ -57,29 +55,26 @@
   AMGCHK(c->edge_cov.ensure((size_t)(cap + 2) * sizeof(unsigned int)));
   AMGCHK(c->edge_alive.ensure((size_t)(cap + 2)));
   AMGCHK(c->read_fix.ensure((size_t)R + 1));
-  long long total = 0;
+  long long* total = const_cast<long long*>(late_word(c, LATE_N_EDGES));
   {
     ClearList cl;
     cl.add(c->read_fix.p, (size_t)R + 1);
     if (P > 0) {
       AMGCHK(prim_exscan_emit_edges(c, c->pair_key.as<unsigned long long>(), c->pair_cnt.as<unsigned int>(),
-                                    c->pair_first.as<unsigned long long>(), (size_t)P, base + P, c->edge_src.as<int>(),
+                                    c->pair_first.as<unsigned long long>(), (size_t)P, total, c->edge_src.as<int>(),
                                     c->edge_tgt.as<int>(), c->edge_sdir.as<signed char>(), c->edge_tdir.as<signed char>(),
                                     c->edge_cov.as<unsigned int>(), c->edge_alive.as<unsigned char>(), &cl));
     } else {
+      cl.add(total, sizeof(long long));
       AMGCHK(clear_many(c, cl));
     }
   }
-  {
-    FetchList l;
-    l.add(P > 0 ? static_cast<const void*>(base + P) : c->status.p);
-    const bool learn = count_learn_add(c, &l);
-    unsigned long long v[1 + COUNT_LEARN_WORDS] = {0};
-    AMGCHK(fetch(c, l, v));
-    if (P > 0) total = (long long)v[0];
-    if (learn) count_learn_take(c, v + 1);
-  }
-  c->n_edges = total;
+  c->n_edges = 0;
+  c->edge_bound = cap;
+  c->late_pending[LATE_N_EDGES] = P > 0;
+  c->late_pending[LATE_N_COMPONENTS] = false;
+  c->late_learn = true;
+  c->edges_intact = true;
   stage_end(c);
   c->ladj_valid = false;
   c->ladj_stale = false;
@@ -98,8 +93,7 @@
   stages_reset(c);
   AMGCHK(ensure_components(c));
   AMGCHK(ensure_adjacency(c));
-  HIPCHK(hipStreamSynchronize(c->stream));
-  return AMG_OK;
+  return stream_wait(c);
 }
 
 uint64_t slots_for(uint64_t n) {
diff --git a/amira_amd/csrc/amg_correct.h b/amira_amd/csrc/amg_correct.h
--- a/amira_amd/csrc/amg_correct.h
+++ b/amira_amd/csrc/amg_correct.h
@@ -157,7 +157,6 @@
   long long* o_posoff;
   long long* o_rl;
   long long out_reads, out_tokens;
-  unsigned long long* dead_kept;
 };
 
 struct CorrSwitches {
@@ -197,6 +196,7 @@
   bool carry = false;
   long long out_reads = 0, out_tokens = 0, big_total = 0, pos_total = 0;
   unsigned long long n_general = 0;
+  unsigned long long dead_kept = 0, alive_nodes = 0;
   long long n_queries = 0;
   int pool_retries = 0;
   bool lean_ran = false, fast_ran = false, memo = false;
diff --git a/amira_amd/csrc/amg_correct.hip b/amira_amd/csrc/amg_correct.hip
--- a/amira_amd/csrc/amg_correct.hip
+++ b/amira_amd/csrc/amg_correct.hip
@@ -19,6 +19,19 @@
     atomicAdd(out, (unsigned long long)s_part[0] + s_part[1] + s_part[2] + s_part[3]);
 }
 
+__global__ __launch_bounds__(256) void k_corr_dead_kept(CorrArgs a, const unsigned char* __restrict__ final_cls,
+                                                        unsigned long long* dead_kept) {
+  const long long r = (long long)blockIdx.x * blockDim.x + threadIdx.x;
+  unsigned int dead = 0;
+  if (r < a.n_reads && final_cls[r] == RC_KEEP_ORIG && a.new_len[r] > 0) {
+    const long long nw = a.read_off[r + 1] - a.read_off[r] - a.k + 1;
+    dead = nw <= 64 ? (unsigned int)(nw - __popcll(a.lmask[r])) : (unsigned int)nw;
+  }
+  if (__ballot(dead != 0u) == 0ull) return;
+  for (int d = 32; d > 0; d >>= 1) dead += (unsigned int)__shfl_xor((int)dead, d, 64);
+  if ((threadIdx.x & 63) == 0) atomicAdd(dead_kept + 16 * (blockIdx.x & 15), (unsigned long long)dead);
+}
+
 __global__ __launch_bounds__(256) void k_corr_pack(PackArgs A) {
   const CorrArgs& a = A.a;
   const int lane = threadIdx.x & 63;
@@ -26,15 +39,10 @@
   if (blockIdx.x == 0 && threadIdx.x == 0) A.o_off[A.out_reads] = A.out_tokens;
   long long dst = 0, src = 0;
   int n = 0;
-  unsigned int dead = 0;
   if (r < a.n_reads && a.new_len[r] > 0) {
     dst = A.new_off[r];
     n = (int)a.new_len[r];
     const unsigned char fc = A.final_cls[r];
-    if (fc == RC_KEEP_ORIG) {
-      const long long nw = a.read_off[r + 1] - a.read_off[r] - a.k + 1;
-      dead = nw <= 64 ? (unsigned int)(nw - __popcll(a.lmask[r])) : (unsigned int)nw;
-    }
     long long poff = 0;
     if (fc == RC_GAPPED) {
       src = a.tmp_off[r] | (1ll << 62);
@@ -51,10 +59,6 @@
     A.o_src[q] = fc == RC_GAPPED ? -1ll : src;
     if (a.have_pos) A.o_posoff[q] = poff;
     if (a.read_len) A.o_rl[q] = a.read_len[r];
-  }
-  if (__ballot(dead != 0u) != 0ull) {
-    for (int d = 32; d > 0; d >>= 1) dead += (unsigned int)__shfl_xor((int)dead, d, 64);
-    if (lane == 0) atomicAdd(A.dead_kept + 16 * (blockIdx.x & 15), (unsigned long long)dead);
   }
   if (__ballot(n > 0) == 0ull) return;
   for (int j0 = 0; j0 < PACK_READS; j0 += 4) {
@@ -204,6 +208,8 @@
 
 static int corr_shape(amg_ctx* c, const CorrSwitches& sw, CorrScratch& S, const CorrArgs& a, CorrCounts& n) {
   const long long R = c->n_reads;
+  if (R > 0)
+    hipLaunchKernelGGL(k_corr_dead_kept, dim3(nblk(R, 256)), dim3(256), 0, c->stream, a, S.final_cls, S.dead_kept);
   AMGCHK(prim_exscan_keep_and_len(c, S.new_len, S.new_idx, S.new_off, (size_t)R));
   FetchList shape;
   shape.add(S.new_idx + R);
@@ -212,8 +218,13 @@
     AMGCHK(plan_positions(c, S, n.n_gapped));
     AMGCHK(corr_nw_sizes(c, sw, S, a, n.n_gapped, shape));
   }
-  unsigned long long v[5] = {0, 0, 0, 0, 0};
+  const int bound_at = shape.n;
+  for (int i = 0; i < 16; ++i) shape.add(S.dead_kept + 16 * i);
+  shape.add(S.dead_kept + 256);
+  unsigned long long v[5 + 17] = {0};
   AMGCHK(fetch(c, shape, v));
+  for (int i = 0; i < 16; ++i) n.dead_kept += v[bound_at + i];
+  n.alive_nodes = v[bound_at + 16];
   n.out_reads = (long long)v[0];
   n.out_tokens = (long long)v[1];
   n.big_total = (long long)v[2];
@@ -249,7 +260,6 @@
   Pk.o_rl = c->have_read_len ? c->c_read_len.as<long long>() : nullptr;
   Pk.out_reads = n.out_reads;
   Pk.out_tokens = n.out_tokens;
-  Pk.dead_kept = S.dead_kept;
   if (c->n_reads > 0)
     hipLaunchKernelGGL(k_corr_pack, dim3(nblk(c->n_reads, 4 * PACK_READS)), dim3(256), 0, c->stream, Pk);
   else
@@ -258,21 +268,13 @@
   return AMG_OK;
 }
 
-static int corr_node_bound(amg_ctx* c, const CorrSwitches& sw, const CorrScratch& S, const CorrCounts& n) {
-  FetchList l;
-  for (int i = 0; i < 16; ++i) l.add(S.dead_kept + 16 * i);
-  l.add(S.dead_kept + 256);
-  unsigned long long v[17];
-  AMGCHK(fetch(c, l, v));
-  unsigned long long bound = S.count_alive ? v[16] : (unsigned long long)c->n_nodes;
-  unsigned long long dead_kept = 0;
-  for (int i = 0; i < 16; ++i) dead_kept += v[i];
-  bound += dead_kept;
-  c->c_derivable = n.n_gapped == 0 && dead_kept == 0 && !c->edge_own_deaths;
+static void corr_node_bound(amg_ctx* c, const CorrSwitches& sw, const CorrScratch& S, const CorrCounts& n) {
+  unsigned long long bound = S.count_alive ? n.alive_nodes : (unsigned long long)c->n_nodes;
+  bound += n.dead_kept;
+  c->c_derivable = n.n_gapped == 0 && n.dead_kept == 0 && !c->edge_own_deaths;
   c->c_node_bound = (int64_t)bound;
   if (sw.node_bound) c->c_node_bound = atoll(sw.node_bound);
   c->c_node_bound_k = c->k;
-  return AMG_OK;
 }
 
 extern "C" int amg_correct_reads(amg_ctx* c, int64_t* n_out_reads, int64_t* n_out_tokens) {
@@ -319,7 +321,7 @@
 
   stage_begin(c, "correct_pack");
   AMGCHK(corr_pack(c, S, a, n));
-  AMGCHK(corr_node_bound(c, sw, S, n));
+  corr_node_bound(c, sw, S, n);
   stage_end(c);
   if (sw.routes) AMGCHK(routes_end(c, n));
   c->c_reads = n.out_reads;
diff --git a/amira_amd/csrc/amg_count.hip b/amira_amd/csrc/amg_count.hip
--- a/amira_amd/csrc/amg_count.hip
+++ b/amira_amd/csrc/amg_count.hip
@@ -143,6 +143,7 @@
 int count_ids(amg_ctx* c, CountKind what, CountIds form, int* ids, long long n, long long n_ids, unsigned int* out,
               const Slot* gather_tab) {
   hipStream_t st = c->stream;
+  if (c->late_learn) AMGCHK(late_settle(c));
   const bool marked = form == IdsClaimsMarked;
   ClearList cl;
   cl.add(out, (size_t)(n_ids + 1) * sizeof(unsigned int), marked ? 1u : 0u);
diff --git a/amira_amd/csrc/amg_derive.hip b/amira_amd/csrc/amg_derive.hip
--- a/amira_amd/csrc/amg_derive.hip
+++ b/amira_amd/csrc/amg_derive.hip
@@ -196,25 +196,13 @@
     hipLaunchKernelGGL(k_dv_bounds, dim3(nblk(world + 1, 64)), dim3(64), 0, st, d_bases, world, c->node_first.as<long long>(), D,
                        new_id, c->pair_first.as<unsigned long long>(), P, ppos, d_bounds);
   }
-  unsigned long long v[2 + FETCH_MAX - 2];
-  {
-    FetchList l;
-    l.add(new_id + D);
-    l.add(ppos + P);
-    if (d_bounds) l.add_words(d_bounds, 2 * (world + 1));
-    if (l.overflow) return amg_fail(AMG_E_ARG, "derive: world too large");
-    AMGCHK(fetch(c, l, v));
-  }
-  const long long D2 = (long long)v[0], P2 = (long long)v[1];
-  if (bounds_host)
-    for (int i = 0; i < 2 * (world + 1); ++i) bounds_host[i] = (long long)v[2 + i];
-  AMGCHK(c->alt_ntok.ensure((size_t)(D2 * k + 1) * sizeof(int)));
-  AMGCHK(c->alt_ncov.ensure((size_t)(D2 + 1) * sizeof(unsigned int)));
-  AMGCHK(c->alt_nfirst.ensure((size_t)(D2 + 1) * sizeof(long long)));
-  AMGCHK(c->alt_nalive.ensure((size_t)(D2 + 1)));
-  AMGCHK(c->alt_pkey.ensure((size_t)(P2 + 2) * sizeof(unsigned long long)));
-  AMGCHK(c->alt_pfirst.ensure((size_t)(P2 + 2) * sizeof(unsigned long long)));
-  AMGCHK(c->alt_pcnt.ensure((size_t)(P2 + 2) * sizeof(unsigned int)));
+  AMGCHK(c->alt_ntok.ensure((size_t)(D * k + 1) * sizeof(int)));
+  AMGCHK(c->alt_ncov.ensure((size_t)(D + 1) * sizeof(unsigned int)));
+  AMGCHK(c->alt_nfirst.ensure((size_t)(D + 1) * sizeof(long long)));
+  AMGCHK(c->alt_nalive.ensure((size_t)(D + 1)));
+  AMGCHK(c->alt_pkey.ensure((size_t)(P + 2) * sizeof(unsigned long long)));
+  AMGCHK(c->alt_pfirst.ensure((size_t)(P + 2) * sizeof(unsigned long long)));
+  AMGCHK(c->alt_pcnt.ensure((size_t)(P + 2) * sizeof(unsigned int)));
   if (D > 0)
     hipLaunchKernelGGL(k_dv_nodes, dim3(nblk(D, 256)), dim3(256), 0, st, c->node_alive.as<unsigned char>(), new_id, D, k,
                        c->node_tokens.as<int>(), c->node_cov.as<unsigned int>(), c->node_first.as<long long>(),
@@ -229,8 +217,18 @@
                        c->alt_pcnt.as<unsigned int>(), bad);
   stage_end(c);
   AMGCHK(bs_read_stats(c, k));
-  unsigned long long hs[ST_WORDS];
-  AMGCHK(fetch_status(c, hs));
+  unsigned long long v[FETCH_MAX];
+  FetchList l;
+  l.add_words(c->status.p, ST_WORDS);
+  l.add(new_id + D);
+  l.add(ppos + P);
+  if (d_bounds) l.add_words(d_bounds, 2 * (world + 1));
+  if (l.overflow) return amg_fail(AMG_E_ARG, "derive: world too large");
+  AMGCHK(fetch(c, l, v));
+  const unsigned long long* hs = v;
+  const long long D2 = (long long)v[ST_WORDS], P2 = (long long)v[ST_WORDS + 1];
+  if (bounds_host)
+    for (int i = 0; i < 2 * (world + 1); ++i) bounds_host[i] = (long long)v[ST_WORDS + 2 + i];
   if (hs[ST_MISC] || hs[ST_BADINPUT]) return AMG_OK;
   c->n_windows = (int64_t)hs[ST_N_WINDOWS];
   c->n_short = (int64_t)hs[ST_N_SHORT];
diff --git a/amira_amd/csrc/amg_filter.hip b/amira_amd/csrc/amg_filter.hip
--- a/amira_amd/csrc/amg_filter.hip
+++ b/amira_amd/csrc/amg_filter.hip
@@ -9,9 +9,10 @@
 __global__ void k_filter_edges(const int* __restrict__ src, const int* __restrict__ tgt,
                                const unsigned int* __restrict__ cov,
                                const unsigned char* __restrict__ node_alive,
-                               unsigned char* __restrict__ alive, long long n, unsigned int min_cov) {
+                               unsigned char* __restrict__ alive, const long long* __restrict__ n_edges,
+                               unsigned int min_cov) {
   long long e = (long long)blockIdx.x * blockDim.x + threadIdx.x;
-  if (e >= n || !alive[e]) return;
+  if (e >= *n_edges || !alive[e]) return;
   if ((min_cov > 1 && cov[e] < min_cov) || !node_alive[src[e]] || !node_alive[tgt[e]]) alive[e] = 0;
 }
 
@@ -60,11 +61,12 @@
   c->pristine = false;
   if (min_edge_cov > 1) c->edge_own_deaths = true;
   c->match_valid = false;
-  if (c->n_edges > 0)
-    hipLaunchKernelGGL(k_filter_edges, dim3(nblk(c->n_edges, 256)), dim3(256), 0, st,
+  c->edges_intact = false;
+  if (c->edge_bound > 0)
+    hipLaunchKernelGGL(k_filter_edges, dim3(nblk(c->edge_bound, 256)), dim3(256), 0, st,
                        c->edge_src.as<int>(), c->edge_tgt.as<int>(), c->edge_cov.as<unsigned int>(),
                        c->node_alive.as<unsigned char>(), c->edge_alive.as<unsigned char>(),
-                       c->n_edges, min_edge_cov);
+                       late_word(c, LATE_N_EDGES), min_edge_cov);
   if (c->n_reads > 0)
     hipLaunchKernelGGL(k_mask_reads, dim3(nblk(c->n_reads, 4 * READS_PER_WAVE)), dim3(256), 0, st,
                        c->tok_node.as<int>(), c->read_off.as<long long>(), c->n_reads,
@@ -112,25 +114,29 @@
 
 __global__ void k_live_keys(const unsigned char* __restrict__ e_alive, const int* __restrict__ e_src,
                             const signed char* __restrict__ e_sdir, const long long* __restrict__ pos,
-                            long long n_edges, unsigned int* __restrict__ keys, unsigned int* __restrict__ vals) {
+                            const long long* __restrict__ n_edges, unsigned int* __restrict__ keys,
+                            unsigned int* __restrict__ vals) {
   long long e = (long long)blockIdx.x * blockDim.x + threadIdx.x;
-  if (e >= n_edges || !e_alive[e]) return;
-  const long long o = pos[e];
+  if (e >= *n_edges) return;
+  if (pos && !e_alive[e]) return;
+  const long long o = pos ? pos[e] : e;
   keys[o] = 2u * (unsigned int)e_src[e] + (e_sdir[e] > 0 ? 0u : 1u);
   vals[o] = (unsigned int)e;
 }
 
-__global__ void k_lr_count(const unsigned int* __restrict__ keys, long long n_live, int4* __restrict__ lrows) {
-  long long i = (long long)blockIdx.x * blockDim.x + threadIdx.x;
-  if (i < n_live) atomicAdd(&lrows[keys[i]].y, 1);
+__global__ void k_lr_count(const unsigned int* __restrict__ keys, const long long* __restrict__ n_live_at,
+                           int4* __restrict__ lrows) {
+  long long i = (long long)blockIdx.x * blockDim.x + threadIdx.x;
+  if (i < *n_live_at) atomicAdd(&lrows[keys[i]].y, 1);
 }
 
 #define LR_PER 8
-__global__ __launch_bounds__(256) void k_lr_alloc(const unsigned int* __restrict__ keys, long long n_live,
-                                                  int4* __restrict__ lrows, unsigned int* __restrict__ tick,
+__global__ __launch_bounds__(256) void k_lr_alloc(const unsigned int* __restrict__ keys,
+                                                  const long long* __restrict__ n_live_at, int4* __restrict__ lrows, unsigned int* __restrict__ tick,
                                                   unsigned long long* pool) {
   __shared__ unsigned int s_wave[4];
   __shared__ unsigned long long s_base;
+  const long long n_live = *n_live_at;
   const long long i0 = (long long)blockIdx.x * (256 * LR_PER) + threadIdx.x;
   unsigned int cnt[LR_PER], key[LR_PER], mine = 0;
 #pragma unroll
@@ -160,11 +166,11 @@
 
 #define LR_DONE 0xffffffffu
 __global__ void k_lr_fill(const unsigned int* __restrict__ keys, const unsigned int* __restrict__ edge_of,
-                          unsigned int* __restrict__ tick, long long n_live, int4* __restrict__ lrows,
-                          const int* __restrict__ e_tgt, const signed char* __restrict__ e_tdir,
+                          unsigned int* __restrict__ tick, const long long* __restrict__ n_live_at,
+                          int4* __restrict__ lrows, const int* __restrict__ e_tgt, const signed char* __restrict__ e_tdir,
                           unsigned int* __restrict__ tmp, int2* __restrict__ lent) {
   long long i = (long long)blockIdx.x * blockDim.x + threadIdx.x;
-  if (i >= n_live) return;
+  if (i >= *n_live_at) return;
   const unsigned int key = keys[i], e = edge_of[i];
   const int4 rw = lrows[key];
   if (rw.y == 1) {
@@ -178,12 +184,13 @@
 }
 
 __global__ __launch_bounds__(256) void k_lr_finish(const unsigned int* __restrict__ keys, const unsigned int* __restrict__ tick,
-                                                   long long n_live, const unsigned int* __restrict__ tmp,
+                                                   const long long* __restrict__ n_live_at,
+                                                   const unsigned int* __restrict__ tmp,
                                                    const int* __restrict__ e_tgt, const signed char* __restrict__ e_tdir,
                                                    int4* __restrict__ lrows, int2* __restrict__ lent,
                                                    unsigned int* __restrict__ long_rows, unsigned long long* n_long) {
   long long i = (long long)blockIdx.x * blockDim.x + threadIdx.x;
-  bool mine = i < n_live && tick[i] == 0u;
+  bool mine = i < *n_live_at && tick[i] == 0u;
   unsigned int key = 0;
   int off = 0, cnt = 0;
   if (mine) {
@@ -284,20 +291,29 @@
     c->ladj_valid = true;
     return AMG_OK;
   }
-  const long long rows = 2 * c->n_nodes, E = c->n_edges;
+  const bool intact = c->edges_intact && !getenv("AMG_LADJ_SCAN");
+  if (!intact) AMGCHK(late_settle(c));
+  const long long rows = 2 * c->n_nodes, E = c->edge_bound;
   AMGCHK(c->ladj_rows.ensure((size_t)(rows + 2) * sizeof(int4)));
-  AMGCHK(c->ladj_pos.ensure((size_t)(E + 2) * sizeof(long long)));
   unsigned long long* ctr = c->status.as<unsigned long long>() + ST_COMPACT_A;
-  {
+  long long total = E;
+  const long long* n_live = late_word(c, LATE_N_EDGES);
+  if (intact) {
     ClearList cl;
     cl.add(c->ladj_rows.p, (size_t)(rows + 2) * sizeof(int4));
     cl.add(ctr, 2 * sizeof(unsigned long long));
-    AMGCHK(prim_exscan_bytes_set(c, c->edge_alive.as<unsigned char>(), c->ladj_pos.as<long long>(), (size_t)E, &cl));
-  }
-  long long total = 0;
-  {
+    AMGCHK(clear_many(c, cl));
+  } else {
+    AMGCHK(c->ladj_pos.ensure((size_t)(E + 2) * sizeof(long long)));
+    {
+      ClearList cl;
+      cl.add(c->ladj_rows.p, (size_t)(rows + 2) * sizeof(int4));
+      cl.add(ctr, 2 * sizeof(unsigned long long));
+      AMGCHK(prim_exscan_bytes_set(c, c->edge_alive.as<unsigned char>(), c->ladj_pos.as<long long>(), (size_t)E, &cl));
+    }
+    n_live = c->ladj_pos.as<long long>() + E;
     FetchList l;
-    l.add(c->ladj_pos.as<long long>() + E);
+    l.add(n_live);
     AMGCHK(fetch(c, l, reinterpret_cast<unsigned long long*>(&total)));
   }
   AMGCHK(c->ladj.ensure((size_t)(total + 1) * sizeof(int2)));
@@ -309,14 +325,15 @@
   unsigned int* long_rows = tmp + (total + 2);
   if (total > 0) {
     hipLaunchKernelGGL(k_live_keys, dim3(nblk(E, 256)), dim3(256), 0, st, c->edge_alive.as<unsigned char>(),
-                       c->edge_src.as<int>(), c->edge_sdir.as<signed char>(), c->ladj_pos.as<long long>(), E, keys,
+                       c->edge_src.as<int>(), c->edge_sdir.as<signed char>(),
+                       intact ? (const long long*)nullptr : c->ladj_pos.as<long long>(), late_word(c, LATE_N_EDGES), keys,
                        edge_of);
-    hipLaunchKernelGGL(k_lr_count, dim3(nblk(total, 256)), dim3(256), 0, st, keys, total, c->ladj_rows.as<int4>());
-    hipLaunchKernelGGL(k_lr_alloc, dim3(nblk(total, 256 * LR_PER)), dim3(256), 0, st, keys, total, c->ladj_rows.as<int4>(),
+    hipLaunchKernelGGL(k_lr_count, dim3(nblk(total, 256)), dim3(256), 0, st, keys, n_live, c->ladj_rows.as<int4>());
+    hipLaunchKernelGGL(k_lr_alloc, dim3(nblk(total, 256 * LR_PER)), dim3(256), 0, st, keys, n_live, c->ladj_rows.as<int4>(),
                        tick, ctr);
-    hipLaunchKernelGGL(k_lr_fill, dim3(nblk(total, 256)), dim3(256), 0, st, keys, edge_of, tick, total,
+    hipLaunchKernelGGL(k_lr_fill, dim3(nblk(total, 256)), dim3(256), 0, st, keys, edge_of, tick, n_live,
                        c->ladj_rows.as<int4>(), c->edge_tgt.as<int>(), c->edge_tdir.as<signed char>(), tmp, c->ladj.as<int2>());
-    hipLaunchKernelGGL(k_lr_finish, dim3(nblk(total, 256)), dim3(256), 0, st, keys, tick, total, tmp, c->edge_tgt.as<int>(),
+    hipLaunchKernelGGL(k_lr_finish, dim3(nblk(total, 256)), dim3(256), 0, st, keys, tick, n_live, tmp, c->edge_tgt.as<int>(),
                        c->edge_tdir.as<signed char>(), c->ladj_rows.as<int4>(), c->ladj.as<int2>(), long_rows, ctr + 1);
     const long long hub_words = (E + 31) / 32 + 1;
     AMGCHK(c->hub_bits.ensure((size_t)LR_HUB_BLOCKS * (size_t)hub_words * sizeof(unsigned int)));
@@ -360,10 +377,12 @@
   NEED_BUILT(c);
   if (n < 0 || (n > 0 && !edge_ids)) return amg_fail(AMG_E_ARG, "bad edge list");
   if (n == 0) return AMG_OK;
+  AMGCHK(late_settle(c));
   AMGCHK(c->s0.ensure((size_t)n * sizeof(int)));
   HIPCHK(hipMemcpyAsync(c->s0.p, edge_ids, (size_t)n * sizeof(int), hipMemcpyHostToDevice, c->stream));
   hipLaunchKernelGGL(k_kill_listed, dim3(nblk(n, 256)), dim3(256), 0, c->stream, c->s0.as<int>(), (long long)n,
                      c->n_edges, c->edge_alive.as<unsigned char>());
+  c->edges_intact = false;
   c->ladj_valid = false;
   c->pristine = false;
   c->edge_own_deaths = true;
@@ -565,7 +584,10 @@
   if (D == 0) return AMG_OK;
   stages_reset(c);
   const bool by_labels = !c->pristine || getenv("AMG_CLIP_COMPONENTS");
-  if (by_labels) AMGCHK(ensure_components(c));
+  if (by_labels) {
+    AMGCHK(ensure_components(c));
+    AMGCHK(late_settle(c));
+  }
   stage_begin(c, "clip");
   unsigned long long* acc = c->status.as<unsigned long long>() + ST_COV_SUM;
   AMGCHK(c->s0.ensure((size_t)D + 8));
@@ -613,6 +635,7 @@
   const long long D = c->n_nodes;
   if (D == 0) return AMG_OK;
   AMGCHK(ensure_components(c));
+  AMGCHK(late_settle(c));
   size_t nc = (size_t)(c->n_components + 2);
   AMGCHK(c->s0.ensure((size_t)D + 8));
   AMGCHK(c->s4.ensure(2 * nc * sizeof(unsigned int)));
diff --git a/amira_amd/csrc/amg_internal.h b/amira_amd/csrc/amg_internal.h
--- a/amira_amd/csrc/amg_internal.h
+++ b/amira_amd/csrc/amg_internal.h
@@ -243,6 +243,12 @@
   int64_t match_total = 0, match_npat = 0;
   DevBuf match_read, match_pos, match_off, match_wave;
 
+  DevBuf late;
+  bool late_pending[2] = {false, false};
+  bool late_learn = false;
+  int64_t edge_bound = 0;
+  bool edges_intact = false;
+
   DevBuf status;
   unsigned long long* mail_host = nullptr;
   unsigned long long* mail_dev = nullptr;
@@ -340,6 +346,10 @@
 int fetch_status(amg_ctx* c, unsigned long long* out , const ClearList* filler = nullptr);
 int stream_wait(amg_ctx* c);
 
+enum LateWord { LATE_N_EDGES = 0, LATE_N_COMPONENTS = 1, LATE_WORDS = 2 };
+int late_settle(amg_ctx* c);
+static inline const long long* late_word(const amg_ctx* c, LateWord w) { return c->late.as<long long>() + w; }
+
 void stage_begin(amg_ctx* c, const char* name);
 void stage_end(amg_ctx* c);
 void stages_reset(amg_ctx* c);
```

Result: no change. 10.11 billion gene-mers/s (median of 6 runs) (+0.7%).
